# 2Retr0/GodotGaussianSplatting

Hardware: NVIDIA H100
Metric: Msplats/s (higher is better)
Workload: dtype f32

## Files before the change

### godotgaussiansplatting_b200/csrc/common.cuh

```cuda
#pragma once
#include <cuda_runtime.h>
#include <stdint.h>
#include <stdio.h>

#include "../../include/gsr.h"

namespace gsr {

constexpr int TILE = 16;
constexpr int NUM_PLANES = 15;
constexpr int PROJ_THREADS = 256;

void set_last_error(const char *fmt, ...);

#define GSR_CUDA_TRY(expr)                                                                         \
    do {                                                                                           \
        cudaError_t _e = (expr);                                                                   \
        if (_e != cudaSuccess) {                                                                   \
            ::gsr::set_last_error("%s:%d: %s -> %s", __FILE__, __LINE__, #expr, cudaGetErrorString(_e)); \
            return (_e == cudaErrorMemoryAllocation) ? GSR_ERR_OOM : GSR_ERR_CUDA;                 \
        }                                                                                          \
    } while (0)

__device__ __forceinline__ float g_max(float x, float y) { return (x < y) ? y : x; }
__device__ __forceinline__ float g_min(float x, float y) { return (y < x) ? y : x; }
__device__ __forceinline__ float g_clamp(float x, float lo, float hi) { return g_min(g_max(x, lo), hi); }

__device__ __forceinline__ float det_exp2(float t) {
    const float MAGIC = 12582912.0f;
    float tc = g_min(g_max(t, -127.0f), 128.0f);
    float tm = __fadd_rn(tc, MAGIC);
    float nf = __fsub_rn(tm, MAGIC);
    float f = __fsub_rn(tc, nf);
    float p = 0x1.446c7ep-13f;
    p = __fmaf_rn(p, f, 0x1.5f48c8p-10f);
    p = __fmaf_rn(p, f, 0x1.3b29d8p-7f);
    p = __fmaf_rn(p, f, 0x1.c6aeccp-5f);
    p = __fmaf_rn(p, f, 0x1.ebfbe0p-3f);
    p = __fmaf_rn(p, f, 0x1.62e430p-1f);
    p = __fmaf_rn(p, f, 1.0f);
    uint32_t sbits = (__float_as_uint(tm) << 23) + 0x3F800000u;
    return __fmul_rn(p, __uint_as_float(sbits));
}

__device__ __forceinline__ float det_exp(float x) { return det_exp2(__fmul_rn(x, 0x1.715476p+0f)); }

__device__ __forceinline__ float det_log2(float x) {
    int eadj = 0;
    if (x < 0x1p-126f) { x = __fmul_rn(x, 0x1p+32f); eadj = -32; }
    uint32_t u = __float_as_uint(x);
    int e = (int)(u >> 23) - 127;
    float m = __uint_as_float((u & 0x007FFFFFu) | 0x3F800000u);
    if (m >= 0x1.6a09e6p+0f) { m = __fmul_rn(m, 0.5f); e += 1; }
    float s = __fdiv_rn(__fsub_rn(m, 1.0f), __fadd_rn(m, 1.0f));
    float z = __fmul_rn(s, s);
    float g = 0x1.ba18b8p-2f;
    g = __fmaf_rn(g, z, 0x1.27471ep-1f);
    g = __fmaf_rn(g, z, 0x1.ec70e6p-1f);
    g = __fmaf_rn(g, z, 0x1.715476p+1f);
    return __fadd_rn((float)(e + eadj), __fmul_rn(s, g));
}

__device__ __forceinline__ float det_pow(float x, float y) {
    if (!(x > 0.0f)) return 0.0f;
    return det_exp2(__fmul_rn(y, det_log2(x)));
}

struct FrameState {
    unsigned long long dup_total;
    uint32_t dup_sorted;
    uint32_t visible;
    int32_t last_tile_plus1;
    uint32_t overflow;
    uint32_t proj_ticket;
    uint32_t pad0;
    unsigned long long staged;
    uint32_t comp_head;
    uint32_t comp_cta_limit;
    uint32_t pad[4];
};
static_assert(sizeof(FrameState) == 64, "FrameState is one 64-byte slot of the history ring");

struct Uniforms {
    float camera_pos[3];
    float model_scale;
    int32_t dims[2];
    float time;
    float pad;
};
static_assert(sizeof(Uniforms) == 32, "uniform block must be 32 bytes");

struct SortWorkspace {
    uint32_t *hist = nullptr;
    uint32_t *status = nullptr;
    uint32_t *tickets = nullptr;
    uint32_t *alt_keys = nullptr;
    uint32_t *alt_vals = nullptr;
    uint32_t *n_dev = nullptr;
    uint64_t max_n = 0;
    uint32_t max_tiles = 0;
    int grid_hist = 0, grid_sweep_pairs = 0, grid_sweep_keys = 0;
    size_t bytes() const;
};
int sort_workspace_create(SortWorkspace &ws, uint64_t max_n, bool need_alt_buffers);
void sort_workspace_destroy(SortWorkspace &ws);
int sort_pairs_device(SortWorkspace &ws, uint32_t *keys, uint32_t *vals, const uint32_t *n_ptr, uint32_t *alt_keys,
                      uint32_t *alt_vals, cudaStream_t stream, int *launches);
uint32_t sort_tile_keys();

struct ProjectionArgs {
    const float4 *soa;
    uint64_t plane_stride;
    uint32_t num_splats;
    float vp[32];
    Uniforms u;
    float focal_base[2];
    float lim_lo[2], lim_hi[2];
    int32_t band_y0, band_y1;
    int32_t row_mod, row_rem;
    int32_t fast_reject;
    int32_t sh_bulk_min;
    int32_t fast_mode;
    float w_frob2;
    float4 *records;
    uint32_t *keys, *values;
    uint32_t capacity;
    unsigned long long *lookback;
    FrameState *frame;
};
int launch_projection(const ProjectionArgs &a, cudaStream_t stream);

constexpr int GROUP_MAX = 16;
constexpr int GROUP_PHASES = 3;
#define GSR_GROUP_TIMEOUT_NS 2000000000ull
struct GroupFlags {
    unsigned long long seg_meta[GROUP_PHASES][GROUP_MAX][2];
    uint32_t done[GROUP_MAX];
    uint32_t released;
    uint32_t error;
    uint32_t scat_ticket;
    int32_t scat_last;
    unsigned long long seg_total[GROUP_MAX];
    uint32_t seg_prefix[GROUP_MAX + 1];
};
constexpr size_t GROUP_FLAGS_BYTES = 4096;
static_assert(sizeof(GroupFlags) <= GROUP_FLAGS_BYTES, "flag page");
struct GroupPeers {
    GroupFlags *flags[GROUP_MAX];
    int world, rank;
};
struct ScatterPeers {
    int world, rank, parity;
    uint32_t seq;
    uint32_t first, count;
    uint32_t seg_cap;
    float4 *records[GROUP_MAX];
    uint32_t *keys[GROUP_MAX];
    uint32_t *values[GROUP_MAX];
    GroupFlags *flags[GROUP_MAX];
    unsigned long long *lookback;
};
int launch_projection_scatter(const ProjectionArgs &a, const ScatterPeers &sp, cudaStream_t stream);
uint32_t projection_scatter_blocks(uint32_t count);
int launch_group_wait_segments(GroupFlags *flags, int parity, int world, uint32_t seq, uint32_t seg_cap, uint32_t capacity, FrameState *frame, cudaStream_t stream);
int launch_gather_segments(const GroupFlags *flags, int world, uint32_t seg_cap, const uint32_t *rx_keys, const uint32_t *rx_vals, uint32_t *keys, uint32_t *vals,
                           int grid, cudaStream_t stream);
int launch_publish_frame_state(const FrameState *frame, FrameState *host_mapped, cudaStream_t stream);
int launch_group_wait_released(GroupFlags *flags, uint32_t need, cudaStream_t stream);
int launch_group_wait_done(GroupFlags *flags, int world, uint32_t seq, cudaStream_t stream);
int launch_group_signal_done(const GroupPeers &peers, int root, int rank, uint32_t seq, cudaStream_t stream);
int launch_group_release(const GroupPeers &peers, int world, uint32_t value, cudaStream_t stream);
uint32_t projection_num_blocks(uint32_t num_splats);

int launch_tile_ranges(const uint32_t *sorted_keys, const FrameState *frame, uint2 *bounds, uint32_t num_tiles,
                       int quirks, int sharded, int32_t *sync_word, int grid, cudaStream_t stream);
int launch_band_fixup(const int32_t *global_last_plus1, float4 *out, int32_t width, int32_t height, int32_t tiles_x, int32_t num_tiles_total,
                      int32_t band_y0, int32_t band_y1, int32_t row_mod, int32_t row_rem, cudaStream_t stream);

struct CompositeArgs {
    const float4 *records;
    const uint32_t *values;
    const uint2 *bounds;
    float4 *out;
    int32_t width, height, tiles_x;
    int32_t tile_begin;
    int32_t row_step;
    int32_t num_tiles;
    float heatmap_factor;
    uint32_t target_tile_id;
    float4 *pick;
    FrameState *frame;
    int32_t count_staged;
    const uint32_t *order;
    uint32_t *consumed;
    int32_t ctas_per_sm;
    int32_t sm_count;
    int32_t contract;
    ulonglong4 *trace;
    uint32_t *trace_count;
    uint32_t trace_cap;
};
int launch_composite(const CompositeArgs &a, cudaStream_t stream);
int composite_max_ctas_per_sm(int *out);
int launch_tile_order(const uint2 *bounds, int32_t tile_begin, int32_t row_step, int32_t tiles_x, int32_t num_tiles, uint32_t *hint, uint32_t *order,
                      FrameState *frame, uint32_t sparse_tiles, uint32_t sparse_cta_limit, cudaStream_t stream);

int launch_ply_to_soa(const float *ply, uint32_t nprops, uint64_t count, float creation_time, float4 *soa, uint64_t plane_stride, uint64_t first,
                      cudaStream_t stream);
int launch_present(const float4 *rgba, void *out, uint64_t pixels, int format, cudaStream_t stream);
size_t present_bytes_per_pixel(int format);
int launch_aos_to_soa(const float4 *aos, uint64_t count, float4 *soa, uint64_t plane_stride, uint64_t first, cudaStream_t stream);

int preload_group_kernels();
int preload_projection_kernels();
int preload_sort_kernels();
int preload_ranges_kernels();
int launch_frame_clear(FrameState *frame, unsigned long long *links, uint32_t n_links, uint2 *bounds, uint32_t n_bounds, cudaStream_t stream);
int preload_ingest_kernels();
int preload_present_kernels();
int preload_composite_kernels();

}
```

### godotgaussiansplatting_b200/csrc/compositor.cu

```cuda
#include <stdlib.h>
#include <string.h>

#include "common.cuh"

namespace gsr {

namespace {

constexpr int CHUNK = 256;
constexpr int THREADS = 128;
constexpr float MIN_ALPHA = 1.0f / 255.0f;

struct F2 { float lo, hi; };
__device__ __forceinline__ F2 pk(float lo, float hi) { F2 r; r.lo = lo; r.hi = hi; return r; }
__device__ __forceinline__ void upk(F2 v, float &lo, float &hi) { lo = v.lo; hi = v.hi; }
__device__ __forceinline__ F2 fma2(F2 a, F2 b, F2 c) { return pk(__fmaf_rn(a.lo, b.lo, c.lo), __fmaf_rn(a.hi, b.hi, c.hi)); }
__device__ __forceinline__ F2 mul2(F2 a, F2 b) { return pk(__fmul_rn(a.lo, b.lo), __fmul_rn(a.hi, b.hi)); }
__device__ __forceinline__ F2 add2(F2 a, F2 b) { return pk(__fadd_rn(a.lo, b.lo), __fadd_rn(a.hi, b.hi)); }
__device__ __forceinline__ F2 sub2(F2 a, F2 b) { return pk(__fsub_rn(a.lo, b.lo), __fsub_rn(a.hi, b.hi)); }
__device__ __forceinline__ F2 mul_add2_unfused(F2 a, F2 b, F2 c) { return add2(mul2(a, b), c); }
__device__ __forceinline__ F2 bc(float x) { return pk(x, x); }

struct Staged {
    float4 a;
    float4 b;
    float c;
};

__device__ __forceinline__ Staged null_splat() {
    Staged s;
    s.a = make_float4(0.f, 0.f, 0.f, 0.f);
    s.b = make_float4(0.f, 0.f, 0.f, 0.f);
    s.c = 0.f;
    return s;
}

__device__ __forceinline__ Staged gather(const float4 *__restrict__ records, const uint32_t *__restrict__ values, uint32_t idx) {
    const uint32_t v = __ldg(values + idx);
    const float4 *r = records + (uint64_t)v * 3u;
    const float4 r0 = __ldg(r + 0), r1 = __ldg(r + 1), r2 = __ldg(r + 2);
    Staged s;
    s.a = make_float4(r0.x, r0.y, -0.5f * r1.x, -0.5f * r1.z);
    s.b = make_float4(-r1.y, r2.w, r2.x, r2.y);
    s.c = r2.z;
    return s;
}

#ifndef GSR_COMP_GROUP
#define GSR_COMP_GROUP 4
#endif
constexpr int GU = GSR_COMP_GROUP;
static_assert(CHUNK % GU == 0, "a chunk is a whole number of groups");

#ifndef GSR_CPU_EMU
__device__ __forceinline__ unsigned long long globaltimer_ns() { unsigned long long t; asm volatile("mov.u64 %0, %globaltimer;" : "=l"(t)); return t; }
__device__ __forceinline__ uint32_t smid() { uint32_t r; asm volatile("mov.u32 %0, %smid;" : "=r"(r)); return r; }
#else
inline unsigned long long globaltimer_ns() { return 0ull; }
inline uint32_t smid() { return 0u; }
#endif

struct BlendK {
    F2 L2E2, MAGIC2, ONE2, C6, C5, C4, C3, C2, C1;
};
__device__ __forceinline__ BlendK make_blend_k() {
    BlendK k;
    k.L2E2 = bc(0x1.715476p+0f); k.MAGIC2 = bc(12582912.0f); k.ONE2 = bc(1.0f);
    k.C6 = bc(0x1.446c7ep-13f); k.C5 = bc(0x1.5f48c8p-10f); k.C4 = bc(0x1.3b29d8p-7f); k.C3 = bc(0x1.c6aeccp-5f);
    k.C2 = bc(0x1.ebfbe0p-3f); k.C1 = bc(0x1.62e430p-1f);
    return k;
}

template <bool CONTRACT>
__device__ __forceinline__ void phase_a(const float4 A[GU], const float4 B[GU], F2 npx2, float fpy, const BlendK &K, F2 al2[GU], F2 om2[GU]) {
    float oy[GU];
    F2 ox2[GU], pw2[GU], tm2[GU], e2[GU];
#pragma unroll
    for (int u = 0; u < GU; ++u) { ox2[u] = add2(bc(A[u].x), npx2); oy[u] = A[u].y - fpy; }
#pragma unroll
    for (int u = 0; u < GU; ++u) pw2[u] = mul2(bc(A[u].z), ox2[u]);
#pragma unroll
    for (int u = 0; u < GU; ++u) {
        const float czoy = A[u].w * oy[u];
        if (CONTRACT) pw2[u] = fma2(bc(czoy), bc(oy[u]), mul2(pw2[u], ox2[u]));
        else pw2[u] = mul_add2_unfused(pw2[u], ox2[u], bc(__fmul_rn(czoy, oy[u])));
    }
#pragma unroll
    for (int u = 0; u < GU; ++u) e2[u] = mul2(bc(B[u].x), ox2[u]);
#pragma unroll
    for (int u = 0; u < GU; ++u) pw2[u] = CONTRACT ? fma2(e2[u], bc(oy[u]), pw2[u]) : mul_add2_unfused(e2[u], bc(oy[u]), pw2[u]);
#pragma unroll
    for (int u = 0; u < GU; ++u) pw2[u] = mul2(pw2[u], K.L2E2);
#pragma unroll
    for (int u = 0; u < GU; ++u) {
        float tl, th;
        upk(pw2[u], tl, th);
        tl = g_min(g_max(tl, -127.0f), 128.0f);
        th = g_min(g_max(th, -127.0f), 128.0f);
        pw2[u] = pk(tl, th);
    }
#pragma unroll
    for (int u = 0; u < GU; ++u) tm2[u] = add2(pw2[u], K.MAGIC2);
#pragma unroll
    for (int u = 0; u < GU; ++u) al2[u] = sub2(tm2[u], K.MAGIC2);
#pragma unroll
    for (int u = 0; u < GU; ++u) pw2[u] = sub2(pw2[u], al2[u]);
#pragma unroll
    for (int u = 0; u < GU; ++u) e2[u] = fma2(K.C6, pw2[u], K.C5);
#pragma unroll
    for (int u = 0; u < GU; ++u) e2[u] = fma2(e2[u], pw2[u], K.C4);
#pragma unroll
    for (int u = 0; u < GU; ++u) e2[u] = fma2(e2[u], pw2[u], K.C3);
#pragma unroll
    for (int u = 0; u < GU; ++u) e2[u] = fma2(e2[u], pw2[u], K.C2);
#pragma unroll
    for (int u = 0; u < GU; ++u) e2[u] = fma2(e2[u], pw2[u], K.C1);
#pragma unroll
    for (int u = 0; u < GU; ++u) e2[u] = fma2(e2[u], pw2[u], K.ONE2);
#pragma unroll
    for (int u = 0; u < GU; ++u) {
        float ml, mh;
        upk(tm2[u], ml, mh);
        tm2[u] = pk(__uint_as_float((__float_as_uint(ml) << 23) + 0x3F800000u), __uint_as_float((__float_as_uint(mh) << 23) + 0x3F800000u));
    }
#pragma unroll
    for (int u = 0; u < GU; ++u) e2[u] = mul2(e2[u], tm2[u]);
#pragma unroll
    for (int u = 0; u < GU; ++u) al2[u] = mul2(bc(B[u].y), e2[u]);
#pragma unroll
    for (int u = 0; u < GU; ++u) om2[u] = sub2(K.ONE2, al2[u]);
}

template <bool CONTRACT>
__device__ __forceinline__ void phase_b(const float4 B[GU], const float *s_c, int j, const F2 al2[GU], const F2 om2[GU], F2 &cr2, F2 &cg2, F2 &cb2,
                                        float &t0, float &t1, bool &alive_mid) {
#pragma unroll
    for (int u = 0; u < GU; ++u) {
        const float cbl = s_c[j + u];
        if (u == GU / 2) alive_mid = (t0 > MIN_ALPHA) || (t1 > MIN_ALPHA);
        const bool a0 = t0 > MIN_ALPHA, a1 = t1 > MIN_ALPHA;
        float al, ah, pl, ph;
        upk(al2[u], al, ah);
        const F2 t2 = pk(t0, t1);
        upk(mul2(t2, om2[u]), pl, ph);
        const F2 m2 = pk(a0 ? al : 0.0f, a1 ? ah : 0.0f);
        if (CONTRACT) {
            cr2 = fma2(mul2(bc(B[u].z), m2), t2, cr2);
            cg2 = fma2(mul2(bc(B[u].w), m2), t2, cg2);
            cb2 = fma2(mul2(bc(cbl), m2), t2, cb2);
        } else {
            cr2 = mul_add2_unfused(mul2(bc(B[u].z), m2), t2, cr2);
            cg2 = mul_add2_unfused(mul2(bc(B[u].w), m2), t2, cg2);
            cb2 = mul_add2_unfused(mul2(bc(cbl), m2), t2, cb2);
        }
        t0 = a0 ? pl : t0;
        t1 = a1 ? ph : t1;
    }
}

#ifndef GSR_COMP_MIN_BLOCKS
#define GSR_COMP_MIN_BLOCKS 3
#endif

template <bool CONTRACT>
__global__ void __launch_bounds__(THREADS, GSR_COMP_MIN_BLOCKS) composite_kernel(const __grid_constant__ CompositeArgs p) {
    __shared__ float4 s_a[CHUNK];
    __shared__ float4 s_b[CHUNK];
    __shared__ float s_c[CHUNK];
    __shared__ uint32_t s_vote[THREADS / 32];
    __shared__ uint32_t s_tile;

    const uint32_t tid = threadIdx.x, lane = tid & 31u, warp = tid >> 5;
    {
        const uint32_t limit = p.frame->comp_cta_limit;
        if (limit && blockIdx.x >= limit) return;
    }
    const BlendK K = make_blend_k();
    uint32_t staged = 0;
    unsigned long long t_start = 0;

    for (;;) {
        if (tid == 0) {
            const uint32_t ticket = atomicAdd(&p.frame->comp_head, 1u);
            s_tile = ticket < (uint32_t)p.num_tiles ? (p.order ? p.order[ticket] : ticket) : 0xFFFFFFFFu;
            if (p.trace) t_start = globaltimer_ns();
        }
        __syncthreads();
        const uint32_t local_tile = s_tile;
        if (local_tile == 0xFFFFFFFFu) break;
        const uint32_t tile_id = (uint32_t)p.tile_begin + (local_tile / (uint32_t)p.tiles_x) * (uint32_t)(p.row_step * p.tiles_x) + local_tile % (uint32_t)p.tiles_x;

        const uint32_t tx = tile_id % (uint32_t)p.tiles_x, ty = tile_id / (uint32_t)p.tiles_x;
        const int px0 = (int)(tx * TILE + 2u * (tid & 7u)), py = (int)(ty * TILE + (tid >> 3));
        const F2 npx2 = pk(-(float)px0, -(float)(px0 + 1));
        const float fpy = (float)py;

        const uint2 bounds = p.bounds[tile_id];
        const int32_t diff = (int32_t)(bounds.y - bounds.x);
        const int num_splats = diff > 0 ? diff : 0;
        const int num_iterations = (int)ceilf((float)num_splats / (float)CHUNK);

        F2 cr2 = pk(0.f, 0.f), cg2 = cr2, cb2 = cr2;
        float t0 = 1.0f, t1 = 1.0f;

        Staged n0 = null_splat(), n1 = null_splat();
        if (num_iterations > 0) {
            if ((int)tid < num_splats) n0 = gather(p.records, p.values, bounds.x + tid);
            if ((int)tid + THREADS < num_splats) n1 = gather(p.records, p.values, bounds.x + tid + THREADS);
        }

        int consumed = 0;
        for (int i = 0; i < num_iterations; ++i) {
            const int sort_offset = CHUNK * i;
            const int chunk = (num_splats - sort_offset) < CHUNK ? (num_splats - sort_offset) : CHUNK;
            staged += (uint32_t)chunk;
            consumed = i + 1;
            s_a[tid] = n0.a; s_b[tid] = n0.b; s_c[tid] = n0.c;
            s_a[tid + THREADS] = n1.a; s_b[tid + THREADS] = n1.b; s_c[tid + THREADS] = n1.c;
            __syncthreads();
            n0 = null_splat(); n1 = null_splat();
            if (i + 1 < num_iterations) {
                const int nb = sort_offset + CHUNK;
                if (nb + (int)tid < num_splats) n0 = gather(p.records, p.values, bounds.x + (uint32_t)nb + tid);
                if (nb + (int)tid + THREADS < num_splats) n1 = gather(p.records, p.values, bounds.x + (uint32_t)nb + tid + THREADS);
            }

            const int chunkg = (chunk + GU - 1) & ~(GU - 1);
            float4 A[GU], B[GU];
#pragma unroll
            for (int u = 0; u < GU; ++u) { A[u] = s_a[u]; B[u] = s_b[u]; }
            bool go = __any_sync(0xffffffffu, (t0 > MIN_ALPHA) || (t1 > MIN_ALPHA));
            for (int j = 0; j < chunkg && go; j += GU) {
                F2 al2[GU], om2[GU];
                phase_a<CONTRACT>(A, B, npx2, fpy, K, al2, om2);
                float4 Bc[GU];
#pragma unroll
                for (int u = 0; u < GU; ++u) Bc[u] = B[u];
                const int jn = (j + GU < CHUNK) ? j + GU : j;
#pragma unroll
                for (int u = 0; u < GU; ++u) { A[u] = s_a[jn + u]; B[u] = s_b[jn + u]; }
                bool alive_mid = true;
                phase_b<CONTRACT>(Bc, s_c, j, al2, om2, cr2, cg2, cb2, t0, t1, alive_mid);
                go = __any_sync(0xffffffffu, alive_mid);
            }

            const uint32_t wsum = __reduce_add_sync(0xffffffffu, (uint32_t)(t0 * 255.0f) + (uint32_t)(t1 * 255.0f));
            if (lane == 0) s_vote[warp] = wsum;
            __syncthreads();
            uint32_t shared_t = 0;
#pragma unroll
            for (int w = 0; w < THREADS / 32; ++w) shared_t += s_vote[w];
            if (!(shared_t > 255u)) break;
        }

        float r0, r1, g0, g1, b0, b1;
        upk(cr2, r0, r1); upk(cg2, g0, g1); upk(cb2, b0, b1);
        const float hx = (float)num_splats * 5e-4f;
        const float h0 = 0.0f * (1.0f - hx) + 1.0f * hx, h1 = 0.0f * (1.0f - hx) + 0.2f * hx, h2c = 1.0f * (1.0f - hx) + 0.2f * hx;
        if (py < p.height) {
            float4 *row = p.out + (uint64_t)py * (uint64_t)p.width;
            const float k0 = 1.0f - t0, k1 = 1.0f - t1;
            if (px0 < p.width)
                row[px0] = make_float4(r0 + h0 * k0 * p.heatmap_factor, g0 + h1 * k0 * p.heatmap_factor, b0 + h2c * k0 * p.heatmap_factor, 1.0f);
            if (px0 + 1 < p.width)
                row[px0 + 1] = make_float4(r1 + h0 * k1 * p.heatmap_factor, g1 + h1 * k1 * p.heatmap_factor, b1 + h2c * k1 * p.heatmap_factor, 1.0f);
        }
        if ((tid & 15u) == 0u && tile_id == p.target_tile_id && t0 != 1.0f) {
            const uint32_t v = p.values[bounds.x + (bounds.y - bounds.x) / 10u];
            const float4 q0 = p.records[(uint64_t)v * 3u + 0], q1 = p.records[(uint64_t)v * 3u + 1];
            *p.pick = make_float4(q0.z, q0.w, q1.w, (float)num_splats);
        }
        if (tid == 0) {
            if (p.consumed) p.consumed[local_tile] = (uint32_t)consumed | 0x80000000u;
            if (p.trace) {
                const uint32_t k = atomicAdd(p.trace_count, 1u);
                if (k < p.trace_cap) p.trace[k] = make_ulonglong4(((unsigned long long)tile_id << 32) | smid(), t_start, globaltimer_ns(),
                                                                  ((unsigned long long)(uint32_t)consumed << 32) | 1u | ((uint32_t)num_iterations << 1));
            }
        }
        __syncthreads();
    }
    if (tid == 0 && staged && p.count_staged) atomicAdd(&p.frame->staged, (unsigned long long)staged);
}

}

#ifndef GSR_CPU_EMU
int preload_composite_kernels() {
    cudaFuncAttributes fa;
    GSR_CUDA_TRY(cudaFuncGetAttributes(&fa, composite_kernel<true>));
    GSR_CUDA_TRY(cudaFuncGetAttributes(&fa, composite_kernel<false>));
    return GSR_OK;
}

int composite_max_ctas_per_sm(int *out) {
    int a = 0, b = 0;
    GSR_CUDA_TRY(cudaOccupancyMaxActiveBlocksPerMultiprocessor(&a, composite_kernel<true>, THREADS, 0));
    GSR_CUDA_TRY(cudaOccupancyMaxActiveBlocksPerMultiprocessor(&b, composite_kernel<false>, THREADS, 0));
    *out = a < b ? a : b;
    if (*out < 1) *out = 1;
    return GSR_OK;
}

int launch_composite(const CompositeArgs &a, cudaStream_t stream) {
    if (a.num_tiles <= 0) return GSR_OK;
    const int per_sm = a.ctas_per_sm > 0 ? a.ctas_per_sm : 1;
    const int grid = a.num_tiles < a.sm_count * per_sm ? a.num_tiles : a.sm_count * per_sm;
    if (a.contract) composite_kernel<true><<<grid, THREADS, 0, stream>>>(a);
    else composite_kernel<false><<<grid, THREADS, 0, stream>>>(a);
    GSR_CUDA_TRY(cudaGetLastError());
    return GSR_OK;
}
#endif

}
```

### godotgaussiansplatting_b200/csrc/gsr_api.cu

```cuda
#include <stdarg.h>
#include <stdlib.h>
#include <stddef.h>
#include <string.h>
#include <unistd.h>

#include <new>

#include "common.cuh"

namespace gsr {

static thread_local char g_last_error[512] = "";

void set_last_error(const char *fmt, ...) {
    va_list ap;
    va_start(ap, fmt);
    vsnprintf(g_last_error, sizeof g_last_error, fmt, ap);
    va_end(ap);
}

}

using namespace gsr;

constexpr int EV_PER_FRAME = 7;

struct gsr_ctx {
    int device = 0;
    uint32_t flags = 0;
    uint64_t max_splats = 0, capacity = 0, plane_stride = 0, num_splats = 0;
    uint64_t cap_stride = 0;
    cudaStream_t stream = nullptr, own_stream = nullptr;
    float4 *soa = nullptr;
    float4 *records = nullptr;
    float4 *records2 = nullptr;
    uint32_t *keys = nullptr;
    uint32_t *vals = nullptr;
    uint32_t *keys_cur = nullptr, *vals_cur = nullptr;
    float4 *records_cur = nullptr;
    cudaStream_t front_stream = nullptr;
    cudaEvent_t front_gate = nullptr;
    int overlap = -1;
    SortWorkspace sort;
    FrameState *ring = nullptr;
    FrameState *frame = nullptr;
    unsigned long long *lookback = nullptr;
    uint32_t lookback_blocks = 0;
    uint64_t frame_counter = 0;
    uint2 *bounds = nullptr;
    uint32_t *comp_order = nullptr, *comp_hint = nullptr;
    int comp_ctas_per_sm = 2, comp_order_mode = 1, comp_max_ctas = 1, comp_sparse_per_sm = 5;
    uint64_t comp_hint_key = 0;
    FrameState *pick_frame = nullptr;
    ulonglong4 *trace = nullptr;
    uint32_t *trace_count = nullptr;
    uint32_t trace_cap = 0;
    float4 *fb = nullptr, *fb_ext = nullptr;
    float4 *fb2 = nullptr;
    void *stage[2] = {nullptr, nullptr};
    float4 *fb_last = nullptr;
    cudaStream_t copy_stream = nullptr;
    cudaEvent_t ev_done[2] = {nullptr, nullptr}, ev_copied[2] = {nullptr, nullptr};
    bool copied_valid[2] = {false, false};
    uint64_t async_counter = 0;
    bool peer_mode = false, peer_opened = false;
    float4 *peer_fb[2] = {nullptr, nullptr};
    uint64_t peer_counter = 0;
    float4 *pick = nullptr;
    float4 *staging = nullptr;
    uint64_t staging_splats = 0;
    uint32_t *unsorted_keys = nullptr, *unsorted_vals = nullptr;
    bool keep_unsorted = false;
    int width = 0, height = 0, tiles_x = 0, tiles_y = 0, band_y0 = 0, band_y1 = 0;
    bool band_set = false;
    int row_mod = 1, row_rem = 0;
    int32_t *sync_word = nullptr;
    struct Group {
        void *arena = nullptr;
        uint64_t rx_capacity = 0;
        int rank = 0, world = 0;
        char *peer_arena[GROUP_MAX] = {};
        GroupFlags *flags[GROUP_MAX] = {};
        float4 *root_fb[2] = {nullptr, nullptr};
        void *opened[3 * GROUP_MAX] = {};
        int n_opened = 0;
        int present_rows = 0;
        uint32_t seq = 0;
        uint64_t slice = 0;
        uint32_t seg_cap = 0;
    } grp;
    cudaEvent_t *ev = nullptr;
    FrameState *host_ring = nullptr;
    cudaEvent_t *ev_stat = nullptr;
    uint64_t stats_polled = 0;
    uint64_t m_high = 0;
    uint64_t capacity_max = 0;
    bool ev_valid = false;
    uint32_t last_launches = 0;
    int sm_count = 0;
};

struct gsr_sorter {
    int device = 0;
    SortWorkspace ws;
    cudaEvent_t e0 = nullptr, e1 = nullptr;
    bool timed = false;
};

namespace {

int use_device(int device) {
    GSR_CUDA_TRY(cudaSetDevice(device));
    return GSR_OK;
}

int check_device(int device) {
    int count = 0;
    cudaError_t e = cudaGetDeviceCount(&count);
    if (e != cudaSuccess || count == 0) {
        set_last_error("no CUDA device available (%s); libgsr has no CPU fallback", e != cudaSuccess ? cudaGetErrorString(e) : "count=0");
        return GSR_ERR_CUDA;
    }
    if (device < 0 || device >= count) {
        set_last_error("device ordinal %d out of range [0,%d)", device, count);
        return GSR_ERR_INVALID;
    }
    cudaDeviceProp prop;
    GSR_CUDA_TRY(cudaGetDeviceProperties(&prop, device));
    if (prop.major != 9 || prop.minor != 0) {
        set_last_error("device %d is sm_%d%d; libgsr is built for sm_90a only", device, prop.major, prop.minor);
        return GSR_ERR_CUDA;
    }
    return GSR_OK;
}

void group_detach(gsr_ctx *c) {
    if (c->front_stream) cudaStreamSynchronize(c->front_stream);
    if (c->stream) cudaStreamSynchronize(c->stream);
    if (c->copy_stream) cudaStreamSynchronize(c->copy_stream);
    for (int i = 0; i < c->grp.n_opened; ++i) cudaIpcCloseMemHandle(c->grp.opened[i]);
    c->grp.n_opened = 0;
    if (c->grp.world > 1) { c->row_mod = 1; c->row_rem = 0; }
    c->grp.world = 0; c->grp.rank = 0; c->grp.seq = 0; c->grp.present_rows = 0;
    c->grp.root_fb[0] = c->grp.root_fb[1] = nullptr;
}

float4 *framebuffer(gsr_ctx *c) { return c->fb_ext ? c->fb_ext : (c->fb_last ? c->fb_last : c->fb); }

void free_ctx(gsr_ctx *c) {
    if (!c) return;
    cudaSetDevice(c->device);
    if (c->stream) cudaStreamSynchronize(c->stream);
    if (c->front_stream) { cudaStreamSynchronize(c->front_stream); cudaStreamDestroy(c->front_stream); }
    cudaFree(c->soa); cudaFree(c->records); cudaFree(c->records2); cudaFree(c->keys); cudaFree(c->vals);
    sort_workspace_destroy(c->sort);
    if (c->copy_stream) cudaStreamSynchronize(c->copy_stream);
    if (c->peer_opened) { cudaIpcCloseMemHandle(c->peer_fb[0]); cudaIpcCloseMemHandle(c->peer_fb[1]); }
    cudaFree(c->stage[0]); cudaFree(c->stage[1]);
    cudaFree(c->ring); cudaFree(c->lookback); cudaFree(c->bounds); cudaFree(c->comp_order); cudaFree(c->comp_hint); cudaFree(c->pick_frame); cudaFree(c->fb); cudaFree(c->fb2); cudaFree(c->pick); cudaFree(c->staging);
    for (int i = 0; i < 2; ++i) { if (c->ev_done[i]) cudaEventDestroy(c->ev_done[i]); if (c->ev_copied[i]) cudaEventDestroy(c->ev_copied[i]); }
    if (c->copy_stream) cudaStreamDestroy(c->copy_stream);
    cudaFree(c->sync_word);
    for (int i = 0; i < c->grp.n_opened; ++i) cudaIpcCloseMemHandle(c->grp.opened[i]);
    cudaFree(c->grp.arena);
    cudaFree(c->unsorted_keys); cudaFree(c->unsorted_vals); cudaFree(c->trace); cudaFree(c->trace_count);
    if (c->ev) {
        for (int i = 0; i < GSR_HISTORY_FRAMES * EV_PER_FRAME; ++i) if (c->ev[i]) cudaEventDestroy(c->ev[i]);
        delete[] c->ev;
    }
    if (c->ev_stat) {
        for (int i = 0; i < GSR_HISTORY_FRAMES; ++i) if (c->ev_stat[i]) cudaEventDestroy(c->ev_stat[i]);
        delete[] c->ev_stat;
    }
    if (c->host_ring) cudaFreeHost(c->host_ring);
    if (c->own_stream) cudaStreamDestroy(c->own_stream);
    delete c;
}

}

extern "C" {

GSR_API const char *gsr_error_string(int code) {
    switch (code) {
        case GSR_OK: return "ok";
        case GSR_ERR_INVALID: return "invalid argument";
        case GSR_ERR_CUDA: return "CUDA failure or no usable sm_90 device (no CPU fallback exists)";
        case GSR_ERR_OOM: return "device out of memory";
        case GSR_ERR_STATE: return "call order violated";
        case GSR_ERR_OVERFLOW: return "duplicate list exceeded capacity";
        default: return "unknown error";
    }
}
GSR_API const char *gsr_last_error(void) { return g_last_error; }
GSR_API const char *gsr_version(void) { return "gsr 0.1.0 (sm_90a)"; }
GSR_API int gsr_device_count(void) {
    int n = 0;
    if (cudaGetDeviceCount(&n) != cudaSuccess) return 0;
    return n;
}

GSR_API int gsr_create(const gsr_config *cfg, gsr_ctx **out) {
    if (!cfg || !out || cfg->max_splats == 0) { set_last_error("gsr_create: null config/out or max_splats == 0"); return GSR_ERR_INVALID; }
    *out = nullptr;
    int rc = check_device(cfg->device);
    if (rc) return rc;
    if ((rc = use_device(cfg->device))) return rc;
    if (cfg->max_splats >= (1ull << 32) - 256ull) { set_last_error("max_splats must be < 2^32-256"); return GSR_ERR_INVALID; }
    gsr_ctx *c = new (std::nothrow) gsr_ctx();
    if (!c) return GSR_ERR_OOM;
    c->device = cfg->device;
    c->flags = cfg->flags;
    if (!(c->flags & (GSR_FLAG_REFERENCE_QUIRKS | GSR_FLAG_FIXED_RANGES))) c->flags |= GSR_FLAG_REFERENCE_QUIRKS;
    c->max_splats = cfg->max_splats;
    const uint64_t factor = cfg->dup_capacity_factor ? cfg->dup_capacity_factor : 10;
    c->capacity_max = (1ull << 30) - 1;
    c->capacity = c->max_splats * factor;
    if (c->capacity > c->capacity_max) c->capacity = c->capacity_max;
    c->plane_stride = (c->max_splats + 255ull) & ~255ull;
    cudaDeviceGetAttribute(&c->sm_count, cudaDevAttrMultiProcessorCount, c->device);
    if ((rc = composite_max_ctas_per_sm(&c->comp_max_ctas))) { delete c; return rc; }

#define TRY_ALLOC(ptr, bytes)                                                                      \
    do {                                                                                           \
        cudaError_t _e = cudaMalloc((void **)&(ptr), (bytes));                                     \
        if (_e != cudaSuccess) {                                                                   \
            set_last_error("cudaMalloc(%s, %llu B) -> %s", #ptr, (unsigned long long)(bytes), cudaGetErrorString(_e)); \
            free_ctx(c);                                                                           \
            return _e == cudaErrorMemoryAllocation ? GSR_ERR_OOM : GSR_ERR_CUDA;                   \
        }                                                                                          \
    } while (0)

    cudaError_t se;
    {
        int least = 0, greatest = 0;
        cudaDeviceGetStreamPriorityRange(&least, &greatest);
        se = cudaStreamCreateWithPriority(&c->own_stream, cudaStreamNonBlocking, greatest);
    }
    if (se != cudaSuccess) { set_last_error("cudaStreamCreate -> %s", cudaGetErrorString(se)); free_ctx(c); return GSR_ERR_CUDA; }
    c->stream = c->own_stream;
    se = cudaStreamCreateWithFlags(&c->copy_stream, cudaStreamNonBlocking);
    if (se == cudaSuccess) {
        int least = 0, greatest = 0;
        cudaDeviceGetStreamPriorityRange(&least, &greatest);
        se = cudaStreamCreateWithPriority(&c->front_stream, cudaStreamNonBlocking, least);
    }
    for (int i = 0; i < 2 && se == cudaSuccess; ++i) {
        se = cudaEventCreateWithFlags(&c->ev_done[i], cudaEventDisableTiming);
        if (se == cudaSuccess) se = cudaEventCreateWithFlags(&c->ev_copied[i], cudaEventDisableTiming);
    }
    if (se != cudaSuccess) { set_last_error("copy stream/events -> %s", cudaGetErrorString(se)); free_ctx(c); return GSR_ERR_CUDA; }
    TRY_ALLOC(c->soa, sizeof(float4) * NUM_PLANES * c->plane_stride);
    TRY_ALLOC(c->records, sizeof(float4) * 3ull * c->max_splats);
    TRY_ALLOC(c->records2, sizeof(float4) * 3ull * c->max_splats);
    c->cap_stride = (c->capacity + 1023ull) & ~1023ull;
    TRY_ALLOC(c->keys, sizeof(uint32_t) * 3ull * c->cap_stride);
    TRY_ALLOC(c->vals, sizeof(uint32_t) * 3ull * c->cap_stride);
    c->keys_cur = c->keys; c->vals_cur = c->vals; c->records_cur = c->records;
    c->lookback_blocks = projection_num_blocks((uint32_t)c->max_splats);
    TRY_ALLOC(c->ring, sizeof(FrameState) * GSR_HISTORY_FRAMES);
    TRY_ALLOC(c->lookback, sizeof(unsigned long long) * ((size_t)c->lookback_blocks + 2u * GROUP_MAX * GROUP_MAX));
    c->frame = c->ring;
    TRY_ALLOC(c->pick, sizeof(float4));
    TRY_ALLOC(c->sync_word, sizeof(int32_t));
    c->staging_splats = c->max_splats < (1ull << 18) ? c->max_splats : (1ull << 18);
    TRY_ALLOC(c->staging, sizeof(float4) * NUM_PLANES * c->staging_splats);
#undef TRY_ALLOC
    rc = sort_workspace_create(c->sort, c->capacity, false);
    if (rc) { free_ctx(c); return rc; }
    c->ev = new (std::nothrow) cudaEvent_t[GSR_HISTORY_FRAMES * EV_PER_FRAME]();
    if (!c->ev) { free_ctx(c); return GSR_ERR_OOM; }
    for (int i = 0; i < GSR_HISTORY_FRAMES * EV_PER_FRAME; ++i) {
        if (cudaEventCreate(&c->ev[i]) != cudaSuccess) { set_last_error("cudaEventCreate failed"); free_ctx(c); return GSR_ERR_CUDA; }
    }
    c->ev_stat = new (std::nothrow) cudaEvent_t[GSR_HISTORY_FRAMES]();
    if (!c->ev_stat) { free_ctx(c); return GSR_ERR_OOM; }
    for (int i = 0; i < GSR_HISTORY_FRAMES; ++i) {
        if (cudaEventCreateWithFlags(&c->ev_stat[i], cudaEventDisableTiming) != cudaSuccess) { set_last_error("cudaEventCreate failed"); free_ctx(c); return GSR_ERR_CUDA; }
    }
    if (cudaHostAlloc((void **)&c->host_ring, sizeof(FrameState) * GSR_HISTORY_FRAMES, cudaHostAllocMapped | cudaHostAllocPortable) != cudaSuccess) {
        set_last_error("cudaHostAlloc(frame mirror) failed"); c->host_ring = nullptr; free_ctx(c); return GSR_ERR_OOM;
    }
    memset(c->host_ring, 0, sizeof(FrameState) * GSR_HISTORY_FRAMES);
    cudaMemsetAsync(c->soa, 0, sizeof(float4) * NUM_PLANES * c->plane_stride, c->stream);
    cudaMemsetAsync(c->records, 0, sizeof(float4) * 3ull * c->max_splats, c->stream);
    cudaMemsetAsync(c->records2, 0, sizeof(float4) * 3ull * c->max_splats, c->stream);
    cudaMemsetAsync(c->pick, 0, sizeof(float4), c->stream);
    cudaMemsetAsync(c->sync_word, 0, sizeof(int32_t), c->stream);
    cudaMemsetAsync(c->ring, 0, sizeof(FrameState) * GSR_HISTORY_FRAMES, c->stream);
    if ((rc = preload_group_kernels()) || (rc = preload_projection_kernels()) || (rc = preload_sort_kernels()) || (rc = preload_ranges_kernels()) ||
        (rc = preload_ingest_kernels()) || (rc = preload_present_kernels()) || (rc = preload_composite_kernels())) { free_ctx(c); return rc; }
    cudaError_t e = cudaStreamSynchronize(c->stream);
    if (e != cudaSuccess) { set_last_error("init sync -> %s", cudaGetErrorString(e)); free_ctx(c); return GSR_ERR_CUDA; }
    *out = c;
    return GSR_OK;
}

GSR_API int gsr_destroy(gsr_ctx *ctx) {
    free_ctx(ctx);
    return GSR_OK;
}

GSR_API int gsr_set_stream(gsr_ctx *c, void *cuda_stream) {
    if (!c) return GSR_ERR_INVALID;
    int rc = use_device(c->device);
    if (rc) return rc;
    GSR_CUDA_TRY(cudaStreamSynchronize(c->front_stream));
    GSR_CUDA_TRY(cudaStreamSynchronize(c->stream));
    c->stream = cuda_stream ? (cudaStream_t)cuda_stream : c->own_stream;
    c->ev_valid = false; c->front_gate = nullptr;
    return GSR_OK;
}

GSR_API int gsr_upload_splats_aos(gsr_ctx *c, const float *splat60, uint64_t first, uint64_t count) {
    if (!c || (!splat60 && count)) return GSR_ERR_INVALID;
    if (count > c->max_splats || first > c->max_splats - count) { set_last_error("upload range [%llu,%llu) exceeds max_splats %llu", (unsigned long long)first, (unsigned long long)(first + count), (unsigned long long)c->max_splats); return GSR_ERR_INVALID; }
    int rc = use_device(c->device);
    if (rc) return rc;
    GSR_CUDA_TRY(cudaStreamSynchronize(c->front_stream));
    uint64_t done = 0;
    while (done < count) {
        const uint64_t m = (count - done) < c->staging_splats ? (count - done) : c->staging_splats;
        GSR_CUDA_TRY(cudaMemcpyAsync(c->staging, splat60 + (done * 60ull), m * 240ull, cudaMemcpyHostToDevice, c->stream));
        if ((rc = launch_aos_to_soa(c->staging, m, c->soa, c->plane_stride, first + done, c->stream))) return rc;
        done += m;
    }
    GSR_CUDA_TRY(cudaStreamSynchronize(c->stream));
    if (first + count > c->num_splats) c->num_splats = first + count;
    return GSR_OK;
}

GSR_API int gsr_upload_ply_raw(gsr_ctx *c, const float *ply, uint32_t nprops, uint64_t first, uint64_t count, float creation_time) {
    if (!c || (!ply && count)) return GSR_ERR_INVALID;
    if (nprops < 62 || nprops > 256) { set_last_error("gsr_upload_ply_raw: %u properties; need the 62 standard 3DGS floats (x..rot_3) first", nprops); return GSR_ERR_INVALID; }
    if (count > c->max_splats || first > c->max_splats - count) { set_last_error("upload range [%llu,%llu) exceeds max_splats %llu", (unsigned long long)first, (unsigned long long)(first + count), (unsigned long long)c->max_splats); return GSR_ERR_INVALID; }
    int rc = use_device(c->device);
    if (rc) return rc;
    const uint64_t staging_floats = c->staging_splats * 60ull;
    const uint64_t per = staging_floats / nprops;
    if (per == 0) { set_last_error("gsr_upload_ply_raw: staging buffer too small"); return GSR_ERR_INVALID; }
    GSR_CUDA_TRY(cudaStreamSynchronize(c->front_stream));
    uint64_t done = 0;
    while (done < count) {
        const uint64_t m = (count - done) < per ? (count - done) : per;
        GSR_CUDA_TRY(cudaMemcpyAsync(c->staging, ply + done * nprops, m * nprops * sizeof(float), cudaMemcpyHostToDevice, c->stream));
        if ((rc = launch_ply_to_soa(reinterpret_cast<const float *>(c->staging), nprops, m, creation_time, c->soa, c->plane_stride, first + done, c->stream))) return rc;
        done += m;
    }
    GSR_CUDA_TRY(cudaStreamSynchronize(c->stream));
    if (first + count > c->num_splats) c->num_splats = first + count;
    return GSR_OK;
}

GSR_API int gsr_resize(gsr_ctx *c, int32_t width, int32_t height) {
    if (!c || width < 1 || height < 1) { set_last_error("gsr_resize: bad size %dx%d", width, height); return GSR_ERR_INVALID; }
    const int tx = (width + TILE - 1) / TILE, ty = (height + TILE - 1) / TILE;
    if ((int64_t)tx * ty > 65536) {
        set_last_error("gsr_resize: %d tiles exceed the 16-bit tile id of the sort key", tx * ty);
        return GSR_ERR_INVALID;
    }
    int rc = use_device(c->device);
    if (rc) return rc;
    GSR_CUDA_TRY(cudaStreamSynchronize(c->front_stream));
    GSR_CUDA_TRY(cudaStreamSynchronize(c->stream));
    c->front_gate = nullptr;
    c->width = c->height = c->tiles_x = c->tiles_y = 0;
    cudaFree(c->bounds); c->bounds = nullptr;
    cudaFree(c->comp_order); c->comp_order = nullptr;
    cudaFree(c->comp_hint); c->comp_hint = nullptr;
    GSR_CUDA_TRY(cudaStreamSynchronize(c->copy_stream));
    cudaFree(c->fb); c->fb = nullptr;
    cudaFree(c->fb2); c->fb2 = nullptr;
    cudaFree(c->stage[0]); cudaFree(c->stage[1]); c->stage[0] = c->stage[1] = nullptr;
    c->fb_last = nullptr; c->copied_valid[0] = c->copied_valid[1] = false;
    if (c->peer_opened) { cudaIpcCloseMemHandle(c->peer_fb[0]); cudaIpcCloseMemHandle(c->peer_fb[1]); c->peer_opened = false; }
    c->peer_mode = false; c->peer_fb[0] = c->peer_fb[1] = nullptr; c->peer_counter = 0; c->async_counter = 0;
    group_detach(c);
    GSR_CUDA_TRY(cudaMalloc((void **)&c->bounds, sizeof(uint2) * (size_t)tx * ty));
    GSR_CUDA_TRY(cudaMalloc((void **)&c->comp_order, sizeof(uint32_t) * (size_t)tx * ty));
    GSR_CUDA_TRY(cudaMalloc((void **)&c->comp_hint, sizeof(uint32_t) * (size_t)tx * ty));
    GSR_CUDA_TRY(cudaMemsetAsync(c->comp_hint, 0, sizeof(uint32_t) * (size_t)tx * ty, c->stream));
    c->comp_hint_key = 0;
    if (!c->pick_frame) GSR_CUDA_TRY(cudaMalloc((void **)&c->pick_frame, sizeof(FrameState)));
    GSR_CUDA_TRY(cudaMalloc((void **)&c->fb, sizeof(float4) * (size_t)width * height));
    GSR_CUDA_TRY(cudaMalloc((void **)&c->fb2, sizeof(float4) * (size_t)width * height));
    GSR_CUDA_TRY(cudaMemsetAsync(c->fb, 0, sizeof(float4) * (size_t)width * height, c->stream));
    GSR_CUDA_TRY(cudaMemsetAsync(c->fb2, 0, sizeof(float4) * (size_t)width * height, c->stream));
    c->width = width; c->height = height; c->tiles_x = tx; c->tiles_y = ty;
    if (!c->band_set) { c->band_y0 = 0; c->band_y1 = ty; }
    if (c->band_y1 > ty) c->band_y1 = ty;
    if (c->band_y0 > c->band_y1) c->band_y0 = c->band_y1;
    return GSR_OK;
}

GSR_API int gsr_set_row_interleave(gsr_ctx *c, int32_t row_rem, int32_t row_mod) {
    if (!c || row_mod < 1 || row_rem < 0 || row_rem >= row_mod) { set_last_error("gsr_set_row_interleave: need 0 <= rem < mod"); return GSR_ERR_INVALID; }
    c->row_mod = row_mod; c->row_rem = row_rem;
    return GSR_OK;
}

GSR_API void *gsr_band_sync_word(gsr_ctx *c) { return c ? (void *)c->sync_word : nullptr; }

GSR_API int gsr_band_fixup(gsr_ctx *c) {
    if (!c) return GSR_ERR_INVALID;
    if (c->row_mod <= 1 || !c->fb_last) return GSR_OK;
    if (c->flags & GSR_FLAG_FIXED_RANGES) return GSR_OK;
    int rc = use_device(c->device);
    if (rc) return rc;
    return launch_band_fixup(c->sync_word, c->fb_last, c->width, c->height, c->tiles_x, c->tiles_x * c->tiles_y, c->band_y0, c->band_y1,
                             c->row_mod, c->row_rem, c->stream);
}

GSR_API int gsr_set_band(gsr_ctx *c, int32_t row_begin, int32_t row_end) {
    if (!c || c->tiles_y == 0) { set_last_error("gsr_set_band before gsr_resize"); return GSR_ERR_STATE; }
    if (row_begin < 0 || row_end > c->tiles_y || row_begin > row_end) { set_last_error("band [%d,%d) outside [0,%d]", row_begin, row_end, c->tiles_y); return GSR_ERR_INVALID; }
    c->band_y0 = row_begin; c->band_y1 = row_end;
    c->band_set = !(row_begin == 0 && row_end == c->tiles_y);
    return GSR_OK;
}

static void frame_constants(const float *view_proj, const Uniforms &u, ProjectionArgs &pa) {
    {
        const float tfi0 = view_proj[16 + 0], tfi1 = view_proj[16 + 5];
        const volatile float hw = (float)u.dims[0] * 0.5f, hh = (float)u.dims[1] * 0.5f;
        const volatile float f0 = hw * tfi0, f1 = hh * tfi1;
        const volatile float t0 = 1.0f / tfi0, t1 = 1.0f / tfi1;
        const volatile float n0 = -t0, n1 = -t1;
        pa.focal_base[0] = f0; pa.focal_base[1] = f1;
        pa.lim_lo[0] = n0 * 1.3f; pa.lim_lo[1] = n1 * 1.3f;
        pa.lim_hi[0] = t0 * 1.3f; pa.lim_hi[1] = t1 * 1.3f;
    }
    {
        float g[3][3];
        for (int i = 0; i < 3; ++i)
            for (int j = 0; j < 3; ++j) {
                g[i][j] = 0.0f;
                for (int r = 0; r < 3; ++r) g[i][j] += view_proj[4 * i + r] * view_proj[4 * j + r];
            }
        float nrm = 0.0f;
        for (int i = 0; i < 3; ++i) {
            float row = 0.0f;
            for (int j = 0; j < 3; ++j) row += g[i][j] < 0.0f ? -g[i][j] : g[i][j];
            nrm = row > nrm ? row : nrm;
        }
        pa.w_frob2 = nrm * 1.0001f;
    }
}

static int grow_capacity(gsr_ctx *c, uint64_t want) {
    if (want > c->capacity_max) want = c->capacity_max;
    if (want <= c->capacity) return GSR_OK;
    GSR_CUDA_TRY(cudaStreamSynchronize(c->front_stream));
    GSR_CUDA_TRY(cudaStreamSynchronize(c->stream));
    GSR_CUDA_TRY(cudaStreamSynchronize(c->copy_stream));
    c->front_gate = nullptr;
    cudaFree(c->keys); cudaFree(c->vals); c->keys = c->vals = c->keys_cur = c->vals_cur = nullptr;
    sort_workspace_destroy(c->sort);
    const bool unsorted = c->unsorted_keys != nullptr;
    cudaFree(c->unsorted_keys); cudaFree(c->unsorted_vals); c->unsorted_keys = c->unsorted_vals = nullptr;
    c->capacity = want;
    c->cap_stride = (c->capacity + 1023ull) & ~1023ull;
    GSR_CUDA_TRY(cudaMalloc((void **)&c->keys, sizeof(uint32_t) * 3ull * c->cap_stride));
    GSR_CUDA_TRY(cudaMalloc((void **)&c->vals, sizeof(uint32_t) * 3ull * c->cap_stride));
    c->keys_cur = c->keys; c->vals_cur = c->vals;
    if (unsorted) {
        GSR_CUDA_TRY(cudaMalloc((void **)&c->unsorted_keys, sizeof(uint32_t) * c->capacity));
        GSR_CUDA_TRY(cudaMalloc((void **)&c->unsorted_vals, sizeof(uint32_t) * c->capacity));
    }
    return sort_workspace_create(c->sort, c->capacity, false);
}

static int track_capacity(gsr_ctx *c) {
    if (c->flags & GSR_FLAG_STATIC_CAPACITY) return GSR_OK;
    while (c->stats_polled < c->frame_counter) {
        if (c->frame_counter - c->stats_polled > GSR_HISTORY_FRAMES) { c->stats_polled = c->frame_counter - GSR_HISTORY_FRAMES; continue; }
        const uint32_t slot = (uint32_t)(c->stats_polled % GSR_HISTORY_FRAMES);
        if (cudaEventQuery(c->ev_stat[slot]) != cudaSuccess) { cudaGetLastError(); break; }
        const uint64_t m = c->host_ring[slot].dup_total;
        if (m > c->m_high) c->m_high = m;
        c->stats_polled += 1;
    }
    if (c->m_high * 2ull > c->capacity && c->capacity < c->capacity_max) return grow_capacity(c, c->m_high * 3ull);
    return GSR_OK;
}

struct GroupFrame { uint32_t seq; int parity; int rows_local; };

static int stage_times(gsr_ctx *c, uint32_t slot, float out[5], float *front_ms) {
    cudaEvent_t *ev = c->ev + EV_PER_FRAME * slot;
    float front = 0.f, recv = 0.f;
    GSR_CUDA_TRY(cudaEventElapsedTime(&front, ev[0], ev[1]));
    GSR_CUDA_TRY(cudaEventElapsedTime(&recv, ev[2], ev[3]));
    out[0] = front + recv;
    for (int i = 1; i < 4; ++i) GSR_CUDA_TRY(cudaEventElapsedTime(&out[i], ev[2 + i], ev[3 + i]));
    out[4] = out[0] + out[1] + out[2] + out[3];
    if (front_ms) *front_ms = front;
    return GSR_OK;
}

static size_t arena_rx_keys_off(uint64_t cap, int parity) { return GROUP_FLAGS_BYTES + sizeof(uint32_t) * cap * (size_t)parity; }
static size_t arena_rx_vals_off(uint64_t cap, int parity) { return GROUP_FLAGS_BYTES + sizeof(uint32_t) * cap * (size_t)(GROUP_PHASES + parity); }
static size_t arena_records_off(uint64_t cap, uint64_t max_splats, int parity) { return GROUP_FLAGS_BYTES + sizeof(uint32_t) * cap * 2 * GROUP_PHASES + sizeof(float4) * 3ull * max_splats * (size_t)parity; }
static size_t arena_bytes(uint64_t cap, uint64_t max_splats) { return arena_records_off(cap, max_splats, GROUP_PHASES); }

static GroupPeers group_peers(const gsr_ctx *c, int parity) {
    (void)parity;
    GroupPeers p;
    memset(&p, 0, sizeof p);
    p.world = c->grp.world; p.rank = c->grp.rank;
    for (int r = 0; r < c->grp.world; ++r) p.flags[r] = c->grp.flags[r];
    return p;
}

static int render_enqueue(gsr_ctx *c, const float *view_proj, const void *uniforms32, float heatmap_factor, float4 *target = nullptr,
                          const GroupFrame *gf = nullptr) {
    if (!c || !view_proj || !uniforms32) return GSR_ERR_INVALID;
    if (c->width == 0) { set_last_error("gsr_render before gsr_resize"); return GSR_ERR_STATE; }
    Uniforms u;
    memcpy(&u, uniforms32, sizeof u);
    if (u.dims[0] != c->width || u.dims[1] != c->height) {
        set_last_error("uniform dims %dx%d differ from gsr_resize %dx%d", u.dims[0], u.dims[1], c->width, c->height);
        return GSR_ERR_INVALID;
    }
    int rc = use_device(c->device);
    if (rc) return rc;
    if ((rc = track_capacity(c))) return rc;
    cudaStream_t s = c->stream;
    const bool overlap = c->overlap > 0 && c->front_stream != nullptr;
    cudaStream_t fs = overlap ? c->front_stream : s;
    int launches = 0;
    const uint32_t slot = (uint32_t)(c->frame_counter % GSR_HISTORY_FRAMES);
    c->frame = c->ring + slot;
    cudaEvent_t *ev = c->ev + EV_PER_FRAME * slot;
    const int half = (int)(c->frame_counter & 1u);
    uint32_t *keys_in = c->keys + (size_t)half * c->cap_stride, *vals_in = c->vals + (size_t)half * c->cap_stride;
    uint32_t *keys_alt = c->keys + 2ull * c->cap_stride, *vals_alt = c->vals + 2ull * c->cap_stride;
    float4 *records = half ? c->records2 : c->records;
    const uint32_t n_tiles = (uint32_t)(c->tiles_x * c->tiles_y);

    if (overlap && c->front_gate) GSR_CUDA_TRY(cudaStreamWaitEvent(fs, c->front_gate, 0));
    {
        uint32_t links = projection_num_blocks((uint32_t)c->max_splats);
        if (gf) {
            const uint64_t first = (uint64_t)c->grp.rank * c->grp.slice;
            const uint64_t count = first < c->max_splats ? ((c->max_splats - first) < c->grp.slice ? (c->max_splats - first) : c->grp.slice) : 0;
            links = projection_scatter_blocks((uint32_t)count) * (uint32_t)c->grp.world;
        }
        if ((rc = launch_frame_clear(c->frame, c->lookback, links, overlap ? nullptr : c->bounds, overlap ? 0u : n_tiles, fs))) return rc;
        launches += 1;
    }
    GSR_CUDA_TRY(cudaEventRecord(ev[0], fs));

    ProjectionArgs pa;
    pa.soa = c->soa; pa.plane_stride = c->plane_stride; pa.num_splats = (uint32_t)c->max_splats;
    memcpy(pa.vp, view_proj, sizeof pa.vp);
    pa.u = u;
    frame_constants(view_proj, u, pa);
    const bool fast = c->row_mod > 1 && !gf;
    pa.band_y0 = c->band_y0; pa.band_y1 = c->band_y1;
    pa.row_mod = c->row_mod; pa.row_rem = c->row_rem;
    const bool want_reject = (c->flags & GSR_FLAG_FAST_REJECT) != 0 || c->row_mod >= 6;
    pa.fast_reject = (want_reject && fast) ? 1 : 0;
    pa.fast_mode = fast ? 1 : 0;
    pa.sh_bulk_min = (fast || c->row_mod > 1) ? 1 : 12;
    pa.records = records; pa.keys = keys_in; pa.values = vals_in; pa.capacity = (uint32_t)c->capacity;
    pa.lookback = c->lookback; pa.frame = c->frame;
    if (gf) {
        const int G = c->grp.world;
        ScatterPeers sp;
        memset(&sp, 0, sizeof sp);
        sp.world = G; sp.rank = c->grp.rank; sp.parity = gf->parity; sp.seq = gf->seq;
        const uint64_t first = (uint64_t)c->grp.rank * c->grp.slice;
        sp.first = (uint32_t)(first < c->max_splats ? first : c->max_splats);
        sp.count = (uint32_t)(first < c->max_splats ? ((c->max_splats - first) < c->grp.slice ? (c->max_splats - first) : c->grp.slice) : 0);
        sp.seg_cap = c->grp.seg_cap;
        for (int d = 0; d < G; ++d) {
            char *ar = c->grp.peer_arena[d];
            sp.records[d] = reinterpret_cast<float4 *>(ar + arena_records_off(c->grp.rx_capacity, c->max_splats, gf->parity));
            sp.keys[d] = reinterpret_cast<uint32_t *>(ar + arena_rx_keys_off(c->grp.rx_capacity, gf->parity)) + (size_t)c->grp.rank * c->grp.seg_cap;
            sp.values[d] = reinterpret_cast<uint32_t *>(ar + arena_rx_vals_off(c->grp.rx_capacity, gf->parity)) + (size_t)c->grp.rank * c->grp.seg_cap;
            sp.flags[d] = c->grp.flags[d];
        }
        sp.lookback = c->lookback;
        if ((rc = launch_projection_scatter(pa, sp, fs))) return rc;
        launches += 1;
    } else {
        if ((rc = launch_projection(pa, fs))) return rc;
        launches += pa.num_splats ? 1 : 0;
    }
    GSR_CUDA_TRY(cudaEventRecord(ev[1], fs));

    if (overlap) {
        GSR_CUDA_TRY(cudaStreamWaitEvent(s, ev[1], 0));
        if ((rc = launch_frame_clear(nullptr, nullptr, 0u, c->bounds, n_tiles, s))) return rc;
        launches += 1;
    }
    GSR_CUDA_TRY(cudaEventRecord(ev[2], s));
    if (gf) {
        const int G = c->grp.world;
        char *mine = c->grp.peer_arena[c->grp.rank];
        if ((rc = launch_group_wait_segments(c->grp.flags[c->grp.rank], gf->parity, G, gf->seq, c->grp.seg_cap, (uint32_t)c->capacity, c->frame, s))) return rc;
        if ((rc = launch_gather_segments(c->grp.flags[c->grp.rank], G, c->grp.seg_cap,
                                         reinterpret_cast<const uint32_t *>(mine + arena_rx_keys_off(c->grp.rx_capacity, gf->parity)),
                                         reinterpret_cast<const uint32_t *>(mine + arena_rx_vals_off(c->grp.rx_capacity, gf->parity)), keys_in, vals_in,
                                         c->sm_count * 8, s))) return rc;
        records = reinterpret_cast<float4 *>(mine + arena_records_off(c->grp.rx_capacity, c->max_splats, gf->parity));
        launches += 2;
    }
    c->keys_cur = keys_in; c->vals_cur = vals_in; c->records_cur = records;
    GSR_CUDA_TRY(cudaEventRecord(ev[3], s));

    if (c->keep_unsorted) {
        GSR_CUDA_TRY(cudaMemcpyAsync(c->unsorted_keys, keys_in, sizeof(uint32_t) * c->capacity, cudaMemcpyDeviceToDevice, s));
        GSR_CUDA_TRY(cudaMemcpyAsync(c->unsorted_vals, vals_in, sizeof(uint32_t) * c->capacity, cudaMemcpyDeviceToDevice, s));
    }
    const uint32_t *m_ptr = reinterpret_cast<const uint32_t *>(reinterpret_cast<const char *>(c->frame) + offsetof(FrameState, dup_sorted));
    if ((rc = sort_pairs_device(c->sort, keys_in, vals_in, m_ptr, keys_alt, vals_alt, s, &launches))) return rc;
    GSR_CUDA_TRY(cudaEventRecord(ev[4], s));

    const int sharded = fast ? 2 : ((!(c->band_y0 == 0 && c->band_y1 == c->tiles_y) || c->row_mod > 1) ? 1 : 0);
    if (fast) GSR_CUDA_TRY(cudaMemsetAsync(c->sync_word, 0, sizeof(int32_t), s));
    const int quirks = (c->flags & GSR_FLAG_FIXED_RANGES) ? 0 : 1;
    if ((rc = launch_tile_ranges(keys_in, c->frame, c->bounds, n_tiles, quirks, sharded, fast ? c->sync_word : nullptr, c->sm_count * 8, s))) return rc;
    launches += 1;
    GSR_CUDA_TRY(cudaEventRecord(ev[5], s));
    c->front_gate = ev[5];

    CompositeArgs ca;
    float4 *out_fb = c->fb_ext ? c->fb_ext : (target ? target : c->fb);
    for (int i = 0; i < 2; ++i) {
        const float4 *owned = c->peer_mode ? c->peer_fb[i] : (i ? c->fb2 : c->fb);
        if (c->copied_valid[i] && owned == out_fb) GSR_CUDA_TRY(cudaStreamWaitEvent(s, c->ev_copied[i], 0));
    }
    c->fb_last = out_fb;
    ca.records = records; ca.values = vals_in; ca.bounds = c->bounds; ca.out = out_fb;
    ca.width = c->width; ca.height = c->height; ca.tiles_x = c->tiles_x;
    {
        int first = c->band_y0 + ((c->row_rem - c->band_y0 % c->row_mod) + c->row_mod) % c->row_mod;
        int nrows = first < c->band_y1 ? (c->band_y1 - 1 - first) / c->row_mod + 1 : 0;
        ca.tile_begin = first * c->tiles_x;
        ca.row_step = c->row_mod;
        ca.num_tiles = nrows * c->tiles_x;
    }
    ca.heatmap_factor = heatmap_factor;
    ca.target_tile_id = 0xFFFFFFFFu;
    ca.pick = c->pick;
    ca.frame = c->frame; ca.count_staged = 1;
    ca.order = nullptr; ca.consumed = c->comp_hint;
    ca.ctas_per_sm = c->comp_ctas_per_sm < c->comp_max_ctas ? c->comp_ctas_per_sm : c->comp_max_ctas; ca.sm_count = c->sm_count;
    ca.contract = (c->flags & GSR_FLAG_UNCONTRACTED_BLEND) ? 0 : 1;
    {
        const uint64_t key = ((uint64_t)(uint32_t)ca.tile_begin << 32) ^ ((uint64_t)(uint32_t)ca.row_step << 24) ^ (uint64_t)(uint32_t)ca.num_tiles;
        if (key != c->comp_hint_key) { GSR_CUDA_TRY(cudaMemsetAsync(c->comp_hint, 0, sizeof(uint32_t) * (size_t)c->tiles_x * c->tiles_y, s)); c->comp_hint_key = key; }
    }
    if (c->comp_order_mode && ca.num_tiles > 0) {
        if ((rc = launch_tile_order(c->bounds, ca.tile_begin, ca.row_step, ca.tiles_x, ca.num_tiles, c->comp_hint, c->comp_order, c->frame,
                                    (uint32_t)(c->comp_sparse_per_sm * c->sm_count), (uint32_t)c->sm_count, s))) return rc;
        ca.order = c->comp_order;
        launches += 1;
    }
    ca.trace = c->trace; ca.trace_count = c->trace_count; ca.trace_cap = c->trace_cap;
    if (c->trace) GSR_CUDA_TRY(cudaMemsetAsync(c->trace_count, 0, sizeof(uint32_t), s));
    if (gf && !gf->rows_local && c->grp.rank != 0 && gf->seq >= 3u) {
        if ((rc = launch_group_wait_released(c->grp.flags[c->grp.rank], gf->seq - 2u, s))) return rc;
        launches += 1;
    }
    if ((rc = launch_composite(ca, s))) return rc;
    launches += ca.num_tiles > 0 ? 1 : 0;
    if (gf && !gf->rows_local) {
        if ((rc = launch_group_signal_done(group_peers(c, gf->parity), 0, c->grp.rank, gf->seq, s))) return rc;
        launches += 1;
    }
    GSR_CUDA_TRY(cudaEventRecord(ev[6], s));
    if ((rc = launch_publish_frame_state(c->frame, c->host_ring + slot, s))) return rc;
    GSR_CUDA_TRY(cudaEventRecord(c->ev_stat[slot], s));
    c->ev_valid = true;
    c->frame_counter += 1;
    c->last_launches = (uint32_t)launches;
    return GSR_OK;
}

GSR_API int gsr_render(gsr_ctx *c, const float view_proj[32], const void *uniforms32, float heatmap_factor, float *out_host) {
    if (c && c->grp.world > 1) { set_last_error("gsr_render: a context attached to a group renders with gsr_render_async (all ranks, same frame)"); return GSR_ERR_STATE; }
    int rc = render_enqueue(c, view_proj, uniforms32, heatmap_factor);
    if (rc) return rc;
    if (out_host) {
        for (int attempt = 0; attempt < 8 && !(c->flags & GSR_FLAG_STATIC_CAPACITY); ++attempt) {
            const uint32_t slot = (uint32_t)((c->frame_counter - 1) % GSR_HISTORY_FRAMES);
            GSR_CUDA_TRY(cudaEventSynchronize(c->ev_stat[slot]));
            const FrameState &fs = c->host_ring[slot];
            if (!fs.overflow || c->capacity >= c->capacity_max) break;
            if ((rc = grow_capacity(c, fs.dup_total + fs.dup_total / 4ull + 1024ull))) return rc;
            if ((rc = render_enqueue(c, view_proj, uniforms32, heatmap_factor))) return rc;
        }
        GSR_CUDA_TRY(cudaMemcpyAsync(out_host, framebuffer(c), sizeof(float4) * (size_t)c->width * c->height, cudaMemcpyDeviceToHost, c->stream));
        GSR_CUDA_TRY(cudaStreamSynchronize(c->stream));
    }
    return GSR_OK;
}

static int readback_enqueue(gsr_ctx *c, float4 *frame, int slot, void *pinned_host, int format, uint32_t group_seq = 0) {
    const size_t pixels = (size_t)c->width * c->height;
    const size_t bpp = present_bytes_per_pixel(format);
    if (!bpp) { set_last_error("unknown output format 0x%x", format); return GSR_ERR_INVALID; }
    int rc;
    const bool convert = format != GSR_OUT_RGBA32F;
    if (convert && !c->stage[slot]) GSR_CUDA_TRY(cudaMalloc(&c->stage[slot], sizeof(float4) * pixels + 64));
    GSR_CUDA_TRY(cudaEventRecord(c->ev_done[slot], c->stream));
    GSR_CUDA_TRY(cudaStreamWaitEvent(c->copy_stream, c->ev_done[slot], 0));
    if (group_seq && (rc = launch_group_wait_done(c->grp.flags[c->grp.rank], c->grp.world, group_seq, c->copy_stream))) return rc;
    if (convert) {
        if ((rc = launch_present(frame, c->stage[slot], pixels, format, c->copy_stream))) return rc;
        GSR_CUDA_TRY(cudaMemcpyAsync(pinned_host, c->stage[slot], bpp * pixels, cudaMemcpyDeviceToHost, c->copy_stream));
    } else {
        GSR_CUDA_TRY(cudaMemcpyAsync(pinned_host, frame, sizeof(float4) * pixels, cudaMemcpyDeviceToHost, c->copy_stream));
    }
    GSR_CUDA_TRY(cudaEventRecord(c->ev_copied[slot], c->copy_stream));
    c->copied_valid[slot] = true;
    return GSR_OK;
}

static int render_async_impl(gsr_ctx *c, const float *view_proj, const void *uniforms32, float heatmap_factor, void *pinned_host, int format) {
    if (!c) return GSR_ERR_INVALID;
    if (c->grp.world > 1) {
        if (pinned_host) { set_last_error("group mode: render with a NULL host pointer on every rank, then gsr_readback_async on rank 0"); return GSR_ERR_STATE; }
        int rc = use_device(c->device);
        if (rc) return rc;
        GroupFrame gf;
        gf.seq = c->grp.seq + 1u; gf.parity = (int)(gf.seq % (uint32_t)GROUP_PHASES);
        const int slot = (int)((gf.seq - 1u) & 1u);
        gf.rows_local = c->grp.present_rows;
        float4 *target = c->grp.root_fb[slot];
        if (gf.rows_local) {
            target = slot ? c->fb2 : c->fb;
        } else if (c->grp.rank == 0) {
            if (c->copied_valid[slot]) GSR_CUDA_TRY(cudaStreamWaitEvent(c->stream, c->ev_copied[slot], 0));
            if (gf.seq >= 3u && (rc = launch_group_release(group_peers(c, gf.parity), c->grp.world, gf.seq - 2u, c->stream))) return rc;
        }
        if ((rc = render_enqueue(c, view_proj, uniforms32, heatmap_factor, target, &gf))) return rc;
        c->grp.seq = gf.seq;
        return GSR_OK;
    }
    if (c->peer_mode) {
        if (pinned_host) { set_last_error("peer mode: render with a NULL host pointer, then gsr_readback_async on the presenting rank"); return GSR_ERR_STATE; }
        int rc = use_device(c->device);
        if (rc) return rc;
        const int slot = (int)(c->peer_counter & 1u);
        if (c->copied_valid[slot]) GSR_CUDA_TRY(cudaStreamWaitEvent(c->stream, c->ev_copied[slot], 0));
        if ((rc = render_enqueue(c, view_proj, uniforms32, heatmap_factor, c->peer_fb[slot]))) return rc;
        c->peer_counter += 1;
        return GSR_OK;
    }
    if (!pinned_host || c->fb_ext) {
        if (format != GSR_OUT_RGBA32F && pinned_host) { set_last_error("converted read-back is unavailable with an external framebuffer"); return GSR_ERR_STATE; }
        int rc = render_enqueue(c, view_proj, uniforms32, heatmap_factor);
        if (rc) return rc;
        if (pinned_host)
            GSR_CUDA_TRY(cudaMemcpyAsync(pinned_host, framebuffer(c), sizeof(float4) * (size_t)c->width * c->height, cudaMemcpyDeviceToHost, c->stream));
        return GSR_OK;
    }
    int rc = use_device(c->device);
    if (rc) return rc;
    const int slot = (int)(c->async_counter & 1u);
    float4 *target = slot ? c->fb2 : c->fb;
    if ((rc = render_enqueue(c, view_proj, uniforms32, heatmap_factor, target))) return rc;
    if ((rc = readback_enqueue(c, target, slot, pinned_host, format))) return rc;
    c->async_counter += 1;
    return GSR_OK;
}

GSR_API int gsr_render_async(gsr_ctx *c, const float view_proj[32], const void *uniforms32, float heatmap_factor, float *pinned_host) {
    return render_async_impl(c, view_proj, uniforms32, heatmap_factor, pinned_host, GSR_OUT_RGBA32F);
}

GSR_API int gsr_render_async_rgb(gsr_ctx *c, const float view_proj[32], const void *uniforms32, float heatmap_factor, float *pinned_host_rgb) {
    return render_async_impl(c, view_proj, uniforms32, heatmap_factor, pinned_host_rgb, GSR_OUT_RGB32F);
}

GSR_API int gsr_render_async_fmt(gsr_ctx *c, const float view_proj[32], const void *uniforms32, float heatmap_factor, void *pinned_host, int32_t format) {
    if (!present_bytes_per_pixel(format)) { set_last_error("unknown output format 0x%x", format); return GSR_ERR_INVALID; }
    return render_async_impl(c, view_proj, uniforms32, heatmap_factor, pinned_host, format);
}

GSR_API size_t gsr_output_bytes(int32_t format, int32_t width, int32_t height) {
    return (width > 0 && height > 0) ? present_bytes_per_pixel(format) * (size_t)width * (size_t)height : 0;
}

GSR_API int gsr_present_device(gsr_ctx *c, void *dst_device, int32_t format) {
    if (!c || !dst_device) return GSR_ERR_INVALID;
    if (!c->fb_last && !c->fb_ext) { set_last_error("gsr_present_device: no frame rendered yet"); return GSR_ERR_STATE; }
    if (!present_bytes_per_pixel(format)) { set_last_error("unknown output format 0x%x", format); return GSR_ERR_INVALID; }
    int rc = use_device(c->device);
    if (rc) return rc;
    if (c->grp.world > 1) {
        if (c->grp.rank != 0) { set_last_error("gsr_present_device: only rank 0 of a group presents the frame"); return GSR_ERR_STATE; }
        if ((rc = launch_group_wait_done(c->grp.flags[0], c->grp.world, c->grp.seq, c->stream))) return rc;
    }
    return launch_present(framebuffer(c), dst_device, (uint64_t)c->width * c->height, format, c->stream);
}

GSR_API int gsr_readback_async(gsr_ctx *c, void *pinned_host, int32_t format) {
    if (!c || !pinned_host) return GSR_ERR_INVALID;
    if (!c->fb_last || c->fb_ext) { set_last_error("gsr_readback_async: no library-owned frame rendered yet"); return GSR_ERR_STATE; }
    int rc = use_device(c->device);
    if (rc) return rc;
    if (c->grp.world > 1) {
        if (c->grp.rank != 0) { set_last_error("gsr_readback_async: only rank 0 of a group presents the frame"); return GSR_ERR_STATE; }
        return readback_enqueue(c, c->fb_last, (int)((c->grp.seq - 1u) & 1u), pinned_host, format, c->grp.seq);
    }
    const int slot = (c->fb_last == c->fb2 || (c->peer_mode && c->fb_last == c->peer_fb[1])) ? 1 : 0;
    return readback_enqueue(c, c->fb_last, slot, pinned_host, format);
}

GSR_API int gsr_group_set_present(gsr_ctx *c, int32_t rows_local) {
    if (!c) return GSR_ERR_INVALID;
    if (c->grp.world <= 1) { set_last_error("gsr_group_set_present: attach the group first"); return GSR_ERR_STATE; }
    int rc = use_device(c->device);
    if (rc) return rc;
    GSR_CUDA_TRY(cudaStreamSynchronize(c->stream));
    GSR_CUDA_TRY(cudaStreamSynchronize(c->copy_stream));
    c->grp.present_rows = rows_local != 0;
    c->copied_valid[0] = c->copied_valid[1] = false;
    return GSR_OK;
}

GSR_API int gsr_readback_rows_async(gsr_ctx *c, void *host_frame) {
    if (!c || !host_frame) return GSR_ERR_INVALID;
    if (c->grp.world <= 1 || !c->grp.present_rows || !c->fb_last) { set_last_error("gsr_readback_rows_async: needs an attached group in rows-local presentation and a rendered frame"); return GSR_ERR_STATE; }
    int rc = use_device(c->device);
    if (rc) return rc;
    const int slot = (int)((c->grp.seq - 1u) & 1u);
    const size_t row_bytes = sizeof(float4) * (size_t)c->width, slab = row_bytes * TILE;
    const int G = c->grp.world, r = c->grp.rank;
    GSR_CUDA_TRY(cudaEventRecord(c->ev_done[slot], c->stream));
    GSR_CUDA_TRY(cudaStreamWaitEvent(c->copy_stream, c->ev_done[slot], 0));
    const int full_rows = c->height / TILE;
    const int n_full = r < full_rows ? (full_rows - 1 - r) / G + 1 : 0;
    const char *src = reinterpret_cast<const char *>(c->fb_last);
    char *dst = static_cast<char *>(host_frame);
    if (n_full) GSR_CUDA_TRY(cudaMemcpy2DAsync(dst + (size_t)r * slab, (size_t)G * slab, src + (size_t)r * slab, (size_t)G * slab, slab, (size_t)n_full,
                                               cudaMemcpyDeviceToHost, c->copy_stream));
    if (c->height % TILE && full_rows % G == r)
        GSR_CUDA_TRY(cudaMemcpyAsync(dst + (size_t)full_rows * slab, src + (size_t)full_rows * slab, row_bytes * (size_t)(c->height % TILE), cudaMemcpyDeviceToHost, c->copy_stream));
    GSR_CUDA_TRY(cudaEventRecord(c->ev_copied[slot], c->copy_stream));
    c->copied_valid[slot] = true;
    return GSR_OK;
}

GSR_API int gsr_peer_export_framebuffers(gsr_ctx *c, void *handles128) {
    if (!c || !handles128) return GSR_ERR_INVALID;
    if (!c->fb || !c->fb2 || c->fb_ext) { set_last_error("gsr_peer_export_framebuffers: call gsr_resize first (library-owned frames only)"); return GSR_ERR_STATE; }
    int rc = use_device(c->device);
    if (rc) return rc;
    cudaIpcMemHandle_t h[2];
    GSR_CUDA_TRY(cudaIpcGetMemHandle(&h[0], c->fb));
    GSR_CUDA_TRY(cudaIpcGetMemHandle(&h[1], c->fb2));
    memcpy(handles128, h, sizeof h);
    c->peer_fb[0] = c->fb; c->peer_fb[1] = c->fb2;
    c->peer_mode = true;
    return GSR_OK;
}

GSR_API int gsr_peer_import_framebuffers(gsr_ctx *c, const void *handles128) {
    if (!c || !handles128) return GSR_ERR_INVALID;
    int rc = use_device(c->device);
    if (rc) return rc;
    cudaIpcMemHandle_t h[2];
    memcpy(h, handles128, sizeof h);
    GSR_CUDA_TRY(cudaIpcOpenMemHandle((void **)&c->peer_fb[0], h[0], cudaIpcMemLazyEnablePeerAccess));
    GSR_CUDA_TRY(cudaIpcOpenMemHandle((void **)&c->peer_fb[1], h[1], cudaIpcMemLazyEnablePeerAccess));
    c->peer_mode = true; c->peer_opened = true;
    return GSR_OK;
}

namespace {
struct GroupBlob {
    uint32_t magic, version;
    uint64_t pid;
    int32_t device, width, height, pad;
    uint64_t max_splats, rx_capacity;
    void *arena, *fb[2];
    cudaIpcMemHandle_t h_arena, h_fb[2];
    unsigned char reserved[GSR_GROUP_BLOB_BYTES - 264];
};
static_assert(sizeof(GroupBlob) == GSR_GROUP_BLOB_BYTES, "blob layout");
constexpr uint32_t GROUP_MAGIC = 0x47535247u;

}

GSR_API int gsr_group_export(gsr_ctx *c, void *blob) {
    if (!c || !blob) return GSR_ERR_INVALID;
    if (!c->fb || !c->fb2 || c->fb_ext) { set_last_error("gsr_group_export: call gsr_resize first (library-owned frames only)"); return GSR_ERR_STATE; }
    int rc = use_device(c->device);
    if (rc) return rc;
    if (!c->grp.arena) {
        c->grp.rx_capacity = (c->capacity + 1023ull) & ~1023ull;
        const size_t bytes = arena_bytes(c->grp.rx_capacity, c->max_splats);
        cudaError_t e = cudaMalloc(&c->grp.arena, bytes);
        if (e != cudaSuccess) { set_last_error("cudaMalloc(group arena, %zu B) -> %s", bytes, cudaGetErrorString(e)); c->grp.arena = nullptr; return GSR_ERR_OOM; }
        GSR_CUDA_TRY(cudaMemset(c->grp.arena, 0, bytes));
    }
    GroupBlob b;
    memset(&b, 0, sizeof b);
    b.magic = GROUP_MAGIC; b.version = 1; b.pid = (uint64_t)getpid();
    b.device = c->device; b.width = c->width; b.height = c->height;
    b.max_splats = c->max_splats; b.rx_capacity = c->grp.rx_capacity;
    b.arena = c->grp.arena; b.fb[0] = c->fb; b.fb[1] = c->fb2;
    if (cudaIpcGetMemHandle(&b.h_arena, c->grp.arena) != cudaSuccess || cudaIpcGetMemHandle(&b.h_fb[0], c->fb) != cudaSuccess ||
        cudaIpcGetMemHandle(&b.h_fb[1], c->fb2) != cudaSuccess) {
        cudaGetLastError();
        memset(&b.h_arena, 0, sizeof b.h_arena); memset(b.h_fb, 0, sizeof b.h_fb);
    }
    memcpy(blob, &b, sizeof b);
    return GSR_OK;
}

GSR_API int gsr_group_attach(gsr_ctx *c, int32_t rank, int32_t world, const void *blobs) {
    if (!c || !blobs || world < 1 || world > GROUP_MAX || rank < 0 || rank >= world) { set_last_error("gsr_group_attach: need 0 <= rank < world <= %d", GROUP_MAX); return GSR_ERR_INVALID; }
    if (!c->grp.arena || !c->fb) { set_last_error("gsr_group_attach before gsr_group_export"); return GSR_ERR_STATE; }
    int rc = use_device(c->device);
    if (rc) return rc;
    group_detach(c);
    if (world == 1) return GSR_OK;
    const GroupBlob *B = reinterpret_cast<const GroupBlob *>(blobs);
    const uint64_t slice = (((c->max_splats + (uint64_t)world - 1) / (uint64_t)world) + 255ull) & ~255ull;
    for (int r = 0; r < world; ++r) {
        if (B[r].magic != GROUP_MAGIC || B[r].version != 1) { set_last_error("gsr_group_attach: blob %d is not a gsr_group_export blob", r); return GSR_ERR_INVALID; }
        if (B[r].max_splats != c->max_splats || B[r].width != c->width || B[r].height != c->height || B[r].rx_capacity != c->grp.rx_capacity) {
            set_last_error("gsr_group_attach: rank %d was created with a different scene / frame size", r);
            return GSR_ERR_INVALID;
        }
    }
    if (B[rank].arena != c->grp.arena || B[rank].pid != (uint64_t)getpid()) { set_last_error("gsr_group_attach: blob %d is not this context's export", rank); return GSR_ERR_INVALID; }
    auto fail = [&](const char *what, int r, cudaError_t e) {
        set_last_error("gsr_group_attach: %s of rank %d -> %s", what, r, cudaGetErrorString(e));
        group_detach(c);
        return GSR_ERR_CUDA;
    };
    for (int r = 0; r < world; ++r) {
        char *arena = nullptr;
        float4 *fb[2] = {nullptr, nullptr};
        if (r == rank) {
            arena = (char *)c->grp.arena; fb[0] = c->fb; fb[1] = c->fb2;
        } else if (B[r].pid == (uint64_t)getpid()) {
            if (B[r].device != c->device) {
                int can = 0;
                cudaDeviceCanAccessPeer(&can, c->device, B[r].device);
                if (!can) return fail("no peer access to the device", r, cudaErrorPeerAccessUnsupported);
                cudaError_t e = cudaDeviceEnablePeerAccess(B[r].device, 0);
                if (e != cudaSuccess && e != cudaErrorPeerAccessAlreadyEnabled) return fail("cudaDeviceEnablePeerAccess", r, e);
                cudaGetLastError();
            }
            arena = (char *)B[r].arena; fb[0] = (float4 *)B[r].fb[0]; fb[1] = (float4 *)B[r].fb[1];
        } else {
            cudaError_t e = cudaIpcOpenMemHandle((void **)&arena, B[r].h_arena, cudaIpcMemLazyEnablePeerAccess);
            if (e != cudaSuccess) return fail("cudaIpcOpenMemHandle(arena)", r, e);
            c->grp.opened[c->grp.n_opened++] = arena;
            if (r == 0) {
                for (int k = 0; k < 2; ++k) {
                    e = cudaIpcOpenMemHandle((void **)&fb[k], B[r].h_fb[k], cudaIpcMemLazyEnablePeerAccess);
                    if (e != cudaSuccess) return fail("cudaIpcOpenMemHandle(frame)", r, e);
                    c->grp.opened[c->grp.n_opened++] = fb[k];
                }
            }
        }
        c->grp.flags[r] = reinterpret_cast<GroupFlags *>(arena);
        c->grp.peer_arena[r] = arena;
        if (r == 0) { c->grp.root_fb[0] = fb[0]; c->grp.root_fb[1] = fb[1]; }
    }
    GSR_CUDA_TRY(cudaMemsetAsync(c->grp.arena, 0, GROUP_FLAGS_BYTES, c->stream));
    GSR_CUDA_TRY(cudaStreamSynchronize(c->stream));
    c->grp.rank = rank; c->grp.world = world; c->grp.slice = slice; c->grp.seq = 0;
    c->grp.seg_cap = (uint32_t)(c->grp.rx_capacity / (uint64_t)world) & ~3u;
    c->row_mod = world; c->row_rem = rank;
    c->band_y0 = 0; c->band_y1 = c->tiles_y; c->band_set = false;
    c->copied_valid[0] = c->copied_valid[1] = false;
    return GSR_OK;
}

GSR_API int gsr_group_detach(gsr_ctx *c) {
    if (!c) return GSR_ERR_INVALID;
    int rc = use_device(c->device);
    if (rc) return rc;
    group_detach(c);
    return GSR_OK;
}

GSR_API int gsr_stream_join(gsr_ctx *c) {
    if (!c) return GSR_ERR_INVALID;
    int rc = use_device(c->device);
    if (rc) return rc;
    for (int i = 0; i < 2; ++i)
        if (c->copied_valid[i]) GSR_CUDA_TRY(cudaStreamWaitEvent(c->stream, c->ev_copied[i], 0));
    return GSR_OK;
}

GSR_API int gsr_sync(gsr_ctx *c) {
    if (!c) return GSR_ERR_INVALID;
    int rc = use_device(c->device);
    if (rc) return rc;
    GSR_CUDA_TRY(cudaStreamSynchronize(c->stream));
    GSR_CUDA_TRY(cudaStreamSynchronize(c->copy_stream));
    if (c->grp.world > 1) {
        uint32_t err = 0;
        GSR_CUDA_TRY(cudaMemcpy(&err, &c->grp.flags[c->grp.rank]->error, sizeof err, cudaMemcpyDeviceToHost));
        if (err) {
            cudaMemset(&c->grp.flags[c->grp.rank]->error, 0, sizeof err);
            set_last_error("group: a device-side wait timed out (%s)", err == 1 ? "segments of a peer" : "done / released flag");
            return GSR_ERR_STATE;
        }
    }
    return GSR_OK;
}

GSR_API void *gsr_framebuffer_device_ptr(gsr_ctx *c) { return c ? (void *)framebuffer(c) : nullptr; }

GSR_API int gsr_set_framebuffer_external(gsr_ctx *c, void *device_ptr) {
    if (!c) return GSR_ERR_INVALID;
    c->fb_ext = (float4 *)device_ptr;
    return GSR_OK;
}

GSR_API int gsr_pick(gsr_ctx *c, uint32_t tile_id, float heatmap_factor, float out_xyzn[4]) {
    if (!c || !out_xyzn) return GSR_ERR_INVALID;
    if (c->width == 0) { set_last_error("gsr_pick before gsr_resize"); return GSR_ERR_STATE; }
    if (c->frame_counter == 0 || !c->fb_last) { set_last_error("gsr_pick before the first gsr_render at this size"); return GSR_ERR_STATE; }
    int rc = use_device(c->device);
    if (rc) return rc;
    const uint32_t T = (uint32_t)(c->tiles_x * c->tiles_y);
    const uint32_t t0 = (uint32_t)(c->band_y0 * c->tiles_x), t1 = (uint32_t)(c->band_y1 * c->tiles_x);
    if (tile_id < T && tile_id >= t0 && tile_id < t1 && (int)(tile_id / (uint32_t)c->tiles_x) % c->row_mod == c->row_rem) {
        CompositeArgs ca;
        ca.records = c->records_cur; ca.values = c->vals_cur; ca.bounds = c->bounds; ca.out = framebuffer(c);
        ca.width = c->width; ca.height = c->height; ca.tiles_x = c->tiles_x;
        ca.tile_begin = (int32_t)tile_id; ca.num_tiles = 1; ca.row_step = 1;
        ca.heatmap_factor = heatmap_factor; ca.target_tile_id = tile_id; ca.pick = c->pick;
        ca.frame = c->pick_frame; ca.count_staged = 0;
        ca.order = nullptr; ca.consumed = nullptr; ca.ctas_per_sm = 1; ca.sm_count = c->sm_count;
        ca.contract = (c->flags & GSR_FLAG_UNCONTRACTED_BLEND) ? 0 : 1;
        ca.trace = nullptr; ca.trace_count = nullptr; ca.trace_cap = 0;
        for (int i = 0; i < 2; ++i)
            if (c->copied_valid[i]) GSR_CUDA_TRY(cudaStreamWaitEvent(c->stream, c->ev_copied[i], 0));
        GSR_CUDA_TRY(cudaMemsetAsync(c->pick_frame, 0, sizeof(FrameState), c->stream));
        if ((rc = launch_composite(ca, c->stream))) return rc;
    }
    GSR_CUDA_TRY(cudaMemcpyAsync(out_xyzn, c->pick, sizeof(float4), cudaMemcpyDeviceToHost, c->stream));
    GSR_CUDA_TRY(cudaStreamSynchronize(c->stream));
    return GSR_OK;
}

GSR_API int gsr_get_stats(gsr_ctx *c, gsr_stats *out) {
    if (!c || !out) return GSR_ERR_INVALID;
    int rc = use_device(c->device);
    if (rc) return rc;
    memset(out, 0, sizeof *out);
    FrameState fs;
    GSR_CUDA_TRY(cudaMemcpyAsync(&fs, c->frame, sizeof fs, cudaMemcpyDeviceToHost, c->stream));
    GSR_CUDA_TRY(cudaStreamSynchronize(c->stream));
    out->num_splats = c->num_splats;
    out->duplicates = fs.dup_total;
    out->visible = fs.visible;
    out->capacity = c->capacity;
    out->last_tile = (int64_t)fs.last_tile_plus1 - 1;
    out->overflow = fs.overflow;
    out->width = (uint32_t)c->width; out->height = (uint32_t)c->height;
    out->tiles_x = (uint32_t)c->tiles_x; out->tiles_y = (uint32_t)c->tiles_y;
    out->band_y0 = (uint32_t)c->band_y0; out->band_y1 = (uint32_t)c->band_y1;
    out->kernel_launches = c->last_launches;
    out->staged = fs.staged;
    if (c->ev_valid && c->frame_counter > 0) {
        if ((rc = stage_times(c, (uint32_t)((c->frame_counter - 1) % GSR_HISTORY_FRAMES), out->stage_ms, nullptr))) return rc;
    }
    return GSR_OK;
}

GSR_API int gsr_get_frame_history(gsr_ctx *c, uint32_t max_frames, gsr_frame_record *out, uint32_t *n_out) {
    if (!c || !out || !n_out) return GSR_ERR_INVALID;
    int rc = use_device(c->device);
    if (rc) return rc;
    *n_out = 0;
    if (!c->ev_valid || c->frame_counter == 0) return GSR_OK;
    uint64_t n = c->frame_counter < GSR_HISTORY_FRAMES ? c->frame_counter : GSR_HISTORY_FRAMES;
    if (n > max_frames) n = max_frames;
    static thread_local FrameState host_ring[GSR_HISTORY_FRAMES];
    GSR_CUDA_TRY(cudaMemcpyAsync(host_ring, c->ring, sizeof(FrameState) * GSR_HISTORY_FRAMES, cudaMemcpyDeviceToHost, c->stream));
    GSR_CUDA_TRY(cudaStreamSynchronize(c->stream));
    for (uint64_t k = 0; k < n; ++k) {
        const uint64_t fi = c->frame_counter - n + k;
        const uint32_t slot = (uint32_t)(fi % GSR_HISTORY_FRAMES);
        const FrameState &fs = host_ring[slot];
        gsr_frame_record &r = out[k];
        memset(&r, 0, sizeof r);
        r.frame_index = fi; r.duplicates = fs.dup_total; r.visible = fs.visible; r.staged = fs.staged; r.overflow = fs.overflow;
        if ((rc = stage_times(c, slot, r.stage_ms, &r.front_ms))) return rc;
    }
    *n_out = (uint32_t)n;
    return GSR_OK;
}

GSR_API int gsr_debug_keep_unsorted(gsr_ctx *c, int enable) {
    if (!c) return GSR_ERR_INVALID;
    int rc = use_device(c->device);
    if (rc) return rc;
    if (enable && !c->unsorted_keys) {
        GSR_CUDA_TRY(cudaMalloc((void **)&c->unsorted_keys, sizeof(uint32_t) * c->capacity));
        GSR_CUDA_TRY(cudaMalloc((void **)&c->unsorted_vals, sizeof(uint32_t) * c->capacity));
    }
    c->keep_unsorted = enable != 0;
    return GSR_OK;
}

GSR_API int gsr_debug_compositor_config(gsr_ctx *c, int32_t ctas_per_sm, int32_t longest_first, int32_t sparse_tiles_per_sm) {
    if (!c || ctas_per_sm < 0 || sparse_tiles_per_sm < 0) return GSR_ERR_INVALID;
    c->comp_ctas_per_sm = ctas_per_sm ? ctas_per_sm : c->comp_max_ctas; c->comp_order_mode = longest_first != 0; c->comp_sparse_per_sm = sparse_tiles_per_sm;
    return GSR_OK;
}

GSR_API int gsr_debug_pipeline(gsr_ctx *c, int32_t overlap) {
    if (!c) return GSR_ERR_INVALID;
    int rc = use_device(c->device);
    if (rc) return rc;
    GSR_CUDA_TRY(cudaStreamSynchronize(c->front_stream));
    GSR_CUDA_TRY(cudaStreamSynchronize(c->stream));
    c->overlap = overlap < 0 ? -1 : (overlap != 0); c->front_gate = nullptr;
    return GSR_OK;
}

GSR_API int gsr_debug_enable_trace(gsr_ctx *c, uint32_t max_items) {
    if (!c) return GSR_ERR_INVALID;
    int rc = use_device(c->device);
    if (rc) return rc;
    GSR_CUDA_TRY(cudaStreamSynchronize(c->stream));
    cudaFree(c->trace); cudaFree(c->trace_count);
    c->trace = nullptr; c->trace_count = nullptr; c->trace_cap = 0;
    if (max_items) {
        GSR_CUDA_TRY(cudaMalloc((void **)&c->trace, sizeof(ulonglong4) * (size_t)max_items + 32));
        GSR_CUDA_TRY(cudaMalloc((void **)&c->trace_count, sizeof(uint32_t)));
        GSR_CUDA_TRY(cudaMemset(c->trace_count, 0, sizeof(uint32_t)));
        c->trace_cap = max_items;
    }
    return GSR_OK;
}

GSR_API int gsr_debug_copy(gsr_ctx *c, int which, void *dst, size_t bytes) {
    if (!c || !dst) return GSR_ERR_INVALID;
    int rc = use_device(c->device);
    if (rc) return rc;
    const void *src = nullptr;
    size_t avail = 0;
    switch (which) {
        case GSR_BUF_RECORDS: src = c->records_cur; avail = sizeof(float4) * 3ull * c->max_splats; break;
        case GSR_BUF_KEYS: src = c->keys_cur; avail = sizeof(uint32_t) * c->capacity; break;
        case GSR_BUF_VALUES: src = c->vals_cur; avail = sizeof(uint32_t) * c->capacity; break;
        case GSR_BUF_BOUNDS: src = c->bounds; avail = sizeof(uint2) * (size_t)c->tiles_x * c->tiles_y; break;
        case GSR_BUF_KEYS_UNSORTED: src = c->unsorted_keys; avail = c->unsorted_keys ? sizeof(uint32_t) * c->capacity : 0; break;
        case GSR_BUF_VALUES_UNSORTED: src = c->unsorted_vals; avail = c->unsorted_vals ? sizeof(uint32_t) * c->capacity : 0; break;
        case GSR_BUF_FRAMEBUFFER: src = framebuffer(c); avail = sizeof(float4) * (size_t)c->width * c->height; break;
        case GSR_BUF_COMPOSITOR_TRACE: src = c->trace; avail = c->trace ? sizeof(ulonglong4) * (size_t)c->trace_cap : 0; break;
        case GSR_BUF_COMPOSITOR_TRACE_COUNT: src = c->trace_count; avail = c->trace_count ? sizeof(uint32_t) : 0; break;
        default: set_last_error("gsr_debug_copy: unknown buffer %d", which); return GSR_ERR_INVALID;
    }
    if (!src || bytes > avail) { set_last_error("gsr_debug_copy(%d): %zu bytes requested, %zu available", which, bytes, avail); return GSR_ERR_INVALID; }
    GSR_CUDA_TRY(cudaMemcpyAsync(dst, src, bytes, cudaMemcpyDeviceToHost, c->stream));
    GSR_CUDA_TRY(cudaStreamSynchronize(c->stream));
    return GSR_OK;
}

GSR_API int gsr_sorter_create(int32_t device, uint64_t max_n, gsr_sorter **out) {
    if (!out || max_n == 0) return GSR_ERR_INVALID;
    *out = nullptr;
    int rc = check_device(device);
    if (rc) return rc;
    if ((rc = use_device(device))) return rc;
    gsr_sorter *s = new (std::nothrow) gsr_sorter();
    if (!s) return GSR_ERR_OOM;
    s->device = device;
    rc = sort_workspace_create(s->ws, max_n, true);
    if (rc == GSR_OK && (cudaEventCreate(&s->e0) != cudaSuccess || cudaEventCreate(&s->e1) != cudaSuccess)) rc = GSR_ERR_CUDA;
    if (rc) { sort_workspace_destroy(s->ws); delete s; return rc; }
    *out = s;
    return GSR_OK;
}

GSR_API int gsr_sorter_destroy(gsr_sorter *s) {
    if (!s) return GSR_OK;
    cudaSetDevice(s->device);
    cudaDeviceSynchronize();
    sort_workspace_destroy(s->ws);
    if (s->e0) cudaEventDestroy(s->e0);
    if (s->e1) cudaEventDestroy(s->e1);
    delete s;
    return GSR_OK;
}

GSR_API int gsr_sorter_sort_device(gsr_sorter *s, void *d_keys, void *d_values, uint64_t n, void *cuda_stream) {
    if (!s || (!d_keys && n)) return GSR_ERR_INVALID;
    if (n > s->ws.max_n) { set_last_error("sort of %llu exceeds sorter capacity %llu", (unsigned long long)n, (unsigned long long)s->ws.max_n); return GSR_ERR_INVALID; }
    int rc = use_device(s->device);
    if (rc) return rc;
    cudaStream_t st = (cudaStream_t)cuda_stream;
    const uint32_t n32 = (uint32_t)n;
    GSR_CUDA_TRY(cudaMemcpyAsync(s->ws.n_dev, &n32, sizeof n32, cudaMemcpyHostToDevice, st));
    GSR_CUDA_TRY(cudaEventRecord(s->e0, st));
    int launches = 0;
    rc = sort_pairs_device(s->ws, (uint32_t *)d_keys, (uint32_t *)d_values, s->ws.n_dev, s->ws.alt_keys, d_values ? s->ws.alt_vals : nullptr, st, &launches);
    if (rc) return rc;
    GSR_CUDA_TRY(cudaEventRecord(s->e1, st));
    s->timed = true;
    return GSR_OK;
}

GSR_API int gsr_sorter_last_ms(gsr_sorter *s, float *ms) {
    if (!s || !ms || !s->timed) return GSR_ERR_STATE;
    int rc = use_device(s->device);
    if (rc) return rc;
    GSR_CUDA_TRY(cudaEventSynchronize(s->e1));
    GSR_CUDA_TRY(cudaEventElapsedTime(ms, s->e0, s->e1));
    return GSR_OK;
}

GSR_API int gsr_sort_pairs_host(int32_t device, uint32_t *keys, uint32_t *values, uint64_t n) {
    if (n == 0) return GSR_OK;
    if (!keys) return GSR_ERR_INVALID;
    gsr_sorter *s = nullptr;
    int rc = gsr_sorter_create(device, n, &s);
    if (rc) return rc;
    uint32_t *dk = nullptr, *dv = nullptr;
    cudaError_t e = cudaMalloc((void **)&dk, 4 * n);
    if (e == cudaSuccess && values) e = cudaMalloc((void **)&dv, 4 * n);
    if (e == cudaSuccess) e = cudaMemcpy(dk, keys, 4 * n, cudaMemcpyHostToDevice);
    if (e == cudaSuccess && values) e = cudaMemcpy(dv, values, 4 * n, cudaMemcpyHostToDevice);
    if (e == cudaSuccess) {
        rc = gsr_sorter_sort_device(s, dk, dv, n, nullptr);
        if (rc == GSR_OK) e = cudaDeviceSynchronize();
    }
    if (e == cudaSuccess && rc == GSR_OK) e = cudaMemcpy(keys, dk, 4 * n, cudaMemcpyDeviceToHost);
    if (e == cudaSuccess && rc == GSR_OK && values) e = cudaMemcpy(values, dv, 4 * n, cudaMemcpyDeviceToHost);
    cudaFree(dk); cudaFree(dv);
    gsr_sorter_destroy(s);
    if (e != cudaSuccess) { set_last_error("gsr_sort_pairs_host: %s", cudaGetErrorString(e)); return e == cudaErrorMemoryAllocation ? GSR_ERR_OOM : GSR_ERR_CUDA; }
    return rc;
}

}
```

### godotgaussiansplatting_b200/csrc/ingest.cu

```cuda
#include "common.cuh"

namespace gsr {

namespace {

constexpr int SPLATS_PER_BLOCK = 128;

__global__ void __launch_bounds__(256) aos_to_soa_kernel(const float4 *__restrict__ aos, uint64_t count, float4 *__restrict__ soa,
                                                         uint64_t plane_stride, uint64_t first) {
    __shared__ float4 s[SPLATS_PER_BLOCK * NUM_PLANES];
    const uint64_t s0 = (uint64_t)blockIdx.x * SPLATS_PER_BLOCK;
    const uint32_t here = (uint32_t)((count - s0) < (uint64_t)SPLATS_PER_BLOCK ? (count - s0) : SPLATS_PER_BLOCK);
    const float4 *src = aos + s0 * NUM_PLANES;
    for (uint32_t i = threadIdx.x; i < here * NUM_PLANES; i += blockDim.x) s[i] = src[i];
    __syncthreads();
    for (uint32_t i = threadIdx.x; i < here * NUM_PLANES; i += blockDim.x) {
        const uint32_t plane = i / here, k = i - plane * here;
        soa[(uint64_t)plane * plane_stride + first + s0 + k] = s[k * NUM_PLANES + plane];
    }
}

constexpr int INGEST_SPLATS = 128;

__device__ __forceinline__ void godot_basis_mul(const float a[3][3], const float b[3][3], float o[3][3]) {
#pragma unroll
    for (int i = 0; i < 3; ++i)
#pragma unroll
        for (int j = 0; j < 3; ++j) o[i][j] = (b[0][j] * a[i][0] + b[1][j] * a[i][1]) + b[2][j] * a[i][2];
}

__global__ void __launch_bounds__(INGEST_SPLATS) ply_to_soa_kernel(const float *__restrict__ ply, uint32_t nprops, uint64_t count, float creation_time,
                                                                  float4 *__restrict__ soa, uint64_t plane_stride, uint64_t first) {
#ifndef GSR_CPU_EMU
    extern __shared__ float s_v[];
#else
    __shared__ float s_v[INGEST_SPLATS * 256];
#endif
    const uint64_t s0 = (uint64_t)blockIdx.x * INGEST_SPLATS;
    const uint32_t here = (uint32_t)((count - s0) < (uint64_t)INGEST_SPLATS ? (count - s0) : INGEST_SPLATS);
    const float *src = ply + s0 * nprops;
    for (uint32_t i = threadIdx.x; i < here * nprops; i += blockDim.x) s_v[i] = src[i];
    __syncthreads();
    if (threadIdx.x >= here) return;
    const float *p = s_v + (size_t)threadIdx.x * nprops;
    const uint64_t id = first + s0 + threadIdx.x;

    const float sc0 = (float)exp((double)p[55]), sc1 = (float)exp((double)p[56]), sc2 = (float)exp((double)p[57]);
    const float qx = p[59], qy = p[60], qz = p[61], qw = p[58];
    const float d = ((qx * qx + qy * qy) + qz * qz) + qw * qw;
    const float s = 2.0f / d;
    const float xs = qx * s, ys = qy * s, zs = qz * s;
    const float wx = qw * xs, wy = qw * ys, wz = qw * zs;
    const float xx = qx * xs, xy = qx * ys, xz = qx * zs;
    const float yy = qy * ys, yz = qy * zs, zz = qz * zs;
    const float Bq[3][3] = {{1.0f - (yy + zz), xy - wz, xz + wy}, {xy + wz, 1.0f - (xx + zz), yz - wx}, {xz - wy, yz + wx, 1.0f - (xx + yy)}};
    float R[3][3], M[3][3], Mt[3][3], Cv[3][3];
    const float S[3][3] = {{sc0, 0.0f, 0.0f}, {0.0f, sc1, 0.0f}, {0.0f, 0.0f, sc2}};
#pragma unroll
    for (int r = 0; r < 3; ++r)
#pragma unroll
        for (int c = 0; c < 3; ++c) R[r][c] = Bq[c][r];
    godot_basis_mul(S, R, M);
#pragma unroll
    for (int r = 0; r < 3; ++r)
#pragma unroll
        for (int c = 0; c < 3; ++c) Mt[r][c] = M[c][r];
    godot_basis_mul(Mt, M, Cv);
    const float opacity = (float)(1.0 / (1.0 + exp(-(double)p[54])));

    soa[0 * plane_stride + id] = make_float4(p[0], p[1], p[2], creation_time);
    soa[1 * plane_stride + id] = make_float4(Cv[0][0], Cv[0][1], Cv[0][2], Cv[1][1]);
    soa[2 * plane_stride + id] = make_float4(Cv[1][2], Cv[2][2], opacity, 0.0f);
    float sh[48];
    sh[0] = p[6]; sh[1] = p[7]; sh[2] = p[8];
#pragma unroll
    for (int k = 0; k < 15; ++k) { sh[3 + 3 * k + 0] = p[9 + k]; sh[3 + 3 * k + 1] = p[9 + 15 + k]; sh[3 + 3 * k + 2] = p[9 + 30 + k]; }
#pragma unroll
    for (int k = 0; k < 12; ++k) soa[(uint64_t)(3 + k) * plane_stride + id] = make_float4(sh[4 * k], sh[4 * k + 1], sh[4 * k + 2], sh[4 * k + 3]);
}

}

#ifndef GSR_CPU_EMU
int preload_ingest_kernels() {
    cudaFuncAttributes fa;
    GSR_CUDA_TRY(cudaFuncGetAttributes(&fa, ply_to_soa_kernel));
    GSR_CUDA_TRY(cudaFuncGetAttributes(&fa, aos_to_soa_kernel));
    return GSR_OK;
}
int launch_ply_to_soa(const float *ply, uint32_t nprops, uint64_t count, float creation_time, float4 *soa, uint64_t plane_stride, uint64_t first,
                      cudaStream_t stream) {
    if (count == 0) return GSR_OK;
    const size_t smem = sizeof(float) * (size_t)INGEST_SPLATS * nprops;
    if (smem > 48 * 1024) GSR_CUDA_TRY(cudaFuncSetAttribute(ply_to_soa_kernel, cudaFuncAttributeMaxDynamicSharedMemorySize, (int)smem));
    const uint32_t blocks = (uint32_t)((count + INGEST_SPLATS - 1) / INGEST_SPLATS);
    ply_to_soa_kernel<<<blocks, INGEST_SPLATS, smem, stream>>>(ply, nprops, count, creation_time, soa, plane_stride, first);
    GSR_CUDA_TRY(cudaGetLastError());
    return GSR_OK;
}

int launch_aos_to_soa(const float4 *aos, uint64_t count, float4 *soa, uint64_t plane_stride, uint64_t first, cudaStream_t stream) {
    if (count == 0) return GSR_OK;
    const uint32_t blocks = (uint32_t)((count + SPLATS_PER_BLOCK - 1) / SPLATS_PER_BLOCK);
    aos_to_soa_kernel<<<blocks, 256, 0, stream>>>(aos, count, soa, plane_stride, first);
    GSR_CUDA_TRY(cudaGetLastError());
    return GSR_OK;
}
#endif

}
```

### godotgaussiansplatting_b200/csrc/projection.cu

```cuda
#include <string.h>

#include "common.cuh"

namespace gsr {

namespace {

constexpr float SH_C0 = 0.28209479177387814f;
constexpr float SH_C1 = 0.4886025119029199f;
constexpr float SH_C2_0 = 1.0925484305920792f;
constexpr float SH_C2_1 = 1.0925484305920792f;
constexpr float SH_C2_2 = 0.31539156525252005f;
constexpr float SH_C2_3 = 1.0925484305920792f;
constexpr float SH_C2_4 = 0.5462742152960396f;
constexpr float SH_C3_0 = 0.5900435899266435f;
constexpr float SH_C3_1 = 2.890611442640554f;
constexpr float SH_C3_2 = 0.4570457994644658f;
constexpr float SH_C3_3 = 0.3731763325901154f;
constexpr float SH_C3_4 = 0.4570457994644658f;
constexpr float SH_C3_5 = 1.445305721320277f;
constexpr float SH_C3_6 = 0.5900435899266435f;

#define LB_AGG (1ull << 62)
#define LB_PREFIX (2ull << 62)
#define LB_VAL ((1ull << 62) - 1ull)

struct Mat3 { float m[3][3]; };

__device__ __forceinline__ float ease_out_cubic(float x) {
    float a = 1.0f - x;
    return 1.0f - a * a * a;
}

__device__ __forceinline__ uint32_t warp_incl_scan_u32(uint32_t v, uint32_t lane) {
#pragma unroll
    for (int o = 1; o < 32; o <<= 1) {
        const uint32_t t = __shfl_up_sync(0xffffffffu, v, o);
        if (lane >= (uint32_t)o) v += t;
    }
    return v;
}

__device__ __forceinline__ unsigned long long lookback_exclusive(volatile unsigned long long *status, uint32_t bid,
                                                                 unsigned long long total, uint32_t lane) {
    if (bid == 0) return 0ull;
    unsigned long long excl = 0ull;
    int64_t start = (int64_t)bid - 1;
    while (true) {
        const int64_t t = start - (int64_t)lane;
        unsigned long long v = (t >= 0) ? status[t] : LB_PREFIX;
        while (__any_sync(0xffffffffu, (v >> 62) == 0ull)) {
            if ((v >> 62) == 0ull) v = status[t];
        }
        const uint32_t pmask = __ballot_sync(0xffffffffu, (v >> 62) == 2ull);
        const uint32_t first = pmask ? (uint32_t)(__ffs(pmask) - 1) : 32u;
        unsigned long long c = (lane <= first) ? (v & LB_VAL) : 0ull;
#pragma unroll
        for (int o = 16; o > 0; o >>= 1) c += __shfl_xor_sync(0xffffffffu, c, o);
        excl += c;
        if (pmask) break;
        start -= 32;
    }
    if (lane == 0) status[bid] = LB_PREFIX | ((excl + total) & LB_VAL);
    return excl;
}

#ifndef GSR_CPU_EMU
__device__ __forceinline__ uint32_t smem_u32(const void *p) { return (uint32_t)__cvta_generic_to_shared(p); }
__device__ __forceinline__ void mbar_init(uint64_t *bar, uint32_t count) {
    asm volatile("mbarrier.init.shared::cta.b64 [%0], %1;" ::"r"(smem_u32(bar)), "r"(count) : "memory");
}
__device__ __forceinline__ void fence_mbar_init() { asm volatile("fence.mbarrier_init.release.cluster;" ::: "memory"); }
__device__ __forceinline__ void mbar_expect_tx(uint64_t *bar, uint32_t bytes) {
    asm volatile("mbarrier.arrive.expect_tx.shared::cta.b64 _, [%0], %1;" ::"r"(smem_u32(bar)), "r"(bytes) : "memory");
}
__device__ __forceinline__ void bulk_g2s(void *dst, const void *src, uint32_t bytes, uint64_t *bar) {
    asm volatile("cp.async.bulk.shared::cluster.global.mbarrier::complete_tx::bytes [%0], [%1], %2, [%3];" ::"r"(smem_u32(dst)), "l"(src),
                 "r"(bytes), "r"(smem_u32(bar))
                 : "memory");
}
__device__ __forceinline__ void mbar_wait(uint64_t *bar, uint32_t parity) {
    uint32_t ok;
    do {
        asm volatile("{\n\t.reg .pred p;\n\tmbarrier.try_wait.parity.shared::cta.b64 p, [%1], %2;\n\tselp.u32 %0, 1, 0, p;\n\t}"
                     : "=r"(ok)
                     : "r"(smem_u32(bar)), "r"(parity)
                     : "memory");
    } while (!ok);
}
#else
inline void mbar_init(uint64_t *, uint32_t) {}
inline void fence_mbar_init() {}
inline void mbar_expect_tx(uint64_t *, uint32_t) {}
inline void bulk_g2s(void *dst, const void *src, uint32_t bytes, uint64_t *) { memcpy(dst, src, bytes); }
inline void mbar_wait(uint64_t *, uint32_t) {}
#endif

template <bool FROM_SMEM>
__device__ __forceinline__ void sh_color(const float4 *src, uint64_t stride, float x, float y, float z, float col[3]) {
    const float xx = x * x, yy = y * y, zz = z * z, xy = x * y, yz = y * z, xz = x * z;
    {
        float sh[24];
#pragma unroll
        for (int k = 0; k < 6; ++k) {
            const float4 v = FROM_SMEM ? src[(uint64_t)k * stride] : __ldg(src + (uint64_t)k * stride);
            sh[4 * k + 0] = v.x; sh[4 * k + 1] = v.y; sh[4 * k + 2] = v.z; sh[4 * k + 3] = v.w;
        }
#pragma unroll
        for (int ch = 0; ch < 3; ++ch) {
#define SHC(k) (sh[3 * (k) + ch])
            float r = 0.5f + SHC(0) * SH_C0;
            r = r - SHC(1) * SH_C1 * y;
            r = r + SHC(2) * SH_C1 * z;
            r = r - SHC(3) * SH_C1 * x;
            r = r + SHC(4) * SH_C2_0 * xy;
            r = r - SHC(5) * SH_C2_1 * yz;
            r = r + SHC(6) * SH_C2_2 * (2.0f * zz - xx - yy);
            r = r - SHC(7) * SH_C2_3 * xz;
#undef SHC
            col[ch] = r;
        }
    }
    {
        float sh[24];
#pragma unroll
        for (int k = 0; k < 6; ++k) {
            const float4 v = FROM_SMEM ? src[(uint64_t)(6 + k) * stride] : __ldg(src + (uint64_t)(6 + k) * stride);
            sh[4 * k + 0] = v.x; sh[4 * k + 1] = v.y; sh[4 * k + 2] = v.z; sh[4 * k + 3] = v.w;
        }
#pragma unroll
        for (int ch = 0; ch < 3; ++ch) {
#define SHC(k) (sh[3 * ((k) - 8) + ch])
            float r = col[ch];
            r = r + SHC(8) * SH_C2_4 * (xx - yy);
            r = r - SHC(9) * SH_C3_0 * y * (3.0f * xx - yy);
            r = r + SHC(10) * SH_C3_1 * x * yz;
            r = r - SHC(11) * SH_C3_2 * y * (4.0f * zz - xx - yy);
            r = r + SHC(12) * SH_C3_3 * z * (2.0f * zz - 3.0f * xx - 3.0f * yy);
            r = r - SHC(13) * SH_C3_4 * x * (4.0f * zz - xx - yy);
            r = r + SHC(14) * SH_C3_5 * z * (xx - yy);
            r = r - SHC(15) * SH_C3_6 * x * (xx - 3.0f * yy);
#undef SHC
            col[ch] = g_max(0.0f, r);
        }
    }
}

struct LaneOut {
    uint32_t n, x0, y0, w, depth;
    int32_t last_tile;
    float4 r0, r1;
    float opacity, vx, vy, vz;
};

template <bool QUICK>
__device__ __forceinline__ bool project_lane(const ProjectionArgs &a, const float4 pt, const float4 ca, const float4 cb, LaneOut &o) {
    const float *V = a.vp, *P = a.vp + 16;
    const int W = a.u.dims[0], H = a.u.dims[1];
    const uint32_t gx = (uint32_t)((W + TILE - 1) / TILE), gy = (uint32_t)((H + TILE - 1) / TILE);
    const float ms = a.u.model_scale;
    o.n = 0; o.last_tile = -1;
            const float sp0 = pt.x * ms, sp1 = pt.y * ms, sp2 = pt.z * ms;
            float view[4], clip[4];
#pragma unroll
            for (int r = 0; r < 4; ++r) view[r] = ((V[0 + r] * sp0 + V[4 + r] * sp1) + V[8 + r] * sp2) + V[12 + r] * 1.0f;
#pragma unroll
            for (int r = 0; r < 4; ++r) clip[r] = ((P[0 + r] * view[0] + P[4 + r] * view[1]) + P[8 + r] * view[2]) + P[12 + r] * view[3];
            const float vb = clip[3] * 1.2f;
            if (clip[0] < -vb || clip[1] < -vb || clip[2] < 0.0f || clip[0] > vb || clip[1] > vb || clip[2] > clip[3]) return false;


            const float splat_time = a.u.time - pt.w;
            const float tf = ease_out_cubic(g_clamp(splat_time, 0.0f, 1.0f));
            const float tfl = ease_out_cubic(g_clamp(splat_time - 0.35f, 0.0f, 1.0f));
            const float splat_opacity = cb.z * tfl * tfl;
            const float splat_scale = ms * (2.0f * (1.0f - tfl) + 1.0f * tfl);

            const float z_inv = 1.0f / view[2];
            const float focal0 = a.focal_base[0] * z_inv, focal1 = a.focal_base[1] * z_inv;
            const float mx = g_clamp(view[0] * z_inv, a.lim_lo[0], a.lim_hi[0]);
            const float my = g_clamp(view[1] * z_inv, a.lim_lo[1], a.lim_hi[1]);
            const float ndc0 = clip[0] / clip[3], ndc1 = clip[1] / clip[3], ndc2 = clip[2] / clip[3];
            const float ipx = ((ndc0 + 1.0f) * 0.5f - 1.0f * (1.0f - tf)) * (float)(W - 1);
            const float ipy = ((ndc1 + 1.0f) * 0.5f - 0.75f * (1.0f - tf)) * (float)(H - 1);

            if (a.fast_reject) {
                const float sf2 = (ca.x * ca.x + ca.w * ca.w + cb.y * cb.y) + 2.0f * (ca.y * ca.y + ca.z * ca.z + cb.x * cb.x);
                const float lam = sqrtf(sf2) * splat_scale * splat_scale * 1.0001f;
                const float jf2 = focal0 * focal0 + focal1 * focal1 * (1.0f + mx * mx + my * my);
                const float rb = g_max(1.0f, splat_opacity) * 2.5f * sqrtf(lam * jf2 * a.w_frob2 + 0.92f) * 1.001f + 1.0f;
                const float fa = floorf((ipy - rb) * 0.0625f), fb = floorf((ipy + rb) * 0.0625f);
                if (fa == fa && fb == fb && fabsf(fa) < 1.0e9f && fabsf(fb) < 1.0e9f) {
                    int32_t lo = (int32_t)fa, hi = (int32_t)fb;
                    if (lo < a.band_y0) lo = a.band_y0;
                    if (hi > a.band_y1 - 1) hi = a.band_y1 - 1;
                    if (hi < lo) return false;
                    const int32_t first = lo + ((a.row_rem - lo % a.row_mod) + a.row_mod) % a.row_mod;
                    if (first > hi) return false;
                }
            }

            if (QUICK) return true;

            Mat3 cov3 = {{{ca.x, ca.y, ca.z}, {ca.y, ca.w, cb.x}, {ca.z, cb.x, cb.y}}};
#pragma unroll
            for (int c = 0; c < 3; ++c)
#pragma unroll
                for (int r = 0; r < 3; ++r) cov3.m[c][r] = cov3.m[c][r] * splat_scale * splat_scale;
            const float j02 = -focal1 * mx, j12 = -focal1 * my;
            float B0[3], B1[3];
#pragma unroll
            for (int r = 0; r < 3; ++r) {
                B0[r] = V[4 * r + 0] * focal0 + V[4 * r + 2] * j02;
                B1[r] = V[4 * r + 1] * focal1 + V[4 * r + 2] * j12;
            }
            float T0[3], T1[3];
#pragma unroll
            for (int c = 0; c < 3; ++c) {
                T0[c] = (B0[0] * cov3.m[c][0] + B0[1] * cov3.m[c][1]) + B0[2] * cov3.m[c][2];
                T1[c] = (B1[0] * cov3.m[c][0] + B1[1] * cov3.m[c][1]) + B1[2] * cov3.m[c][2];
            }
            const float c2_00 = (T0[0] * B0[0] + T0[1] * B0[1]) + T0[2] * B0[2];
            const float c2_01 = (T1[0] * B0[0] + T1[1] * B0[1]) + T1[2] * B0[2];
            const float c2_11 = (T1[0] * B1[0] + T1[1] * B1[1]) + T1[2] * B1[2];
            const float cx = c2_00 + 0.3f, cy = c2_01, cz = c2_11 + 0.3f;

            const float det = cx * cz - cy * cy;
            if (det == 0.0f) return false;
            const float mid = 0.5f * (cx + cz);
            const float sq = sqrtf(g_max(0.1f, mid * mid - det));
            const float e1 = mid + 1.0f * sq, e2 = mid + -1.0f * sq;
            if (e1 < 0.0f || e2 < 0.0f) return false;


            const float radius = det_pow(splat_opacity, 0.2f) * 2.5f * sqrtf(g_max(e1, e2));
            if (!(fabsf(ipx) <= 3.0e38f) || !(fabsf(ipy) <= 3.0e38f) || !(radius <= 3.0e38f)) return false;
            const float fgx = (float)gx, fgy = (float)gy;
            int32_t x0 = (int32_t)g_clamp((ipx - radius) / 16.0f, 0.0f, fgx);
            int32_t y0 = (int32_t)g_clamp((ipy - radius) / 16.0f, 0.0f, fgy);
            int32_t x1 = (int32_t)g_clamp(ceilf((ipx + radius) / 16.0f), 0.0f, fgx);
            int32_t y1 = (int32_t)g_clamp(ceilf((ipy + radius) / 16.0f), 0.0f, fgy);
            if ((uint32_t)(x1 - x0) * (uint32_t)(y1 - y0) != 0u) o.last_tile = (y1 - 1) * (int32_t)gx + (x1 - 1);
            if (y0 < a.band_y0) y0 = a.band_y0;
            if (y1 > a.band_y1) y1 = a.band_y1;
            if (y1 < y0) y1 = y0;
            int32_t nrows = y1 - y0;
            if (a.row_mod > 1) {
                y0 += ((a.row_rem - y0 % a.row_mod) + a.row_mod) % a.row_mod;
                nrows = y0 < y1 ? (y1 - 1 - y0) / a.row_mod + 1 : 0;
            }
            const uint32_t nt = (uint32_t)(x1 - x0) * (uint32_t)nrows;
            if (a.fast_mode) o.last_tile = nt ? (y0 + (nrows - 1) * a.row_mod) * (int32_t)gx + (x1 - 1) : -1;
            if (nt == 0u) return false;

            const float d0 = sp0 - a.u.camera_pos[0], d1 = sp1 - a.u.camera_pos[1], d2 = sp2 - a.u.camera_pos[2];
            const float inv_len = 1.0f / sqrtf((d0 * d0 + d1 * d1) + d2 * d2);
            o.vx = d0 * inv_len; o.vy = d1 * inv_len; o.vz = d2 * inv_len; o.opacity = splat_opacity;
            o.r0.x = ipx; o.r0.y = ipy; o.r0.z = sp0; o.r0.w = sp1;
            o.r1.x = cz / det; o.r1.y = -cy / det; o.r1.z = cx / det; o.r1.w = sp2;
            o.depth = ((uint32_t)(ndc2 * ndc2 * ndc2 * 65535.0f)) & 0xFFFFu;
            o.n = nt; o.x0 = (uint32_t)x0; o.y0 = (uint32_t)y0; o.w = (uint32_t)(x1 - x0);

    return true;
}

constexpr int PROJ_WARPS = PROJ_THREADS / 32;
#ifndef GSR_PROJ_MIN_BLOCKS
#define GSR_PROJ_MIN_BLOCKS 3
#endif
constexpr size_t PROJ_SLAB_BYTES = sizeof(float4) * NUM_PLANES * 32;
constexpr size_t PROJ_SMEM_BYTES = PROJ_SLAB_BYTES * PROJ_WARPS;

__global__ void __launch_bounds__(PROJ_THREADS, GSR_PROJ_MIN_BLOCKS) projection_kernel(const __grid_constant__ ProjectionArgs a) {
#ifndef GSR_CPU_EMU
    extern __shared__ __align__(128) unsigned char proj_smem[];
#else
    __shared__ __align__(128) unsigned char proj_smem[PROJ_SMEM_BYTES];
#endif
    __shared__ uint32_t s_bid;
    __shared__ __align__(8) uint64_t s_bar[PROJ_WARPS][2];
    __shared__ uint32_t s_wtotal[PROJ_WARPS];
    __shared__ uint32_t s_count, s_ready, s_nvis;
    __shared__ int32_t s_last;
    __shared__ unsigned long long s_cta_base;
    __shared__ uint4 s_res[PROJ_THREADS];
    __shared__ uint16_t s_list[PROJ_THREADS];
    __shared__ uint32_t s_ncomp;

    const uint32_t tid = threadIdx.x, lane = tid & 31u, warp = tid >> 5;
    float4 *slab = reinterpret_cast<float4 *>(proj_smem + (size_t)warp * PROJ_SLAB_BYTES);
    if (lane == 0) {
        mbar_init(&s_bar[warp][0], 1);
        mbar_init(&s_bar[warp][1], 1);
        fence_mbar_init();
    }
    if (tid == 0) {
        s_bid = atomicAdd(&a.frame->proj_ticket, 1u);
        s_count = 0u; s_ready = 0u; s_nvis = 0u; s_last = -1; s_ncomp = 0u;
    }
    __syncthreads();
    const uint32_t bid = s_bid;
    const uint32_t vwarp = bid * PROJ_WARPS + warp;
    const uint32_t id0 = vwarp * 32u;
    const uint32_t id = id0 + lane;

    if (lane == 0) {
        mbar_expect_tx(&s_bar[warp][0], 3u * 512u);
#pragma unroll
        for (int k = 0; k < 3; ++k) bulk_g2s(slab + k * 32, a.soa + (uint64_t)k * a.plane_stride + id0, 512u, &s_bar[warp][0]);
    }

    const uint32_t gx = (uint32_t)((a.u.dims[0] + TILE - 1) / TILE);

    uint32_t n = 0, x0u = 0, y0u = 0, wu = 0, depth = 0;
    int32_t last_tile = -1;
    float4 r0, r1;
    float splat_opacity = 0.0f, vx = 0.0f, vy = 0.0f, vz = 0.0f;

    mbar_wait(&s_bar[warp][0], 0);
    bool colour_done = false;
    if (!a.fast_reject) {
        if (id < a.num_splats) {
            LaneOut o;
            if (project_lane<false>(a, slab[lane], slab[32 + lane], slab[64 + lane], o) && o.n) {
                n = o.n; x0u = o.x0; y0u = o.y0; wu = o.w; depth = o.depth;
                r0 = o.r0; r1 = o.r1; splat_opacity = o.opacity; vx = o.vx; vy = o.vy; vz = o.vz;
            }
            last_tile = o.last_tile;
        }
    } else {
        bool live = false;
        LaneOut q;
        if (id < a.num_splats) live = project_lane<true>(a, slab[lane], slab[32 + lane], slab[64 + lane], q);
        s_res[tid] = make_uint4(0u, 0u, 0u, 0xFFFFFFFFu);
        const uint32_t lmask = __ballot_sync(0xffffffffu, live);
        uint32_t wbase = 0;
        if (lane == 0 && lmask) wbase = atomicAdd(&s_ncomp, (uint32_t)__popc(lmask));
        wbase = __shfl_sync(0xffffffffu, wbase, 0);
        if (live) s_list[wbase + __popc(lmask & ((1u << lane) - 1u))] = (uint16_t)tid;
        __syncthreads();
        const uint32_t nsurv = s_ncomp;
        if (tid < nsurv) {
            const uint32_t li = s_list[tid];
            const float4 *sl = reinterpret_cast<const float4 *>(proj_smem + (size_t)(li >> 5) * PROJ_SLAB_BYTES);
            const uint32_t l2 = li & 31u;
            const uint32_t gid = bid * PROJ_THREADS + li;
            LaneOut o;
            if (project_lane<false>(a, sl[l2], sl[32 + l2], sl[64 + l2], o) && o.n) {
                float col[3];
                sh_color<false>(a.soa + 3ull * a.plane_stride + gid, a.plane_stride, o.vx, o.vy, o.vz, col);
                float4 *rec = a.records + (uint64_t)gid * 3u;
                rec[0] = o.r0; rec[1] = o.r1; rec[2] = make_float4(col[0], col[1], col[2], o.opacity);
                s_res[li] = make_uint4(o.n, o.x0 | (o.y0 << 16), o.w | (o.depth << 16), (uint32_t)o.last_tile);
            }
        }
        __syncthreads();
        const uint4 r = s_res[tid];
        n = r.x; x0u = r.y & 0xFFFFu; y0u = r.y >> 16; wu = r.z & 0xFFFFu; depth = r.z >> 16; last_tile = (int32_t)r.w;
        colour_done = true;
    }

    const uint32_t incl = warp_incl_scan_u32(n, lane);
    const uint32_t total = __shfl_sync(0xffffffffu, incl, 31);
    const uint32_t emit_mask = __ballot_sync(0xffffffffu, n != 0u);
    const uint32_t nvis = __popc(emit_mask);
    const int32_t wl = __reduce_max_sync(0xffffffffu, last_tile);
    bool closer = false;
    uint32_t cta_total = 0;
    if (lane == 0) {
        s_wtotal[warp] = total;
        if (nvis) atomicAdd(&s_nvis, nvis);
        if (wl >= 0) atomicMax(&s_last, wl);
        __threadfence_block();
        closer = atomicAdd(&s_count, 1u) == PROJ_WARPS - 1;
        if (closer) {
            __threadfence_block();
#pragma unroll
            for (int w = 0; w < PROJ_WARPS; ++w) cta_total += ((volatile uint32_t *)s_wtotal)[w];
            volatile unsigned long long *st = a.lookback + bid;
            *st = (bid == 0 ? LB_PREFIX : LB_AGG) | (unsigned long long)cta_total;
        }
    }
    closer = __shfl_sync(0xffffffffu, (int)closer, 0) != 0;
    cta_total = __shfl_sync(0xffffffffu, cta_total, 0);

    const bool bulk = !colour_done && nvis >= (uint32_t)a.sh_bulk_min;
    if (bulk && lane == 0) {
        mbar_expect_tx(&s_bar[warp][1], 12u * 512u);
#pragma unroll
        for (int k = 3; k < NUM_PLANES; ++k) bulk_g2s(slab + k * 32, a.soa + (uint64_t)k * a.plane_stride + id0, 512u, &s_bar[warp][1]);
    }
    if (closer) {
        const unsigned long long cta_base = lookback_exclusive(a.lookback, bid, (unsigned long long)cta_total, lane);
        if (lane == 0) {
            s_cta_base = cta_base;
            __threadfence_block();
            *(volatile uint32_t *)&s_ready = 1u;
            const uint32_t nv = *(volatile uint32_t *)&s_nvis;
            const int32_t lt = *(volatile int32_t *)&s_last;
            if (nv) atomicAdd(&a.frame->visible, nv);
            if (lt >= 0) atomicMax(&a.frame->last_tile_plus1, lt + 1);
            if (bid == gridDim.x - 1) {
                const unsigned long long m = cta_base + cta_total;
                a.frame->dup_total = m;
                a.frame->dup_sorted = m < (unsigned long long)a.capacity ? (uint32_t)m : a.capacity;
                a.frame->overflow = m > (unsigned long long)a.capacity ? 1u : 0u;
            }
        }
    }
    if (bulk) {
        mbar_wait(&s_bar[warp][1], 0);
        if (n) {
            float col[3];
            sh_color<true>(slab + 3 * 32 + lane, 32, vx, vy, vz, col);
            float4 *rec = a.records + (uint64_t)id * 3u;
            rec[0] = r0; rec[1] = r1; rec[2] = make_float4(col[0], col[1], col[2], splat_opacity);
        }
    } else if (n && !colour_done) {
        float col[3];
        sh_color<false>(a.soa + 3ull * a.plane_stride + id, a.plane_stride, vx, vy, vz, col);
        float4 *rec = a.records + (uint64_t)id * 3u;
        rec[0] = r0; rec[1] = r1; rec[2] = make_float4(col[0], col[1], col[2], splat_opacity);
    }

    unsigned long long base = 0;
    if (lane == 0) {
        while (*(volatile uint32_t *)&s_ready == 0u) __nanosleep(100);
        __threadfence_block();
        base = *(volatile unsigned long long *)&s_cta_base;
        for (uint32_t w = 0; w < warp; ++w) base += ((volatile uint32_t *)s_wtotal)[w];
    }
    base = __shfl_sync(0xffffffffu, base, 0);

    constexpr uint32_t EMIT_SMALL = 4;
    const uint32_t my_off = incl - n;
    if (n != 0u && n <= EMIT_SMALL) {
        uint32_t x = x0u, y = y0u;
        const uint32_t x1 = x0u + wu;
#pragma unroll
        for (uint32_t j = 0; j < EMIT_SMALL; ++j) {
            if (j < n) {
                const unsigned long long g = base + my_off + j;
                if (g < (unsigned long long)a.capacity) {
                    a.keys[g] = ((y * gx + x) << 16) | depth;
                    a.values[g] = id;
                }
                if (++x == x1) { x = x0u; y += (uint32_t)a.row_mod; }
            }
        }
    }
    uint32_t big = __ballot_sync(0xffffffffu, n > EMIT_SMALL);
    while (big) {
        const int src = __ffs(big) - 1;
        big &= big - 1u;
        const uint32_t sn = __shfl_sync(0xffffffffu, n, src), soff = __shfl_sync(0xffffffffu, my_off, src);
        const uint32_t sx0 = __shfl_sync(0xffffffffu, x0u, src), sy0 = __shfl_sync(0xffffffffu, y0u, src);
        const uint32_t sw = __shfl_sync(0xffffffffu, wu, src), sdepth = __shfl_sync(0xffffffffu, depth, src);
        for (uint32_t j = lane; j < sn; j += 32u) {
            const uint32_t ry = j / sw, rx = j - ry * sw;
            const unsigned long long g = base + soff + j;
            if (g < (unsigned long long)a.capacity) {
                a.keys[g] = (((sy0 + ry * (uint32_t)a.row_mod) * gx + sx0 + rx) << 16) | sdepth;
                a.values[g] = id0 + (uint32_t)src;
            }
        }
    }
}

constexpr int SH_GROUPS = 4;
constexpr int SH_SPLATS = SH_GROUPS * PROJ_THREADS;
constexpr size_t SH_SLAB_BYTES = sizeof(float4) * 3 * SH_SPLATS;

__global__ void __launch_bounds__(PROJ_THREADS, 3) projection_sharded_kernel(const __grid_constant__ ProjectionArgs a) {
#ifndef GSR_CPU_EMU
    extern __shared__ __align__(128) unsigned char proj_smem[];
#else
    __shared__ __align__(128) unsigned char proj_smem[SH_SLAB_BYTES];
#endif
    __shared__ uint4 s_res[SH_SPLATS];
    __shared__ uint16_t s_list[SH_SPLATS];
    __shared__ __align__(8) uint64_t s_bar[PROJ_WARPS];
    __shared__ uint32_t s_bid, s_ncomp, s_wsum[PROJ_WARPS], s_nvis;
    __shared__ int32_t s_last;
    __shared__ unsigned long long s_base;

    const uint32_t tid = threadIdx.x, lane = tid & 31u, warp = tid >> 5;
    float4 *slab = reinterpret_cast<float4 *>(proj_smem);
    auto slab_at = [&](uint32_t slot, int plane) -> const float4 & {
        return slab[((slot >> 5) * 3u + (uint32_t)plane) * 32u + (slot & 31u)];
    };
    if (lane == 0) { mbar_init(&s_bar[warp], 1); fence_mbar_init(); }
    if (tid == 0) { s_bid = atomicAdd(&a.frame->proj_ticket, 1u); s_ncomp = 0u; s_nvis = 0u; s_last = -1; }
#pragma unroll
    for (int r = 0; r < SH_GROUPS; ++r) s_res[r * PROJ_THREADS + tid] = make_uint4(0u, 0u, 0u, 0xFFFFFFFFu);
    __syncthreads();
    const uint32_t bid = s_bid;
    const uint32_t base_id = bid * SH_SPLATS;
    const uint32_t gx = (uint32_t)((a.u.dims[0] + TILE - 1) / TILE);

    if (lane == 0) {
        mbar_expect_tx(&s_bar[warp], 12u * 512u);
#pragma unroll
        for (int g = 0; g < SH_GROUPS; ++g)
#pragma unroll
            for (int k = 0; k < 3; ++k)
                bulk_g2s(slab + ((g * PROJ_WARPS + warp) * 3u + k) * 32u, a.soa + (uint64_t)k * a.plane_stride + base_id + g * PROJ_THREADS + warp * 32u,
                         512u, &s_bar[warp]);
    }
    mbar_wait(&s_bar[warp], 0);

#pragma unroll
    for (int g = 0; g < SH_GROUPS; ++g) {
        const uint32_t slot = g * PROJ_THREADS + tid;
        bool live = false;
        LaneOut q;
        if (base_id + slot < a.num_splats) live = project_lane<true>(a, slab_at(slot, 0), slab_at(slot, 1), slab_at(slot, 2), q);
        const uint32_t lmask = __ballot_sync(0xffffffffu, live);
        uint32_t wbase = 0;
        if (lane == 0 && lmask) wbase = atomicAdd(&s_ncomp, (uint32_t)__popc(lmask));
        wbase = __shfl_sync(0xffffffffu, wbase, 0);
        if (live) s_list[wbase + __popc(lmask & ((1u << lane) - 1u))] = (uint16_t)slot;
    }
    __syncthreads();

    const uint32_t nsurv = s_ncomp;
    for (uint32_t it = tid; it < nsurv; it += PROJ_THREADS) {
        const uint32_t slot = s_list[it];
        const uint32_t gid = base_id + slot;
        LaneOut o;
        const bool hit = project_lane<false>(a, slab_at(slot, 0), slab_at(slot, 1), slab_at(slot, 2), o);
        if (hit && o.n) {
            float col[3];
            sh_color<false>(a.soa + 3ull * a.plane_stride + gid, a.plane_stride, o.vx, o.vy, o.vz, col);
            float4 *rec = a.records + (uint64_t)gid * 3u;
            rec[0] = o.r0; rec[1] = o.r1; rec[2] = make_float4(col[0], col[1], col[2], o.opacity);
            s_res[slot] = make_uint4(o.n, o.x0 | (o.y0 << 16), o.w | (o.depth << 16), (uint32_t)o.last_tile);
        }
    }
    __syncthreads();

    uint4 r[SH_GROUPS];
    uint32_t tsum = 0, tvis = 0;
    int32_t tlast = -1;
#pragma unroll
    for (int j = 0; j < SH_GROUPS; ++j) {
        r[j] = s_res[SH_GROUPS * tid + j];
        tsum += r[j].x;
        tvis += r[j].x != 0u;
        tlast = tlast > (int32_t)r[j].w ? tlast : (int32_t)r[j].w;
    }
    const uint32_t incl = warp_incl_scan_u32(tsum, lane);
    if (lane == 31) s_wsum[warp] = incl;
    const uint32_t wvis = __reduce_add_sync(0xffffffffu, tvis);
    const int32_t wlast = __reduce_max_sync(0xffffffffu, tlast);
    if (lane == 0) {
        if (wvis) atomicAdd(&s_nvis, wvis);
        if (wlast >= 0) atomicMax(&s_last, wlast);
    }
    __syncthreads();
    uint32_t woff = 0, total = 0;
#pragma unroll
    for (uint32_t w = 0; w < PROJ_WARPS; ++w) {
        const uint32_t sw = s_wsum[w];
        if (w < warp) woff += sw;
        total += sw;
    }
    uint32_t off = woff + incl - tsum;

    if (warp == 0) {
        if (lane == 0) {
            volatile unsigned long long *st = a.lookback + bid;
            *st = (bid == 0 ? LB_PREFIX : LB_AGG) | (unsigned long long)total;
        }
        __syncwarp();
        const unsigned long long cb = lookback_exclusive(a.lookback, bid, (unsigned long long)total, lane);
        if (lane == 0) {
            s_base = cb;
            const uint32_t nv = s_nvis;
            const int32_t lt = s_last;
            if (nv) atomicAdd(&a.frame->visible, nv);
            if (lt >= 0) atomicMax(&a.frame->last_tile_plus1, lt + 1);
            if (bid == gridDim.x - 1) {
                const unsigned long long m = cb + total;
                a.frame->dup_total = m;
                a.frame->dup_sorted = m < (unsigned long long)a.capacity ? (uint32_t)m : a.capacity;
                a.frame->overflow = m > (unsigned long long)a.capacity ? 1u : 0u;
            }
        }
    }
    __syncthreads();
    const unsigned long long base = s_base;

    constexpr uint32_t EMIT_SMALL = 4;
#pragma unroll
    for (int j = 0; j < SH_GROUPS; ++j) {
        const uint32_t n = r[j].x, x0u = r[j].y & 0xFFFFu, y0u = r[j].y >> 16, wu = r[j].z & 0xFFFFu, depth = r[j].z >> 16;
        const uint32_t id = base_id + SH_GROUPS * tid + j;
        if (n != 0u && n <= EMIT_SMALL) {
            uint32_t x = x0u, y = y0u;
            const uint32_t x1 = x0u + wu;
#pragma unroll
            for (uint32_t e = 0; e < EMIT_SMALL; ++e) {
                if (e < n) {
                    const unsigned long long gpos = base + off + e;
                    if (gpos < (unsigned long long)a.capacity) {
                        a.keys[gpos] = ((y * gx + x) << 16) | depth;
                        a.values[gpos] = id;
                    }
                    if (++x == x1) { x = x0u; y += (uint32_t)a.row_mod; }
                }
            }
        }
        uint32_t big = __ballot_sync(0xffffffffu, n > EMIT_SMALL);
        while (big) {
            const int src = __ffs(big) - 1;
            big &= big - 1u;
            const uint32_t sn = __shfl_sync(0xffffffffu, n, src), soff = __shfl_sync(0xffffffffu, off, src);
            const uint32_t sx0 = __shfl_sync(0xffffffffu, x0u, src), sy0 = __shfl_sync(0xffffffffu, y0u, src);
            const uint32_t sw = __shfl_sync(0xffffffffu, wu, src), sdepth = __shfl_sync(0xffffffffu, depth, src);
            const uint32_t sid = __shfl_sync(0xffffffffu, id, src);
            for (uint32_t e = lane; e < sn; e += 32u) {
                const uint32_t ry = e / sw, rx = e - ry * sw;
                const unsigned long long gpos = base + soff + e;
                if (gpos < (unsigned long long)a.capacity) {
                    a.keys[gpos] = (((sy0 + ry * (uint32_t)a.row_mod) * gx + sx0 + rx) << 16) | sdepth;
                    a.values[gpos] = sid;
                }
            }
        }
        off += n;
    }
}

__device__ __forceinline__ unsigned long long lookback_exclusive_strided(volatile unsigned long long *status, uint32_t stride, uint32_t col, uint32_t bid,
                                                                         unsigned long long total, uint32_t lane) {
    if (bid == 0) return 0ull;
    unsigned long long excl = 0ull;
    int64_t start = (int64_t)bid - 1;
    while (true) {
        const int64_t t = start - (int64_t)lane;
        unsigned long long v = (t >= 0) ? status[(uint64_t)t * stride + col] : LB_PREFIX;
        while (__any_sync(0xffffffffu, (v >> 62) == 0ull)) {
            if ((v >> 62) == 0ull) v = status[(uint64_t)t * stride + col];
        }
        const uint32_t pmask = __ballot_sync(0xffffffffu, (v >> 62) == 2ull);
        const uint32_t first = pmask ? (uint32_t)(__ffs(pmask) - 1) : 32u;
        unsigned long long c = (lane <= first) ? (v & LB_VAL) : 0ull;
#pragma unroll
        for (int o = 16; o > 0; o >>= 1) c += __shfl_xor_sync(0xffffffffu, c, o);
        excl += c;
        if (pmask) break;
        start -= 32;
    }
    if (lane == 0) status[(uint64_t)bid * stride + col] = LB_PREFIX | ((excl + total) & LB_VAL);
    return excl;
}

__device__ __forceinline__ void rows_of(uint32_t y0, uint32_t y1, uint32_t d, uint32_t G, uint32_t &first, uint32_t &count) {
    first = y0 + ((d + G - y0 % G) % G);
    count = first < y1 ? (y1 - 1u - first) / G + 1u : 0u;
}

__global__ void __launch_bounds__(PROJ_THREADS, GSR_PROJ_MIN_BLOCKS) projection_scatter_kernel(const __grid_constant__ ProjectionArgs a,
                                                                                               const __grid_constant__ ScatterPeers sp) {
#ifndef GSR_CPU_EMU
    extern __shared__ __align__(128) unsigned char proj_smem[];
#else
    __shared__ __align__(128) unsigned char proj_smem[PROJ_SMEM_BYTES];
#endif
    __shared__ uint32_t s_bid, s_is_last;
    __shared__ __align__(8) uint64_t s_bar[PROJ_WARPS][2];
    __shared__ uint32_t s_wtotal[PROJ_WARPS][GROUP_MAX];
    __shared__ uint32_t s_count, s_ready, s_nvis;
    __shared__ int32_t s_last;
    __shared__ unsigned long long s_cta_base[GROUP_MAX];

    const uint32_t tid = threadIdx.x, lane = tid & 31u, warp = tid >> 5;
    const uint32_t G = (uint32_t)sp.world;
    float4 *slab = reinterpret_cast<float4 *>(proj_smem + (size_t)warp * PROJ_SLAB_BYTES);
    GroupFlags *mine = sp.flags[sp.rank];
    if (lane == 0) {
        mbar_init(&s_bar[warp][0], 1);
        mbar_init(&s_bar[warp][1], 1);
        fence_mbar_init();
    }
    if (tid == 0) {
        s_bid = atomicAdd(&a.frame->proj_ticket, 1u);
        s_count = 0u; s_ready = 0u; s_nvis = 0u; s_last = -1;
    }
    __syncthreads();
    const uint32_t bid = s_bid;
    const uint32_t li0 = (bid * PROJ_WARPS + warp) * 32u;
    const uint32_t id0 = sp.first + li0, id = id0 + lane;
    const bool warp_in = li0 < sp.count;

    if (warp_in && lane == 0) {
        mbar_expect_tx(&s_bar[warp][0], 3u * 512u);
#pragma unroll
        for (int k = 0; k < 3; ++k) bulk_g2s(slab + k * 32, a.soa + (uint64_t)k * a.plane_stride + id0, 512u, &s_bar[warp][0]);
    }
    const uint32_t gx = (uint32_t)((a.u.dims[0] + TILE - 1) / TILE);

    uint32_t n = 0, x0u = 0, y0u = 0, y1u = 0, wu = 0, depth = 0;
    int32_t last_tile = -1;
    float4 r0 = make_float4(0.f, 0.f, 0.f, 0.f), r1 = r0;
    float splat_opacity = 0.0f, vx = 0.0f, vy = 0.0f, vz = 0.0f;
    if (warp_in) {
        mbar_wait(&s_bar[warp][0], 0);
        if (li0 + lane < sp.count && id < a.num_splats) {
            LaneOut o;
            if (project_lane<false>(a, slab[lane], slab[32 + lane], slab[64 + lane], o) && o.n) {
                n = o.n; x0u = o.x0; y0u = o.y0; wu = o.w; depth = o.depth; y1u = o.y0 + o.n / o.w;
                r0 = o.r0; r1 = o.r1; splat_opacity = o.opacity; vx = o.vx; vy = o.vy; vz = o.vz;
            }
            last_tile = o.last_tile;
        }
    }

    for (uint32_t d = 0; d < G; ++d) {
        uint32_t f, c;
        rows_of(y0u, y1u, d, G, f, c);
        const uint32_t tot = __reduce_add_sync(0xffffffffu, n ? wu * c : 0u);
        if (lane == 0) s_wtotal[warp][d] = tot;
    }
    const uint32_t emit_mask = __ballot_sync(0xffffffffu, n != 0u);
    const uint32_t nvis = __popc(emit_mask);
    const int32_t wl = __reduce_max_sync(0xffffffffu, last_tile);
    bool closer = false;
    if (lane == 0) {
        if (nvis) atomicAdd(&s_nvis, nvis);
        if (wl >= 0) atomicMax(&s_last, wl);
        __threadfence_block();
        closer = atomicAdd(&s_count, 1u) == PROJ_WARPS - 1;
    }
    closer = __shfl_sync(0xffffffffu, (int)closer, 0) != 0;
    uint32_t cta_total = 0;
    if (closer) {
        __threadfence_block();
        if (lane < G) {
#pragma unroll
            for (int w = 0; w < PROJ_WARPS; ++w) cta_total += ((volatile uint32_t *)&s_wtotal[w][0])[lane];
            volatile unsigned long long *st = sp.lookback + (uint64_t)bid * G + lane;
            *st = (bid == 0 ? LB_PREFIX : LB_AGG) | (unsigned long long)cta_total;
        }
    }

    const bool bulk = warp_in && nvis >= (uint32_t)a.sh_bulk_min;
    if (bulk && lane == 0) {
        mbar_expect_tx(&s_bar[warp][1], 12u * 512u);
#pragma unroll
        for (int k = 3; k < NUM_PLANES; ++k) bulk_g2s(slab + k * 32, a.soa + (uint64_t)k * a.plane_stride + id0, 512u, &s_bar[warp][1]);
    }
    if (closer) {
        for (uint32_t d = 0; d < G; ++d) {
            const uint32_t tot_d = __shfl_sync(0xffffffffu, cta_total, (int)d);
            const unsigned long long base_d = lookback_exclusive_strided(sp.lookback, G, d, bid, (unsigned long long)tot_d, lane);
            if (lane == 0) {
                s_cta_base[d] = base_d;
                if (bid == gridDim.x - 1) mine->seg_total[d] = base_d + tot_d;
            }
        }
        if (lane == 0) {
            __threadfence_block();
            *(volatile uint32_t *)&s_ready = 1u;
            const uint32_t nv = *(volatile uint32_t *)&s_nvis;
            const int32_t lt = *(volatile int32_t *)&s_last;
            if (nv) atomicAdd(&a.frame->visible, nv);
            if (lt >= 0) atomicMax(&mine->scat_last, lt + 1);
        }
    }
    if (bulk) mbar_wait(&s_bar[warp][1], 0);
    if (n) {
        float col[3];
        if (bulk) sh_color<true>(slab + 3 * 32 + lane, 32, vx, vy, vz, col);
        else sh_color<false>(a.soa + 3ull * a.plane_stride + id, a.plane_stride, vx, vy, vz, col);
        const float4 r2 = make_float4(col[0], col[1], col[2], splat_opacity);
        for (uint32_t d = 0; d < G; ++d) {
            uint32_t f, c;
            rows_of(y0u, y1u, d, G, f, c);
            if (c) {
                float4 *rec = sp.records[d] + (uint64_t)id * 3u;
                rec[0] = r0; rec[1] = r1; rec[2] = r2;
            }
        }
    }

    if (lane == 0) {
        while (*(volatile uint32_t *)&s_ready == 0u) __nanosleep(100);
        __threadfence_block();
    }
    __syncwarp();

    constexpr uint32_t EMIT_SMALL = 4;
    for (uint32_t d = 0; d < G; ++d) {
        uint32_t fy, cnt;
        rows_of(y0u, y1u, d, G, fy, cnt);
        const uint32_t nd = n ? wu * cnt : 0u;
        if (!__any_sync(0xffffffffu, nd != 0u)) continue;
        const uint32_t incl = warp_incl_scan_u32(nd, lane);
        unsigned long long base = 0;
        if (lane == 0) {
            base = *(volatile unsigned long long *)&s_cta_base[d];
            for (uint32_t w = 0; w < warp; ++w) base += ((volatile uint32_t *)&s_wtotal[w][0])[d];
        }
        base = __shfl_sync(0xffffffffu, base, 0);
        uint32_t *kd = sp.keys[d], *vd = sp.values[d];
        const uint32_t my_off = incl - nd;
        if (nd != 0u && nd <= EMIT_SMALL) {
            uint32_t x = x0u, y = fy;
            const uint32_t x1 = x0u + wu;
#pragma unroll
            for (uint32_t j = 0; j < EMIT_SMALL; ++j) {
                if (j < nd) {
                    const unsigned long long g = base + my_off + j;
                    if (g < (unsigned long long)sp.seg_cap) {
                        kd[g] = ((y * gx + x) << 16) | depth;
                        vd[g] = id;
                    }
                    if (++x == x1) { x = x0u; y += G; }
                }
            }
        }
        uint32_t big = __ballot_sync(0xffffffffu, nd > EMIT_SMALL);
        while (big) {
            const int src = __ffs(big) - 1;
            big &= big - 1u;
            const uint32_t sn = __shfl_sync(0xffffffffu, nd, src), soff = __shfl_sync(0xffffffffu, my_off, src);
            const uint32_t sx0 = __shfl_sync(0xffffffffu, x0u, src), sy0 = __shfl_sync(0xffffffffu, fy, src);
            const uint32_t sw = __shfl_sync(0xffffffffu, wu, src), sdepth = __shfl_sync(0xffffffffu, depth, src);
            for (uint32_t j = lane; j < sn; j += 32u) {
                const uint32_t ry = j / sw, rx = j - ry * sw;
                const unsigned long long g = base + soff + j;
                if (g < (unsigned long long)sp.seg_cap) {
                    kd[g] = (((sy0 + ry * G) * gx + sx0 + rx) << 16) | sdepth;
                    vd[g] = id0 + (uint32_t)src;
                }
            }
        }
    }

    __syncthreads();
#ifdef GSR_SCATTER_FENCE_PER_CTA_SYS
    if (tid == 0) __threadfence_system();
#else
    if (tid == 0) __threadfence();
#endif
    if (tid == 0) s_is_last = atomicAdd(&mine->scat_ticket, 1u) == gridDim.x - 1u ? 1u : 0u;
    __syncthreads();
    if (s_is_last && tid < 32u) {
        __threadfence_system();
        const int32_t lp1 = __shfl_sync(0xffffffffu, lane == 0 ? *(volatile int32_t *)&mine->scat_last : 0, 0);
        if (lane < G) {
            const unsigned long long cnt = *(volatile unsigned long long *)&mine->seg_total[lane];
            volatile unsigned long long *m = &sp.flags[lane]->seg_meta[sp.parity][sp.rank][0];
            m[1] = ((unsigned long long)sp.seq << 32) | (unsigned long long)(uint32_t)(lp1 > 0 ? lp1 : 0);
            m[0] = ((unsigned long long)sp.seq << 32) | (cnt < 0xFFFFFFFFull ? cnt : 0xFFFFFFFFull);
        }
        __syncwarp();
        if (lane == 0) { mine->scat_last = 0; mine->scat_ticket = 0u; __threadfence(); }
    }
}

}

uint32_t projection_num_blocks(uint32_t num_splats) { return (num_splats + PROJ_THREADS - 1) / PROJ_THREADS; }

#ifndef GSR_CPU_EMU
int preload_projection_kernels() {
    cudaFuncAttributes fa;
    GSR_CUDA_TRY(cudaFuncSetAttribute(projection_kernel, cudaFuncAttributeMaxDynamicSharedMemorySize, (int)PROJ_SMEM_BYTES));
    GSR_CUDA_TRY(cudaFuncSetAttribute(projection_sharded_kernel, cudaFuncAttributeMaxDynamicSharedMemorySize, (int)SH_SLAB_BYTES));
    GSR_CUDA_TRY(cudaFuncSetAttribute(projection_scatter_kernel, cudaFuncAttributeMaxDynamicSharedMemorySize, (int)PROJ_SMEM_BYTES));
    GSR_CUDA_TRY(cudaFuncGetAttributes(&fa, projection_kernel));
    GSR_CUDA_TRY(cudaFuncGetAttributes(&fa, projection_sharded_kernel));
    GSR_CUDA_TRY(cudaFuncGetAttributes(&fa, projection_scatter_kernel));
    return GSR_OK;
}
uint32_t projection_scatter_blocks(uint32_t count) { return count ? (count + PROJ_THREADS - 1) / PROJ_THREADS : 1u; }

int launch_projection_scatter(const ProjectionArgs &frame_args, const ScatterPeers &sp, cudaStream_t stream) {
    ProjectionArgs a = frame_args;
    a.band_y0 = 0; a.band_y1 = (a.u.dims[1] + TILE - 1) / TILE;
    a.row_mod = 1; a.row_rem = 0; a.fast_reject = 0; a.fast_mode = 0; a.sh_bulk_min = 12;
    projection_scatter_kernel<<<projection_scatter_blocks(sp.count), PROJ_THREADS, PROJ_SMEM_BYTES, stream>>>(a, sp);
    GSR_CUDA_TRY(cudaGetLastError());
    return GSR_OK;
}

int launch_projection(const ProjectionArgs &a, cudaStream_t stream) {
    const uint32_t blocks = projection_num_blocks(a.num_splats);
    if (blocks == 0) return GSR_OK;
    if (a.fast_reject) {
        const uint32_t sblocks = (a.num_splats + SH_SPLATS - 1) / SH_SPLATS;
        projection_sharded_kernel<<<sblocks, PROJ_THREADS, SH_SLAB_BYTES, stream>>>(a);
        GSR_CUDA_TRY(cudaGetLastError());
        return GSR_OK;
    }
    projection_kernel<<<blocks, PROJ_THREADS, PROJ_SMEM_BYTES, stream>>>(a);
    GSR_CUDA_TRY(cudaGetLastError());
    return GSR_OK;
}
#endif

}
```

Before: 3426.

## Defer SH colour evaluation from projection to compositor with splat-major SH buffer

Adds a splat-major copy of the 12 SH planes and a defer_colour mode. In that mode projection stores the splat position in the record instead of a colour, so only 3 planes are staged and projection can run at higher occupancy (min blocks 3→4). Colour is then computed only for splats that reach compositing, either inside the compositor (SH prefetched with cp.async into dynamic shared memory and overlapped with blending) or by a separate fill kernel over the sorted values. The cost is extra shared memory in the compositor, which may lower its occupancy. A splat that covers many tiles may also have its colour recomputed once per tile.

```diff
diff --git a/godotgaussiansplatting_b200/csrc/common.cuh b/godotgaussiansplatting_b200/csrc/common.cuh
--- a/godotgaussiansplatting_b200/csrc/common.cuh
+++ b/godotgaussiansplatting_b200/csrc/common.cuh
@@ -9,6 +9,7 @@
 
 constexpr int TILE = 16;
 constexpr int NUM_PLANES = 15;
+constexpr int SH_PLANES = 12;
 constexpr int PROJ_THREADS = 256;
 
 void set_last_error(const char *fmt, ...);
@@ -66,6 +67,73 @@
     return det_exp2(__fmul_rn(y, det_log2(x)));
 }
 
+template <bool SMEM>
+__device__ __forceinline__ void splat_colour(const float4 *sh, uint64_t stride, float sp0, float sp1, float sp2, const float cam[3], float col[3]) {
+    constexpr float SH_C0 = 0.28209479177387814f;
+    constexpr float SH_C1 = 0.4886025119029199f;
+    constexpr float SH_C2_0 = 1.0925484305920792f;
+    constexpr float SH_C2_1 = 1.0925484305920792f;
+    constexpr float SH_C2_2 = 0.31539156525252005f;
+    constexpr float SH_C2_3 = 1.0925484305920792f;
+    constexpr float SH_C2_4 = 0.5462742152960396f;
+    constexpr float SH_C3_0 = 0.5900435899266435f;
+    constexpr float SH_C3_1 = 2.890611442640554f;
+    constexpr float SH_C3_2 = 0.4570457994644658f;
+    constexpr float SH_C3_3 = 0.3731763325901154f;
+    constexpr float SH_C3_4 = 0.4570457994644658f;
+    constexpr float SH_C3_5 = 1.445305721320277f;
+    constexpr float SH_C3_6 = 0.5900435899266435f;
+    const float d0 = sp0 - cam[0], d1 = sp1 - cam[1], d2 = sp2 - cam[2];
+    const float inv_len = 1.0f / sqrtf((d0 * d0 + d1 * d1) + d2 * d2);
+    const float x = d0 * inv_len, y = d1 * inv_len, z = d2 * inv_len;
+    const float xx = x * x, yy = y * y, zz = z * z, xy = x * y, yz = y * z, xz = x * z;
+    {
+        float sh_[24];
+#pragma unroll
+        for (int k = 0; k < 6; ++k) {
+            const float4 v = SMEM ? sh[(uint64_t)k * stride] : __ldg(sh + (uint64_t)k * stride);
+            sh_[4 * k + 0] = v.x; sh_[4 * k + 1] = v.y; sh_[4 * k + 2] = v.z; sh_[4 * k + 3] = v.w;
+        }
+#pragma unroll
+        for (int ch = 0; ch < 3; ++ch) {
+#define SHC(k) (sh_[3 * (k) + ch])
+            float r = 0.5f + SHC(0) * SH_C0;
+            r = r - SHC(1) * SH_C1 * y;
+            r = r + SHC(2) * SH_C1 * z;
+            r = r - SHC(3) * SH_C1 * x;
+            r = r + SHC(4) * SH_C2_0 * xy;
+            r = r - SHC(5) * SH_C2_1 * yz;
+            r = r + SHC(6) * SH_C2_2 * (2.0f * zz - xx - yy);
+            r = r - SHC(7) * SH_C2_3 * xz;
+#undef SHC
+            col[ch] = r;
+        }
+    }
+    {
+        float sh_[24];
+#pragma unroll
+        for (int k = 0; k < 6; ++k) {
+            const float4 v = SMEM ? sh[(uint64_t)(6 + k) * stride] : __ldg(sh + (uint64_t)(6 + k) * stride);
+            sh_[4 * k + 0] = v.x; sh_[4 * k + 1] = v.y; sh_[4 * k + 2] = v.z; sh_[4 * k + 3] = v.w;
+        }
+#pragma unroll
+        for (int ch = 0; ch < 3; ++ch) {
+#define SHC(k) (sh_[3 * ((k) - 8) + ch])
+            float r = col[ch];
+            r = r + SHC(8) * SH_C2_4 * (xx - yy);
+            r = r - SHC(9) * SH_C3_0 * y * (3.0f * xx - yy);
+            r = r + SHC(10) * SH_C3_1 * x * yz;
+            r = r - SHC(11) * SH_C3_2 * y * (4.0f * zz - xx - yy);
+            r = r + SHC(12) * SH_C3_3 * z * (2.0f * zz - 3.0f * xx - 3.0f * yy);
+            r = r - SHC(13) * SH_C3_4 * x * (4.0f * zz - xx - yy);
+            r = r + SHC(14) * SH_C3_5 * z * (xx - yy);
+            r = r - SHC(15) * SH_C3_6 * x * (xx - 3.0f * yy);
+#undef SHC
+            col[ch] = g_max(0.0f, r);
+        }
+    }
+}
+
 struct FrameState {
     unsigned long long dup_total;
     uint32_t dup_sorted;
@@ -120,6 +188,7 @@
     int32_t row_mod, row_rem;
     int32_t fast_reject;
     int32_t sh_bulk_min;
+    int32_t defer_colour;
     int32_t fast_mode;
     float w_frob2;
     float4 *records;
@@ -199,9 +268,13 @@
     ulonglong4 *trace;
     uint32_t *trace_count;
     uint32_t trace_cap;
+    const float4 *sh;
+    float camera_pos[3];
 };
 int launch_composite(const CompositeArgs &a, cudaStream_t stream);
 int composite_max_ctas_per_sm(int *out);
+int launch_fill_record_colours(const float4 *sh, const float camera_pos[3], const uint32_t *values, const FrameState *frame,
+                               float4 *records, uint32_t max_pairs, uint32_t num_splats, cudaStream_t stream);
 int launch_tile_order(const uint2 *bounds, int32_t tile_begin, int32_t row_step, int32_t tiles_x, int32_t num_tiles, uint32_t *hint, uint32_t *order,
                       FrameState *frame, uint32_t sparse_tiles, uint32_t sparse_cta_limit, cudaStream_t stream);
 
@@ -210,6 +283,7 @@
 int launch_present(const float4 *rgba, void *out, uint64_t pixels, int format, cudaStream_t stream);
 size_t present_bytes_per_pixel(int format);
 int launch_aos_to_soa(const float4 *aos, uint64_t count, float4 *soa, uint64_t plane_stride, uint64_t first, cudaStream_t stream);
+int launch_sh_planes_to_splat(const float4 *soa, uint64_t plane_stride, float4 *sh, uint64_t first, uint64_t count, cudaStream_t stream);
 
 int preload_group_kernels();
 int preload_projection_kernels();
diff --git a/godotgaussiansplatting_b200/csrc/compositor.cu b/godotgaussiansplatting_b200/csrc/compositor.cu
--- a/godotgaussiansplatting_b200/csrc/compositor.cu
+++ b/godotgaussiansplatting_b200/csrc/compositor.cu
@@ -35,15 +35,49 @@
     return s;
 }
 
-__device__ __forceinline__ Staged gather(const float4 *__restrict__ records, const uint32_t *__restrict__ values, uint32_t idx) {
-    const uint32_t v = __ldg(values + idx);
-    const float4 *r = records + (uint64_t)v * 3u;
+#ifndef GSR_CPU_EMU
+__device__ __forceinline__ void cp_async16(void *dst, const void *src) {
+    asm volatile("cp.async.cg.shared.global [%0], [%1], 16;" ::"r"((uint32_t)__cvta_generic_to_shared(dst)), "l"(src) : "memory");
+}
+__device__ __forceinline__ void cp_async_commit() { asm volatile("cp.async.commit_group;" ::: "memory"); }
+__device__ __forceinline__ void cp_async_wait_all() { asm volatile("cp.async.wait_all;" ::: "memory"); }
+#else
+inline void cp_async16(void *dst, const void *src) { memcpy(dst, src, 16); }
+inline void cp_async_commit() {}
+inline void cp_async_wait_all() {}
+#endif
+
+__device__ __forceinline__ Staged gather(const CompositeArgs &p, uint32_t idx, uint32_t *v_out) {
+    const uint32_t v = __ldg(p.values + idx);
+    *v_out = v;
+    const float4 *r = p.records + (uint64_t)v * 3u;
     const float4 r0 = __ldg(r + 0), r1 = __ldg(r + 1), r2 = __ldg(r + 2);
     Staged s;
     s.a = make_float4(r0.x, r0.y, -0.5f * r1.x, -0.5f * r1.z);
-    s.b = make_float4(-r1.y, r2.w, r2.x, r2.y);
-    s.c = r2.z;
+    if (p.sh) {
+        s.b = make_float4(-r1.y, r2.w, r0.z, r0.w);
+        s.c = r1.w;
+    } else {
+        s.b = make_float4(-r1.y, r2.w, r2.x, r2.y);
+        s.c = r2.z;
+    }
     return s;
+}
+
+constexpr uint32_t NO_SPLAT = 0xFFFFFFFFu;
+constexpr int SH_COPIES = 2 * SH_PLANES;
+
+__device__ __forceinline__ void sh_copy(const CompositeArgs &p, float4 *s_sh, uint32_t tid, int q, uint32_t sv0, uint32_t sv1) {
+    const bool hi = q >= SH_PLANES;
+    const int k = hi ? q - SH_PLANES : q;
+    const uint32_t v = hi ? sv1 : sv0;
+    if (v != NO_SPLAT) cp_async16(s_sh + k * CHUNK + tid + (hi ? THREADS : 0), p.sh + (uint64_t)v * SH_PLANES + k);
+}
+
+__device__ __forceinline__ void colour_staged(Staged &s, const float4 *sh, const float cam[3]) {
+    float col[3];
+    splat_colour<true>(sh, CHUNK, s.b.z, s.b.w, s.c, cam, col);
+    s.b.z = col[0]; s.b.w = col[1]; s.c = col[2];
 }
 
 #ifndef GSR_COMP_GROUP
@@ -162,8 +196,15 @@
 #define GSR_COMP_MIN_BLOCKS 3
 #endif
 
+constexpr size_t SH_SMEM_BYTES = sizeof(float4) * SH_PLANES * CHUNK;
+
 template <bool CONTRACT>
 __global__ void __launch_bounds__(THREADS, GSR_COMP_MIN_BLOCKS) composite_kernel(const __grid_constant__ CompositeArgs p) {
+#ifndef GSR_CPU_EMU
+    extern __shared__ float4 s_sh[];
+#else
+    __shared__ float4 s_sh[SH_PLANES * CHUNK];
+#endif
     __shared__ float4 s_a[CHUNK];
     __shared__ float4 s_b[CHUNK];
     __shared__ float s_c[CHUNK];
@@ -204,9 +245,14 @@
         float t0 = 1.0f, t1 = 1.0f;
 
         Staged n0 = null_splat(), n1 = null_splat();
+        uint32_t sv0 = NO_SPLAT, sv1 = NO_SPLAT;
         if (num_iterations > 0) {
-            if ((int)tid < num_splats) n0 = gather(p.records, p.values, bounds.x + tid);
-            if ((int)tid + THREADS < num_splats) n1 = gather(p.records, p.values, bounds.x + tid + THREADS);
+            if ((int)tid < num_splats) n0 = gather(p, bounds.x + tid, &sv0);
+            if ((int)tid + THREADS < num_splats) n1 = gather(p, bounds.x + tid + THREADS, &sv1);
+            if (p.sh) {
+                for (int q = 0; q < SH_COPIES; ++q) sh_copy(p, s_sh, tid, q, sv0, sv1);
+                cp_async_commit();
+            }
         }
 
         int consumed = 0;
@@ -215,14 +261,21 @@
             const int chunk = (num_splats - sort_offset) < CHUNK ? (num_splats - sort_offset) : CHUNK;
             staged += (uint32_t)chunk;
             consumed = i + 1;
+            if (p.sh) {
+                cp_async_wait_all();
+                if ((int)tid < chunk) colour_staged(n0, s_sh + tid, p.camera_pos);
+                if ((int)tid + THREADS < chunk) colour_staged(n1, s_sh + tid + THREADS, p.camera_pos);
+            }
             s_a[tid] = n0.a; s_b[tid] = n0.b; s_c[tid] = n0.c;
             s_a[tid + THREADS] = n1.a; s_b[tid + THREADS] = n1.b; s_c[tid + THREADS] = n1.c;
             __syncthreads();
             n0 = null_splat(); n1 = null_splat();
+            sv0 = NO_SPLAT; sv1 = NO_SPLAT;
+            int q = (p.sh && i + 1 < num_iterations) ? 0 : SH_COPIES;
             if (i + 1 < num_iterations) {
                 const int nb = sort_offset + CHUNK;
-                if (nb + (int)tid < num_splats) n0 = gather(p.records, p.values, bounds.x + (uint32_t)nb + tid);
-                if (nb + (int)tid + THREADS < num_splats) n1 = gather(p.records, p.values, bounds.x + (uint32_t)nb + tid + THREADS);
+                if (nb + (int)tid < num_splats) n0 = gather(p, bounds.x + (uint32_t)nb + tid, &sv0);
+                if (nb + (int)tid + THREADS < num_splats) n1 = gather(p, bounds.x + (uint32_t)nb + tid + THREADS, &sv1);
             }
 
             const int chunkg = (chunk + GU - 1) & ~(GU - 1);
@@ -231,6 +284,7 @@
             for (int u = 0; u < GU; ++u) { A[u] = s_a[u]; B[u] = s_b[u]; }
             bool go = __any_sync(0xffffffffu, (t0 > MIN_ALPHA) || (t1 > MIN_ALPHA));
             for (int j = 0; j < chunkg && go; j += GU) {
+                if (q < SH_COPIES) sh_copy(p, s_sh, tid, q++, sv0, sv1);
                 F2 al2[GU], om2[GU];
                 phase_a<CONTRACT>(A, B, npx2, fpy, K, al2, om2);
                 float4 Bc[GU];
@@ -243,6 +297,10 @@
                 phase_b<CONTRACT>(Bc, s_c, j, al2, om2, cr2, cg2, cb2, t0, t1, alive_mid);
                 go = __any_sync(0xffffffffu, alive_mid);
             }
+            if (p.sh) {
+                for (; q < SH_COPIES; ++q) sh_copy(p, s_sh, tid, q, sv0, sv1);
+                cp_async_commit();
+            }
 
             const uint32_t wsum = __reduce_add_sync(0xffffffffu, (uint32_t)(t0 * 255.0f) + (uint32_t)(t1 * 255.0f));
             if (lane == 0) s_vote[warp] = wsum;
@@ -252,6 +310,7 @@
             for (int w = 0; w < THREADS / 32; ++w) shared_t += s_vote[w];
             if (!(shared_t > 255u)) break;
         }
+        if (p.sh) cp_async_wait_all();
 
         float r0, r1, g0, g1, b0, b1;
         upk(cr2, r0, r1); upk(cg2, g0, g1); upk(cb2, b0, b1);
@@ -283,6 +342,21 @@
     if (tid == 0 && staged && p.count_staged) atomicAdd(&p.frame->staged, (unsigned long long)staged);
 }
 
+__global__ void fill_record_colours_kernel(const float4 *__restrict__ sh, float3 cam, const uint32_t *__restrict__ values,
+                                           const FrameState *frame, float4 *records, uint32_t max_pairs, uint32_t num_splats) {
+    const uint32_t m = frame->dup_sorted < max_pairs ? frame->dup_sorted : max_pairs;
+    const float c[3] = {cam.x, cam.y, cam.z};
+    for (uint32_t i = blockIdx.x * blockDim.x + threadIdx.x; i < m; i += gridDim.x * blockDim.x) {
+        const uint32_t v = values[i];
+        if (v >= num_splats) continue;
+        float4 *rec = records + (uint64_t)v * 3u;
+        const float4 r0 = rec[0], r1 = rec[1];
+        float col[3];
+        splat_colour<false>(sh + (uint64_t)v * SH_PLANES, 1, r0.z, r0.w, r1.w, c, col);
+        rec[2] = make_float4(col[0], col[1], col[2], rec[2].w);
+    }
+}
+
 }
 
 #ifndef GSR_CPU_EMU
@@ -290,13 +364,16 @@
     cudaFuncAttributes fa;
     GSR_CUDA_TRY(cudaFuncGetAttributes(&fa, composite_kernel<true>));
     GSR_CUDA_TRY(cudaFuncGetAttributes(&fa, composite_kernel<false>));
+    GSR_CUDA_TRY(cudaFuncGetAttributes(&fa, fill_record_colours_kernel));
     return GSR_OK;
 }
 
 int composite_max_ctas_per_sm(int *out) {
+    GSR_CUDA_TRY(cudaFuncSetAttribute(composite_kernel<true>, cudaFuncAttributeMaxDynamicSharedMemorySize, (int)SH_SMEM_BYTES));
+    GSR_CUDA_TRY(cudaFuncSetAttribute(composite_kernel<false>, cudaFuncAttributeMaxDynamicSharedMemorySize, (int)SH_SMEM_BYTES));
     int a = 0, b = 0;
-    GSR_CUDA_TRY(cudaOccupancyMaxActiveBlocksPerMultiprocessor(&a, composite_kernel<true>, THREADS, 0));
-    GSR_CUDA_TRY(cudaOccupancyMaxActiveBlocksPerMultiprocessor(&b, composite_kernel<false>, THREADS, 0));
+    GSR_CUDA_TRY(cudaOccupancyMaxActiveBlocksPerMultiprocessor(&a, composite_kernel<true>, THREADS, SH_SMEM_BYTES));
+    GSR_CUDA_TRY(cudaOccupancyMaxActiveBlocksPerMultiprocessor(&b, composite_kernel<false>, THREADS, SH_SMEM_BYTES));
     *out = a < b ? a : b;
     if (*out < 1) *out = 1;
     return GSR_OK;
@@ -306,11 +383,22 @@
     if (a.num_tiles <= 0) return GSR_OK;
     const int per_sm = a.ctas_per_sm > 0 ? a.ctas_per_sm : 1;
     const int grid = a.num_tiles < a.sm_count * per_sm ? a.num_tiles : a.sm_count * per_sm;
-    if (a.contract) composite_kernel<true><<<grid, THREADS, 0, stream>>>(a);
-    else composite_kernel<false><<<grid, THREADS, 0, stream>>>(a);
+    const size_t dyn = a.sh ? SH_SMEM_BYTES : 0;
+    if (a.contract) composite_kernel<true><<<grid, THREADS, dyn, stream>>>(a);
+    else composite_kernel<false><<<grid, THREADS, dyn, stream>>>(a);
     GSR_CUDA_TRY(cudaGetLastError());
     return GSR_OK;
 }
-#endif
-
-}
+
+int launch_fill_record_colours(const float4 *sh, const float camera_pos[3], const uint32_t *values, const FrameState *frame,
+                               float4 *records, uint32_t max_pairs, uint32_t num_splats, cudaStream_t stream) {
+    if (max_pairs == 0) return GSR_OK;
+    const uint32_t blocks = (max_pairs + 255u) / 256u < 4096u ? (max_pairs + 255u) / 256u : 4096u;
+    fill_record_colours_kernel<<<blocks, 256, 0, stream>>>(sh, make_float3(camera_pos[0], camera_pos[1], camera_pos[2]), values, frame,
+                                                           records, max_pairs, num_splats);
+    GSR_CUDA_TRY(cudaGetLastError());
+    return GSR_OK;
+}
+#endif
+
+}
diff --git a/godotgaussiansplatting_b200/csrc/gsr_api.cu b/godotgaussiansplatting_b200/csrc/gsr_api.cu
--- a/godotgaussiansplatting_b200/csrc/gsr_api.cu
+++ b/godotgaussiansplatting_b200/csrc/gsr_api.cu
@@ -32,12 +32,15 @@
     uint64_t cap_stride = 0;
     cudaStream_t stream = nullptr, own_stream = nullptr;
     float4 *soa = nullptr;
+    float4 *sh = nullptr;
     float4 *records = nullptr;
     float4 *records2 = nullptr;
     uint32_t *keys = nullptr;
     uint32_t *vals = nullptr;
     uint32_t *keys_cur = nullptr, *vals_cur = nullptr;
     float4 *records_cur = nullptr;
+    bool colour_deferred = false;
+    float colour_cam[3] = {0.f, 0.f, 0.f};
     cudaStream_t front_stream = nullptr;
     cudaEvent_t front_gate = nullptr;
     int overlap = -1;
@@ -152,7 +155,7 @@
     cudaSetDevice(c->device);
     if (c->stream) cudaStreamSynchronize(c->stream);
     if (c->front_stream) { cudaStreamSynchronize(c->front_stream); cudaStreamDestroy(c->front_stream); }
-    cudaFree(c->soa); cudaFree(c->records); cudaFree(c->records2); cudaFree(c->keys); cudaFree(c->vals);
+    cudaFree(c->soa); cudaFree(c->sh); cudaFree(c->records); cudaFree(c->records2); cudaFree(c->keys); cudaFree(c->vals);
     sort_workspace_destroy(c->sort);
     if (c->copy_stream) cudaStreamSynchronize(c->copy_stream);
     if (c->peer_opened) { cudaIpcCloseMemHandle(c->peer_fb[0]); cudaIpcCloseMemHandle(c->peer_fb[1]); }
@@ -251,6 +254,7 @@
     }
     if (se != cudaSuccess) { set_last_error("copy stream/events -> %s", cudaGetErrorString(se)); free_ctx(c); return GSR_ERR_CUDA; }
     TRY_ALLOC(c->soa, sizeof(float4) * NUM_PLANES * c->plane_stride);
+    TRY_ALLOC(c->sh, sizeof(float4) * SH_PLANES * c->plane_stride);
     TRY_ALLOC(c->records, sizeof(float4) * 3ull * c->max_splats);
     TRY_ALLOC(c->records2, sizeof(float4) * 3ull * c->max_splats);
     c->cap_stride = (c->capacity + 1023ull) & ~1023ull;
@@ -283,6 +287,7 @@
     }
     memset(c->host_ring, 0, sizeof(FrameState) * GSR_HISTORY_FRAMES);
     cudaMemsetAsync(c->soa, 0, sizeof(float4) * NUM_PLANES * c->plane_stride, c->stream);
+    cudaMemsetAsync(c->sh, 0, sizeof(float4) * SH_PLANES * c->plane_stride, c->stream);
     cudaMemsetAsync(c->records, 0, sizeof(float4) * 3ull * c->max_splats, c->stream);
     cudaMemsetAsync(c->records2, 0, sizeof(float4) * 3ull * c->max_splats, c->stream);
     cudaMemsetAsync(c->pick, 0, sizeof(float4), c->stream);
@@ -325,6 +330,7 @@
         if ((rc = launch_aos_to_soa(c->staging, m, c->soa, c->plane_stride, first + done, c->stream))) return rc;
         done += m;
     }
+    if ((rc = launch_sh_planes_to_splat(c->soa, c->plane_stride, c->sh, first, count, c->stream))) return rc;
     GSR_CUDA_TRY(cudaStreamSynchronize(c->stream));
     if (first + count > c->num_splats) c->num_splats = first + count;
     return GSR_OK;
@@ -347,6 +353,7 @@
         if ((rc = launch_ply_to_soa(reinterpret_cast<const float *>(c->staging), nprops, m, creation_time, c->soa, c->plane_stride, first + done, c->stream))) return rc;
         done += m;
     }
+    if ((rc = launch_sh_planes_to_splat(c->soa, c->plane_stride, c->sh, first, count, c->stream))) return rc;
     GSR_CUDA_TRY(cudaStreamSynchronize(c->stream));
     if (first + count > c->num_splats) c->num_splats = first + count;
     return GSR_OK;
@@ -562,7 +569,8 @@
     const bool want_reject = (c->flags & GSR_FLAG_FAST_REJECT) != 0 || c->row_mod >= 6;
     pa.fast_reject = (want_reject && fast) ? 1 : 0;
     pa.fast_mode = fast ? 1 : 0;
-    pa.sh_bulk_min = (fast || c->row_mod > 1) ? 1 : 12;
+    pa.defer_colour = 1;
+    pa.sh_bulk_min = 12;
     pa.records = records; pa.keys = keys_in; pa.values = vals_in; pa.capacity = (uint32_t)c->capacity;
     pa.lookback = c->lookback; pa.frame = c->frame;
     if (gf) {
@@ -608,6 +616,8 @@
         launches += 2;
     }
     c->keys_cur = keys_in; c->vals_cur = vals_in; c->records_cur = records;
+    c->colour_deferred = true;
+    memcpy(c->colour_cam, u.camera_pos, sizeof c->colour_cam);
     GSR_CUDA_TRY(cudaEventRecord(ev[3], s));
 
     if (c->keep_unsorted) {
@@ -660,6 +670,8 @@
         launches += 1;
     }
     ca.trace = c->trace; ca.trace_count = c->trace_count; ca.trace_cap = c->trace_cap;
+    ca.sh = c->sh;
+    memcpy(ca.camera_pos, u.camera_pos, sizeof ca.camera_pos);
     if (c->trace) GSR_CUDA_TRY(cudaMemsetAsync(c->trace_count, 0, sizeof(uint32_t), s));
     if (gf && !gf->rows_local && c->grp.rank != 0 && gf->seq >= 3u) {
         if ((rc = launch_group_wait_released(c->grp.flags[c->grp.rank], gf->seq - 2u, s))) return rc;
@@ -1039,6 +1051,8 @@
         ca.order = nullptr; ca.consumed = nullptr; ca.ctas_per_sm = 1; ca.sm_count = c->sm_count;
         ca.contract = (c->flags & GSR_FLAG_UNCONTRACTED_BLEND) ? 0 : 1;
         ca.trace = nullptr; ca.trace_count = nullptr; ca.trace_cap = 0;
+        ca.sh = c->colour_deferred ? c->sh : nullptr;
+        memcpy(ca.camera_pos, c->colour_cam, sizeof ca.camera_pos);
         for (int i = 0; i < 2; ++i)
             if (c->copied_valid[i]) GSR_CUDA_TRY(cudaStreamWaitEvent(c->stream, c->ev_copied[i], 0));
         GSR_CUDA_TRY(cudaMemsetAsync(c->pick_frame, 0, sizeof(FrameState), c->stream));
@@ -1161,6 +1175,10 @@
         default: set_last_error("gsr_debug_copy: unknown buffer %d", which); return GSR_ERR_INVALID;
     }
     if (!src || bytes > avail) { set_last_error("gsr_debug_copy(%d): %zu bytes requested, %zu available", which, bytes, avail); return GSR_ERR_INVALID; }
+    if (which == GSR_BUF_RECORDS && c->colour_deferred) {
+        if ((rc = launch_fill_record_colours(c->sh, c->colour_cam, c->vals_cur, c->frame, c->records_cur, (uint32_t)c->capacity,
+                                             (uint32_t)c->max_splats, c->stream))) return rc;
+    }
     GSR_CUDA_TRY(cudaMemcpyAsync(dst, src, bytes, cudaMemcpyDeviceToHost, c->stream));
     GSR_CUDA_TRY(cudaStreamSynchronize(c->stream));
     return GSR_OK;
diff --git a/godotgaussiansplatting_b200/csrc/ingest.cu b/godotgaussiansplatting_b200/csrc/ingest.cu
--- a/godotgaussiansplatting_b200/csrc/ingest.cu
+++ b/godotgaussiansplatting_b200/csrc/ingest.cu
@@ -79,6 +79,15 @@
     for (int k = 0; k < 12; ++k) soa[(uint64_t)(3 + k) * plane_stride + id] = make_float4(sh[4 * k], sh[4 * k + 1], sh[4 * k + 2], sh[4 * k + 3]);
 }
 
+__global__ void __launch_bounds__(256) sh_planes_to_splat_kernel(const float4 *__restrict__ soa, uint64_t plane_stride, float4 *__restrict__ sh,
+                                                                 uint64_t first, uint64_t count) {
+    const uint64_t t = (uint64_t)blockIdx.x * blockDim.x + threadIdx.x;
+    if (t >= count * SH_PLANES) return;
+    const uint64_t id = first + t / SH_PLANES;
+    const uint32_t k = (uint32_t)(t % SH_PLANES);
+    sh[id * SH_PLANES + k] = soa[(uint64_t)(3 + k) * plane_stride + id];
+}
+
 }
 
 #ifndef GSR_CPU_EMU
@@ -86,6 +95,15 @@
     cudaFuncAttributes fa;
     GSR_CUDA_TRY(cudaFuncGetAttributes(&fa, ply_to_soa_kernel));
     GSR_CUDA_TRY(cudaFuncGetAttributes(&fa, aos_to_soa_kernel));
+    GSR_CUDA_TRY(cudaFuncGetAttributes(&fa, sh_planes_to_splat_kernel));
+    return GSR_OK;
+}
+
+int launch_sh_planes_to_splat(const float4 *soa, uint64_t plane_stride, float4 *sh, uint64_t first, uint64_t count, cudaStream_t stream) {
+    if (count == 0) return GSR_OK;
+    const uint64_t items = count * SH_PLANES;
+    sh_planes_to_splat_kernel<<<(uint32_t)((items + 255) / 256), 256, 0, stream>>>(soa, plane_stride, sh, first, count);
+    GSR_CUDA_TRY(cudaGetLastError());
     return GSR_OK;
 }
 int launch_ply_to_soa(const float *ply, uint32_t nprops, uint64_t count, float creation_time, float4 *soa, uint64_t plane_stride, uint64_t first,
diff --git a/godotgaussiansplatting_b200/csrc/projection.cu b/godotgaussiansplatting_b200/csrc/projection.cu
--- a/godotgaussiansplatting_b200/csrc/projection.cu
+++ b/godotgaussiansplatting_b200/csrc/projection.cu
@@ -5,21 +5,6 @@
 namespace gsr {
 
 namespace {
-
-constexpr float SH_C0 = 0.28209479177387814f;
-constexpr float SH_C1 = 0.4886025119029199f;
-constexpr float SH_C2_0 = 1.0925484305920792f;
-constexpr float SH_C2_1 = 1.0925484305920792f;
-constexpr float SH_C2_2 = 0.31539156525252005f;
-constexpr float SH_C2_3 = 1.0925484305920792f;
-constexpr float SH_C2_4 = 0.5462742152960396f;
-constexpr float SH_C3_0 = 0.5900435899266435f;
-constexpr float SH_C3_1 = 2.890611442640554f;
-constexpr float SH_C3_2 = 0.4570457994644658f;
-constexpr float SH_C3_3 = 0.3731763325901154f;
-constexpr float SH_C3_4 = 0.4570457994644658f;
-constexpr float SH_C3_5 = 1.445305721320277f;
-constexpr float SH_C3_6 = 0.5900435899266435f;
 
 #define LB_AGG (1ull << 62)
 #define LB_PREFIX (2ull << 62)
@@ -96,62 +81,18 @@
 inline void mbar_wait(uint64_t *, uint32_t) {}
 #endif
 
-template <bool FROM_SMEM>
-__device__ __forceinline__ void sh_color(const float4 *src, uint64_t stride, float x, float y, float z, float col[3]) {
-    const float xx = x * x, yy = y * y, zz = z * z, xy = x * y, yz = y * z, xz = x * z;
-    {
-        float sh[24];
-#pragma unroll
-        for (int k = 0; k < 6; ++k) {
-            const float4 v = FROM_SMEM ? src[(uint64_t)k * stride] : __ldg(src + (uint64_t)k * stride);
-            sh[4 * k + 0] = v.x; sh[4 * k + 1] = v.y; sh[4 * k + 2] = v.z; sh[4 * k + 3] = v.w;
-        }
-#pragma unroll
-        for (int ch = 0; ch < 3; ++ch) {
-#define SHC(k) (sh[3 * (k) + ch])
-            float r = 0.5f + SHC(0) * SH_C0;
-            r = r - SHC(1) * SH_C1 * y;
-            r = r + SHC(2) * SH_C1 * z;
-            r = r - SHC(3) * SH_C1 * x;
-            r = r + SHC(4) * SH_C2_0 * xy;
-            r = r - SHC(5) * SH_C2_1 * yz;
-            r = r + SHC(6) * SH_C2_2 * (2.0f * zz - xx - yy);
-            r = r - SHC(7) * SH_C2_3 * xz;
-#undef SHC
-            col[ch] = r;
-        }
-    }
-    {
-        float sh[24];
-#pragma unroll
-        for (int k = 0; k < 6; ++k) {
-            const float4 v = FROM_SMEM ? src[(uint64_t)(6 + k) * stride] : __ldg(src + (uint64_t)(6 + k) * stride);
-            sh[4 * k + 0] = v.x; sh[4 * k + 1] = v.y; sh[4 * k + 2] = v.z; sh[4 * k + 3] = v.w;
-        }
-#pragma unroll
-        for (int ch = 0; ch < 3; ++ch) {
-#define SHC(k) (sh[3 * ((k) - 8) + ch])
-            float r = col[ch];
-            r = r + SHC(8) * SH_C2_4 * (xx - yy);
-            r = r - SHC(9) * SH_C3_0 * y * (3.0f * xx - yy);
-            r = r + SHC(10) * SH_C3_1 * x * yz;
-            r = r - SHC(11) * SH_C3_2 * y * (4.0f * zz - xx - yy);
-            r = r + SHC(12) * SH_C3_3 * z * (2.0f * zz - 3.0f * xx - 3.0f * yy);
-            r = r - SHC(13) * SH_C3_4 * x * (4.0f * zz - xx - yy);
-            r = r + SHC(14) * SH_C3_5 * z * (xx - yy);
-            r = r - SHC(15) * SH_C3_6 * x * (xx - 3.0f * yy);
-#undef SHC
-            col[ch] = g_max(0.0f, r);
-        }
-    }
-}
-
 struct LaneOut {
     uint32_t n, x0, y0, w, depth;
     int32_t last_tile;
     float4 r0, r1;
-    float opacity, vx, vy, vz;
+    float opacity;
 };
+
+__device__ __forceinline__ float4 record_word2(const ProjectionArgs &a, uint32_t id, const float4 &r0, const float4 &r1, float opacity) {
+    float col[3] = {0.0f, 0.0f, 0.0f};
+    if (!a.defer_colour) splat_colour<false>(a.soa + 3ull * a.plane_stride + id, a.plane_stride, r0.z, r0.w, r1.w, a.u.camera_pos, col);
+    return make_float4(col[0], col[1], col[2], opacity);
+}
 
 template <bool QUICK>
 __device__ __forceinline__ bool project_lane(const ProjectionArgs &a, const float4 pt, const float4 ca, const float4 cb, LaneOut &o) {
@@ -253,9 +194,7 @@
             if (a.fast_mode) o.last_tile = nt ? (y0 + (nrows - 1) * a.row_mod) * (int32_t)gx + (x1 - 1) : -1;
             if (nt == 0u) return false;
 
-            const float d0 = sp0 - a.u.camera_pos[0], d1 = sp1 - a.u.camera_pos[1], d2 = sp2 - a.u.camera_pos[2];
-            const float inv_len = 1.0f / sqrtf((d0 * d0 + d1 * d1) + d2 * d2);
-            o.vx = d0 * inv_len; o.vy = d1 * inv_len; o.vz = d2 * inv_len; o.opacity = splat_opacity;
+            o.opacity = splat_opacity;
             o.r0.x = ipx; o.r0.y = ipy; o.r0.z = sp0; o.r0.w = sp1;
             o.r1.x = cz / det; o.r1.y = -cy / det; o.r1.z = cx / det; o.r1.w = sp2;
             o.depth = ((uint32_t)(ndc2 * ndc2 * ndc2 * 65535.0f)) & 0xFFFFu;
@@ -266,10 +205,13 @@
 
 constexpr int PROJ_WARPS = PROJ_THREADS / 32;
 #ifndef GSR_PROJ_MIN_BLOCKS
-#define GSR_PROJ_MIN_BLOCKS 3
+#define GSR_PROJ_MIN_BLOCKS 4
 #endif
 constexpr size_t PROJ_SLAB_BYTES = sizeof(float4) * NUM_PLANES * 32;
 constexpr size_t PROJ_SMEM_BYTES = PROJ_SLAB_BYTES * PROJ_WARPS;
+constexpr size_t PROJ_DEFER_SLAB_BYTES = sizeof(float4) * 3 * 32;
+__device__ __forceinline__ size_t proj_slab_bytes(const ProjectionArgs &a) { return a.defer_colour ? PROJ_DEFER_SLAB_BYTES : PROJ_SLAB_BYTES; }
+inline size_t proj_smem_bytes(const ProjectionArgs &a) { return (a.defer_colour ? PROJ_DEFER_SLAB_BYTES : PROJ_SLAB_BYTES) * PROJ_WARPS; }
 
 __global__ void __launch_bounds__(PROJ_THREADS, GSR_PROJ_MIN_BLOCKS) projection_kernel(const __grid_constant__ ProjectionArgs a) {
 #ifndef GSR_CPU_EMU
@@ -288,7 +230,8 @@
     __shared__ uint32_t s_ncomp;
 
     const uint32_t tid = threadIdx.x, lane = tid & 31u, warp = tid >> 5;
-    float4 *slab = reinterpret_cast<float4 *>(proj_smem + (size_t)warp * PROJ_SLAB_BYTES);
+    const size_t slab_bytes = proj_slab_bytes(a);
+    float4 *slab = reinterpret_cast<float4 *>(proj_smem + (size_t)warp * slab_bytes);
     if (lane == 0) {
         mbar_init(&s_bar[warp][0], 1);
         mbar_init(&s_bar[warp][1], 1);
@@ -315,7 +258,7 @@
     uint32_t n = 0, x0u = 0, y0u = 0, wu = 0, depth = 0;
     int32_t last_tile = -1;
     float4 r0, r1;
-    float splat_opacity = 0.0f, vx = 0.0f, vy = 0.0f, vz = 0.0f;
+    float splat_opacity = 0.0f;
 
     mbar_wait(&s_bar[warp][0], 0);
     bool colour_done = false;
@@ -324,7 +267,7 @@
             LaneOut o;
             if (project_lane<false>(a, slab[lane], slab[32 + lane], slab[64 + lane], o) && o.n) {
                 n = o.n; x0u = o.x0; y0u = o.y0; wu = o.w; depth = o.depth;
-                r0 = o.r0; r1 = o.r1; splat_opacity = o.opacity; vx = o.vx; vy = o.vy; vz = o.vz;
+                r0 = o.r0; r1 = o.r1; splat_opacity = o.opacity;
             }
             last_tile = o.last_tile;
         }
@@ -342,15 +285,13 @@
         const uint32_t nsurv = s_ncomp;
         if (tid < nsurv) {
             const uint32_t li = s_list[tid];
-            const float4 *sl = reinterpret_cast<const float4 *>(proj_smem + (size_t)(li >> 5) * PROJ_SLAB_BYTES);
+            const float4 *sl = reinterpret_cast<const float4 *>(proj_smem + (size_t)(li >> 5) * slab_bytes);
             const uint32_t l2 = li & 31u;
             const uint32_t gid = bid * PROJ_THREADS + li;
             LaneOut o;
             if (project_lane<false>(a, sl[l2], sl[32 + l2], sl[64 + l2], o) && o.n) {
-                float col[3];
-                sh_color<false>(a.soa + 3ull * a.plane_stride + gid, a.plane_stride, o.vx, o.vy, o.vz, col);
                 float4 *rec = a.records + (uint64_t)gid * 3u;
-                rec[0] = o.r0; rec[1] = o.r1; rec[2] = make_float4(col[0], col[1], col[2], o.opacity);
+                rec[0] = o.r0; rec[1] = o.r1; rec[2] = record_word2(a, gid, o.r0, o.r1, o.opacity);
                 s_res[li] = make_uint4(o.n, o.x0 | (o.y0 << 16), o.w | (o.depth << 16), (uint32_t)o.last_tile);
             }
         }
@@ -384,7 +325,7 @@
     closer = __shfl_sync(0xffffffffu, (int)closer, 0) != 0;
     cta_total = __shfl_sync(0xffffffffu, cta_total, 0);
 
-    const bool bulk = !colour_done && nvis >= (uint32_t)a.sh_bulk_min;
+    const bool bulk = !colour_done && !a.defer_colour && nvis >= (uint32_t)a.sh_bulk_min;
     if (bulk && lane == 0) {
         mbar_expect_tx(&s_bar[warp][1], 12u * 512u);
 #pragma unroll
@@ -408,19 +349,17 @@
             }
         }
     }
-    if (bulk) {
-        mbar_wait(&s_bar[warp][1], 0);
-        if (n) {
+    if (bulk) mbar_wait(&s_bar[warp][1], 0);
+    if (n && !colour_done) {
+        float4 *rec = a.records + (uint64_t)id * 3u;
+        rec[0] = r0; rec[1] = r1;
+        if (bulk) {
             float col[3];
-            sh_color<true>(slab + 3 * 32 + lane, 32, vx, vy, vz, col);
-            float4 *rec = a.records + (uint64_t)id * 3u;
-            rec[0] = r0; rec[1] = r1; rec[2] = make_float4(col[0], col[1], col[2], splat_opacity);
-        }
-    } else if (n && !colour_done) {
-        float col[3];
-        sh_color<false>(a.soa + 3ull * a.plane_stride + id, a.plane_stride, vx, vy, vz, col);
-        float4 *rec = a.records + (uint64_t)id * 3u;
-        rec[0] = r0; rec[1] = r1; rec[2] = make_float4(col[0], col[1], col[2], splat_opacity);
+            splat_colour<true>(slab + 3 * 32 + lane, 32, r0.z, r0.w, r1.w, a.u.camera_pos, col);
+            rec[2] = make_float4(col[0], col[1], col[2], splat_opacity);
+        } else {
+            rec[2] = record_word2(a, id, r0, r1, splat_opacity);
+        }
     }
 
     unsigned long long base = 0;
@@ -530,10 +469,8 @@
         LaneOut o;
         const bool hit = project_lane<false>(a, slab_at(slot, 0), slab_at(slot, 1), slab_at(slot, 2), o);
         if (hit && o.n) {
-            float col[3];
-            sh_color<false>(a.soa + 3ull * a.plane_stride + gid, a.plane_stride, o.vx, o.vy, o.vz, col);
             float4 *rec = a.records + (uint64_t)gid * 3u;
-            rec[0] = o.r0; rec[1] = o.r1; rec[2] = make_float4(col[0], col[1], col[2], o.opacity);
+            rec[0] = o.r0; rec[1] = o.r1; rec[2] = record_word2(a, gid, o.r0, o.r1, o.opacity);
             s_res[slot] = make_uint4(o.n, o.x0 | (o.y0 << 16), o.w | (o.depth << 16), (uint32_t)o.last_tile);
         }
     }
@@ -677,7 +614,7 @@
 
     const uint32_t tid = threadIdx.x, lane = tid & 31u, warp = tid >> 5;
     const uint32_t G = (uint32_t)sp.world;
-    float4 *slab = reinterpret_cast<float4 *>(proj_smem + (size_t)warp * PROJ_SLAB_BYTES);
+    float4 *slab = reinterpret_cast<float4 *>(proj_smem + (size_t)warp * proj_slab_bytes(a));
     GroupFlags *mine = sp.flags[sp.rank];
     if (lane == 0) {
         mbar_init(&s_bar[warp][0], 1);
@@ -704,14 +641,14 @@
     uint32_t n = 0, x0u = 0, y0u = 0, y1u = 0, wu = 0, depth = 0;
     int32_t last_tile = -1;
     float4 r0 = make_float4(0.f, 0.f, 0.f, 0.f), r1 = r0;
-    float splat_opacity = 0.0f, vx = 0.0f, vy = 0.0f, vz = 0.0f;
+    float splat_opacity = 0.0f;
     if (warp_in) {
         mbar_wait(&s_bar[warp][0], 0);
         if (li0 + lane < sp.count && id < a.num_splats) {
             LaneOut o;
             if (project_lane<false>(a, slab[lane], slab[32 + lane], slab[64 + lane], o) && o.n) {
                 n = o.n; x0u = o.x0; y0u = o.y0; wu = o.w; depth = o.depth; y1u = o.y0 + o.n / o.w;
-                r0 = o.r0; r1 = o.r1; splat_opacity = o.opacity; vx = o.vx; vy = o.vy; vz = o.vz;
+                r0 = o.r0; r1 = o.r1; splat_opacity = o.opacity;
             }
             last_tile = o.last_tile;
         }
@@ -745,7 +682,7 @@
         }
     }
 
-    const bool bulk = warp_in && nvis >= (uint32_t)a.sh_bulk_min;
+    const bool bulk = warp_in && !a.defer_colour && nvis >= (uint32_t)a.sh_bulk_min;
     if (bulk && lane == 0) {
         mbar_expect_tx(&s_bar[warp][1], 12u * 512u);
 #pragma unroll
@@ -771,10 +708,14 @@
     }
     if (bulk) mbar_wait(&s_bar[warp][1], 0);
     if (n) {
-        float col[3];
-        if (bulk) sh_color<true>(slab + 3 * 32 + lane, 32, vx, vy, vz, col);
-        else sh_color<false>(a.soa + 3ull * a.plane_stride + id, a.plane_stride, vx, vy, vz, col);
-        const float4 r2 = make_float4(col[0], col[1], col[2], splat_opacity);
+        float4 r2;
+        if (bulk) {
+            float col[3];
+            splat_colour<true>(slab + 3 * 32 + lane, 32, r0.z, r0.w, r1.w, a.u.camera_pos, col);
+            r2 = make_float4(col[0], col[1], col[2], splat_opacity);
+        } else {
+            r2 = record_word2(a, id, r0, r1, splat_opacity);
+        }
         for (uint32_t d = 0; d < G; ++d) {
             uint32_t f, c;
             rows_of(y0u, y1u, d, G, f, c);
@@ -882,7 +823,7 @@
     ProjectionArgs a = frame_args;
     a.band_y0 = 0; a.band_y1 = (a.u.dims[1] + TILE - 1) / TILE;
     a.row_mod = 1; a.row_rem = 0; a.fast_reject = 0; a.fast_mode = 0; a.sh_bulk_min = 12;
-    projection_scatter_kernel<<<projection_scatter_blocks(sp.count), PROJ_THREADS, PROJ_SMEM_BYTES, stream>>>(a, sp);
+    projection_scatter_kernel<<<projection_scatter_blocks(sp.count), PROJ_THREADS, proj_smem_bytes(a), stream>>>(a, sp);
     GSR_CUDA_TRY(cudaGetLastError());
     return GSR_OK;
 }
@@ -896,7 +837,7 @@
         GSR_CUDA_TRY(cudaGetLastError());
         return GSR_OK;
     }
-    projection_kernel<<<blocks, PROJ_THREADS, PROJ_SMEM_BYTES, stream>>>(a);
+    projection_kernel<<<blocks, PROJ_THREADS, proj_smem_bytes(a), stream>>>(a);
     GSR_CUDA_TRY(cudaGetLastError());
     return GSR_OK;
 }
```

After: 3712 (median of 6 runs). 1.08x the previous value.
